# Spockuto/drand

Hardware: AMD Instinct MI355X
Metric: beacons verified/s (batch chain verify) (higher is better)
Workload: dtype u32 (381-bit Montgomery, 12x32-bit limbs); 1 GPU; configs[1]: 1000000-round chained beacon history per GPU, chain.VerifyBeacon per round; beacons_per_gpu=1000000, segment_len=64, parallelism=range-shard x1

## Files before the change

drand_amd/csrc/bls_constants.h:

```cpp
#pragma once
#include <stdint.h>
namespace bls {
static constexpr uint32_t P_RAW[12] = {0xffffaaabu, 0xb9feffffu, 0xb153ffffu, 0x1eabfffeu, 0xf6b0f624u, 0x6730d2a0u, 0xf38512bfu, 0x64774b84u, 0x434bacd7u, 0x4b1ba7b6u, 0x397fe69au, 0x1a0111eau};
static constexpr uint32_t P2_RAW[12] = {0xffff5556u, 0x73fdffffu, 0x62a7ffffu, 0x3d57fffdu, 0xed61ec48u, 0xce61a541u, 0xe70a257eu, 0xc8ee9709u, 0x869759aeu, 0x96374f6cu, 0x72ffcd34u, 0x340223d4u};
static constexpr uint32_t P4_RAW[12] = {0xfffeaaacu, 0xe7fbffffu, 0xc54ffffeu, 0x7aaffffau, 0xdac3d890u, 0x9cc34a83u, 0xce144afdu, 0x91dd2e13u, 0xd2eb35du, 0x2c6e9ed9u, 0xe5ff9a69u, 0x680447a8u};
static constexpr uint32_t P_INV32 = 0xfffcfffdu;
static constexpr uint32_t P_INV28 = 0xffcfffdu;
static constexpr uint32_t NEG28_16P[14] = {0x1ffaaab0u, 0x1efffffeu, 0x1ffffb9eu, 0x1ffeb152u, 0x1241eabeu, 0x10f6b0f5u, 0x16730d29u, 0x138512beu, 0x1774b84eu, 0x1bacd763u, 0x1a7b6433u, 0x169a4b1au, 0x1ea397fdu, 0x1a0110u};
static constexpr uint32_t NEG28_32P[14] = {0x2ff55560u, 0x2dfffffdu, 0x2ffff73du, 0x2ffd62a5u, 0x2483d57du, 0x21ed61eau, 0x2ce61a52u, 0x270a257cu, 0x2ee9709cu, 0x2759aec6u, 0x24f6c867u, 0x2d349635u, 0x2d472ffau, 0x340221u};
static constexpr uint32_t NEG28_4P[14] = {0x1ffeaaacu, 0x1fbffffeu, 0x1ffffee6u, 0x1fffac53u, 0x18907aaeu, 0x183dac3cu, 0x1d9cc349u, 0x1ce144aeu, 0x11dd2e12u, 0x12eb35d8u, 0x1e9ed90cu, 0x19a692c5u, 0x17a8e5feu, 0x68043u};
static constexpr uint32_t P28[14] = {0xfffaaabu, 0xfefffffu, 0x3ffffb9u, 0xfffeb15u, 0x6241eabu, 0xa0f6b0fu, 0xf6730d2u, 0xf38512bu, 0x4774b84u, 0x4bacd76u, 0xba7b643u, 0xe69a4b1u, 0x1ea397fu, 0x1a011u};
static constexpr uint32_t FP_INV_FIX[12] = {0x46546125u, 0x2a3b8f55u, 0x6d2fabd9u, 0xdf7c01c3u, 0xfd5fa0c1u, 0xad2b495du, 0xdb357496u, 0x9be1fa38u, 0x9cf0a900u, 0xd59c4badu, 0xdf0786dcu, 0x59a7509u};
static constexpr uint32_t FP_ONE[12] = {0x347fcb8u, 0x19d80000u, 0x6d2002b1u, 0x12e00cdeu, 0xa2090c72u, 0x37669f83u, 0xda0f73e0u, 0x9b09b42u, 0x8f1297bbu, 0xa7c515d9u, 0xfcfa012cu, 0x577a659u};
static constexpr uint32_t FP_R2[12] = {0x510370edu, 0x626d1c34u, 0xc53e243du, 0xd65aec45u, 0x3317d3b1u, 0x4f36a009u, 0x5d74088bu, 0x8c10ea72u, 0x75865d11u, 0xd507320au, 0xa759fd5cu, 0xc8d4cc8u};
static constexpr uint32_t FP_2POW256_R2[12] = {0xbe8eaa74u, 0xc38ed26eu, 0x981fba0u, 0x7d393ebdu, 0xbbe5d6f8u, 0xa0f90a33u, 0x57cc7447u, 0xc62094au, 0x5091120cu, 0x3c87c481u, 0x306035d0u, 0x122a8du};
static constexpr uint32_t FP_INV2[12] = {0x1a3fe5cu, 0x8cec0000u, 0x36900158u, 0x970066fu, 0xd1048639u, 0x1bb34fc1u, 0x6d07b9f0u, 0x84d84da1u, 0xc7894bddu, 0x53e28aecu, 0xfe7d0096u, 0x2bbd32cu};
static constexpr uint32_t FP_TWO[12] = {0x68ff970u, 0x33b00000u, 0xda400562u, 0x25c019bcu, 0x441218e4u, 0x6ecd3f07u, 0xb41ee7c0u, 0x13613685u, 0x1e252f76u, 0x4f8a2bb3u, 0xf9f40259u, 0xaef4cb3u};
static constexpr uint32_t EXP_P_MINUS_2[12] = {0xffffaaa9u, 0xb9feffffu, 0xb153ffffu, 0x1eabfffeu, 0xf6b0f624u, 0x6730d2a0u, 0xf38512bfu, 0x64774b84u, 0x434bacd7u, 0x4b1ba7b6u, 0x397fe69au, 0x1a0111eau};
static constexpr uint32_t EXP_P_PLUS_1_DIV_4[12] = {0xffffeaabu, 0xee7fbfffu, 0xac54ffffu, 0x7aaffffu, 0x3dac3d89u, 0xd9cc34a8u, 0x3ce144afu, 0xd91dd2e1u, 0x90d2eb35u, 0x92c6e9edu, 0x8e5ff9a6u, 0x680447au};
static constexpr uint32_t EXP_P_MINUS_1_DIV_2[12] = {0xffffd555u, 0xdcff7fffu, 0x58a9ffffu, 0xf55ffffu, 0x7b587b12u, 0xb3986950u, 0x79c2895fu, 0xb23ba5c2u, 0x21a5d66bu, 0x258dd3dbu, 0x1cbff34du, 0xd0088f5u};
static constexpr uint32_t EXP_P_MINUS_3_DIV_4[12] = {0xffffeaaau, 0xee7fbfffu, 0xac54ffffu, 0x7aaffffu, 0x3dac3d89u, 0xd9cc34a8u, 0x3ce144afu, 0xd91dd2e1u, 0x90d2eb35u, 0x92c6e9edu, 0x8e5ff9a6u, 0x680447au};
static constexpr int EXP_SQRT_W4_N = 79, EXP_SQRT_W4_TAIL = 1;
static constexpr uint16_t EXP_SQRT_W4[79] = {13, 2305, 1025, 1807, 1029, 1543, 1547, 1039, 1039, 1549, 1549, 1545, 771, 1805, 1037, 1551, 1293, 1033, 2061, 1547, 773, 771, 1549, 1031, 771, 769, 1543, 1031, 1289, 1031, 2057, 775, 1287, 1797, 1801, 1291, 1039, 771, 1287, 1027, 2061, 1285, 513, 2319, 1293, 771, 2063, 771, 1801, 2319, 1029, 1291, 1039, 1039, 1039, 775, 1291, 1541, 1289, 1039, 1039, 1039, 1039, 1037, 515, 1551, 1039, 1295, 1039, 1039, 1039, 1039, 1039, 1039, 1039, 773, 1029, 1029, 513};
static constexpr uint32_t FP_P_MINUS_1_DIV_2_RAW[12] = {0xffffd555u, 0xdcff7fffu, 0x58a9ffffu, 0xf55ffffu, 0x7b587b12u, 0xb3986950u, 0x79c2895fu, 0xb23ba5c2u, 0x21a5d66bu, 0x258dd3dbu, 0x1cbff34du, 0xd0088f5u};
static constexpr uint32_t B2_TWIST[2][12] = {{0xd1ff2e0u, 0x67600000u, 0xb4800ac4u, 0x4b803379u, 0x882431c8u, 0xdd9a7e0eu, 0x683dcf80u, 0x26c26d0bu, 0x3c4a5eecu, 0x9f145766u, 0xf3e804b2u, 0x15de9967u},
    {0xd1ff2e0u, 0x67600000u, 0xb4800ac4u, 0x4b803379u, 0x882431c8u, 0xdd9a7e0eu, 0x683dcf80u, 0x26c26d0bu, 0x3c4a5eecu, 0x9f145766u, 0xf3e804b2u, 0x15de9967u}};
static constexpr uint32_t B2_TWIST_X3[2][12] = {{0x2760834au, 0xc2220000u, 0xbad8204du, 0xa5289a6fu, 0xab0aa910u, 0xca6dd4e9u, 0x51af4903u, 0xab58b018u, 0x2e47c315u, 0x4705b6c6u, 0x68b840e3u, 0xd99a863u},
    {0x2760834au, 0xc2220000u, 0xbad8204du, 0xa5289a6fu, 0xab0aa910u, 0xca6dd4e9u, 0x51af4903u, 0xab58b018u, 0x2e47c315u, 0x4705b6c6u, 0x68b840e3u, 0xd99a863u}};
static constexpr uint32_t G1_GEN_X[12] = {0x534715c5u, 0x1a3890fdu, 0xdbebf58du, 0xe3106880u, 0xab47927eu, 0xf6d425c9u, 0x71e550beu, 0x37ef9707u, 0x54a1c004u, 0xe04fd71du, 0x4a8d053fu, 0x6b9deacu};
static constexpr uint32_t G1_GEN_Y[12] = {0xe748c62fu, 0x1f06d50cu, 0x70418edau, 0x5b1f1b0fu, 0x35a73c52u, 0xfe707508u, 0xdb8a28e1u, 0x8ac13c96u, 0xc55b1b8fu, 0x5f1fe8ccu, 0x342dd2beu, 0xdc3f018u};
static constexpr uint32_t G1_GEN_NEG_Y[12] = {0x18b6e47cu, 0x9af82af3u, 0x41127125u, 0xc38ce4efu, 0xc109b9d1u, 0x68c05d98u, 0x17fae9ddu, 0xd9b60eeeu, 0x7df09147u, 0xebfbbee9u, 0x55213dbu, 0xc3d21d2u};
static constexpr int G1_B = 4;
static constexpr uint32_t SSWU_A[2][12] = {{0x0u, 0x0u, 0x0u, 0x0u, 0x0u, 0x0u, 0x0u, 0x0u, 0x0u, 0x0u, 0x0u, 0x0u},
    {0x138d971au, 0xe6b20003u, 0xab9a8615u, 0xb47410c7u, 0xb9eb97e3u, 0xc8ac67f7u, 0xde7ef8d1u, 0x7644ceb4u, 0xfca67d47u, 0x9d5dba5cu, 0xef660fbau, 0xbf6749du}};
static constexpr uint32_t SSWU_B[2][12] = {{0xf8d9b1c4u, 0x22b4000cu, 0x88faa454u, 0x3742e05cu, 0x41395d09u, 0x8d402710u, 0x5ae28bd9u, 0x1b5b3a2cu, 0xdad4ad03u, 0x4337d19u, 0x6e61acc1u, 0x141ac5c4u},
    {0xf8d9b1c4u, 0x22b4000cu, 0x88faa454u, 0x3742e05cu, 0x41395d09u, 0x8d402710u, 0x5ae28bd9u, 0x1b5b3a2cu, 0xdad4ad03u, 0x4337d19u, 0x6e61acc1u, 0x141ac5c4u}};
static constexpr uint32_t SSWU_Z[2][12] = {{0xf96fb13bu, 0x864effffu, 0xd713fa9du, 0xf8ebe641u, 0xb29edd3fu, 0xf8639399u, 0x3f662afeu, 0x511614ffu, 0x25267d61u, 0xfb917c03u, 0x3f8be440u, 0xf11c536u},
    {0xfcb7adf3u, 0xa026ffffu, 0x4433fd4eu, 0xbcbf320u, 0x54a7e9b2u, 0x2fca331du, 0x19759edfu, 0x5ac6b042u, 0xb439151cu, 0xa35691dcu, 0x3c85e56du, 0x14896b90u}};
static constexpr uint32_t SSWU_MINUS_B_OVER_A[2][12] = {{0x477f0826u, 0x10e35555u, 0xe87905b7u, 0x95649687u, 0xad25656u, 0x514359a7u, 0xa7fffc74u, 0xcf1ad2efu, 0x92e4744cu, 0xd0f3c9f5u, 0xfd481bb0u, 0x4af0497u},
    {0xb880a285u, 0xa91baaaau, 0xc8dafa48u, 0x89476976u, 0xebde9fcdu, 0x15ed78f9u, 0x4b85164bu, 0x955c7895u, 0xb067388au, 0x7a27ddc0u, 0x3c37cae9u, 0x15520d52u}};
static constexpr uint32_t SSWU_B_OVER_ZA[2][12] = {{0x417fce6eu, 0x9cfa4444u, 0x94e50124u, 0xb77a8481u, 0x355d4477u, 0x76a711eeu, 0x87ffff4au, 0x296bc3c9u, 0xea2db0dcu, 0x9030c1fdu, 0xff74d256u, 0xefcdb7u},
    {0x3b803f61u, 0xe3103333u, 0xf2a4fc91u, 0xf83c7279u, 0x569928bcu, 0x33b9cd6u, 0x5b8514e0u, 0xe8340028u, 0x84c29a42u, 0x9a8961bcu, 0x3b216f96u, 0x1731a8c2u}};
static constexpr uint32_t SSWU_SQRT_MINUS_NZ3[12] = {0x8d0eb493u, 0x7d72bd83u, 0x48e019f7u, 0x55b5ace0u, 0x571a00fdu, 0x9f4c7ed0u, 0x26a5cc92u, 0xb1adf598u, 0x2560b3ffu, 0x611680a2u, 0x15d7caf5u, 0x2ddf189u};
static constexpr uint32_t ISO_XNUM[4][2][12] = {
    {{0xe09e0c6bu, 0x3130c71cu, 0xb88d3e7cu, 0xfb03080bu, 0xef69fd13u, 0x836004dbu, 0xbc8765aeu, 0x8c02926cu, 0x9ac20150u, 0x3b748bccu, 0x3a7d34a7u, 0x19c2f748u},
     {0xe09e0c6bu, 0x3130c71cu, 0xb88d3e7cu, 0xfb03080bu, 0xef69fd13u, 0x836004dbu, 0xbc8765aeu, 0x8c02926cu, 0x9ac20150u, 0x3b748bccu, 0x3a7d34a7u, 0x19c2f748u}},
    {{0x0u, 0x0u, 0x0u, 0x0u, 0x0u, 0x0u, 0x0u, 0x0u, 0x0u, 0x0u, 0x0u, 0x0u},
     {0x4c952532u, 0xe1bf5555u, 0xfde2a37cu, 0x8cc7ddadu, 0x49b32d92u, 0xb10ee30cu, 0xb22f8229u, 0x29233efbu, 0xaf5633f2u, 0x1d5a358au, 0x2e654145u, 0x2c1a5acu}},
    {{0x59b51812u, 0x491f5555u, 0xb262ae41u, 0xd8481127u, 0xd1d75f5au, 0x8ea9611au, 0x1a6d51aau, 0x4fe5ac07u, 0xeba092deu, 0xbc6e8cf0u, 0x224d45f7u, 0x18a03f14u},
     {0xa64a9299u, 0x70dfaaaau, 0xfef151beu, 0x4663eed6u, 0x24d996c9u, 0xd8877186u, 0xd917c114u, 0x14919f7du, 0x57ab19f9u, 0x8ead1ac5u, 0x1732a0a2u, 0x160d2d6u}},
    {{0xc7799757u, 0x4dc21c71u, 0xa7878e85u, 0xf6b156c2u, 0x622a6daeu, 0xea2686bdu, 0xbbf6502du, 0xe38ec96du, 0x8a9de2a8u, 0xca970a44u, 0x1f9bb921u, 0xf0de38cu},
     {0x0u, 0x0u, 0x0u, 0x0u, 0x0u, 0x0u, 0x0u, 0x0u, 0x0u, 0x0u, 0x0u, 0x0u}}};
static constexpr uint32_t ISO_XDEN[3][2][12] = {
    {{0x0u, 0x0u, 0x0u, 0x0u, 0x0u, 0x0u, 0x0u, 0x0u, 0x0u, 0x0u, 0x0u, 0x0u},
     {0x13bb96f0u, 0x5b2fffffu, 0x643f3e2cu, 0x9bbc615cu, 0xd883e22cu, 0xde304d09u, 0xe3f894e6u, 0x8dc90d81u, 0xf78020dbu, 0x824c5633u, 0x71ae1515u, 0x166a5554u}},
    {{0x2760834au, 0xc2220000u, 0xbad8204du, 0xa5289a6fu, 0xab0aa910u, 0xca6dd4e9u, 0x51af4903u, 0xab58b018u, 0x2e47c315u, 0x4705b6c6u, 0x68b840e3u, 0xd99a863u},
     {0xd89f2761u, 0xf7dcffffu, 0xf67bdfb1u, 0x7983658eu, 0x4ba64d13u, 0x9cc2fdb7u, 0xa1d5c9bbu, 0xb91e9b6cu, 0x1503e9c1u, 0x415f0f0u, 0xd0c7a5b7u, 0xc676986u}},
    {{0x347fcb8u, 0x19d80000u, 0x6d2002b1u, 0x12e00cdeu, 0xa2090c72u, 0x37669f83u, 0xda0f73e0u, 0x9b09b42u, 0x8f1297bbu, 0xa7c515d9u, 0xfcfa012cu, 0x577a659u},
     {0x0u, 0x0u, 0x0u, 0x0u, 0x0u, 0x0u, 0x0u, 0x0u, 0x0u, 0x0u, 0x0u, 0x0u}}};
static constexpr uint32_t ISO_YNUM[4][2][12] = {
    {{0xfc94688eu, 0x5d4c84bdu, 0xd498e2aeu, 0xe31cf4abu, 0xb6e04d92u, 0xa0223d24u, 0x195094cbu, 0xb108e51u, 0x87f98fcu, 0x97994773u, 0x74de4b3au, 0xba95982u},
     {0xfc94688eu, 0x5d4c84bdu, 0xd498e2aeu, 0xe31cf4abu, 0xb6e04d92u, 0xa0223d24u, 0x195094cbu, 0xb108e51u, 0x87f98fcu, 0x97994773u, 0x74de4b3au, 0xba95982u}},
    {{0x0u, 0x0u, 0x0u, 0x0u, 0x0u, 0x0u, 0x0u, 0x0u, 0x0u, 0x0u, 0x0u, 0x0u},
     {0x91dcb082u, 0x66ebc71cu, 0xf430fde0u, 0xcf5dd32au, 0x9005a116u, 0x55b52da9u, 0xcade666u, 0x99c87dc1u, 0x817e27fcu, 0xf884c5f6u, 0xa28c997au, 0x1890b86bu}},
    {{0x53251ea2u, 0x156f5555u, 0xd822a8dfu, 0xb287f76au, 0x8dc54676u, 0x1fdc2213u, 0x664e69eau, 0x3c847581u, 0xcd7b6368u, 0x6ce4613du, 0x2859439eu, 0xdb0f260u},
     {0xacda8c09u, 0xa48faaaau, 0xd9315720u, 0x6c240893u, 0x68ebafadu, 0x4754b08du, 0x8d36a8d5u, 0x27f2d603u, 0x75d0496fu, 0xde374678u, 0x1126a2fbu, 0xc501f8au}},
    {{0x682cb11cu, 0x7969a12fu, 0x34425d3u, 0x62a8e314u, 0x31822d7cu, 0x7f036ea1u, 0xbd2f9630u, 0xd5a2d607u, 0x3d8f4364u, 0x802c347bu, 0x8a1647du, 0x3a664cau},
     {0x0u, 0x0u, 0x0u, 0x0u, 0x0u, 0x0u, 0x0u, 0x0u, 0x0u, 0x0u, 0x0u, 0x0u}}};
static constexpr uint32_t ISO_YDEN[4][2][12] = {
    {{0x76673449u, 0x8124fffau, 0xe2d7750bu, 0xd0e4830u, 0x41a27e57u, 0x312db116u, 0x963a1facu, 0x5c61d772u, 0x7c8664f0u, 0x963fbea8u, 0x8a94fd7du, 0x478a667u},
     {0x76673449u, 0x8124fffau, 0xe2d7750bu, 0xd0e4830u, 0x41a27e57u, 0x312db116u, 0x963a1facu, 0x5c61d772u, 0x7c8664f0u, 0x963fbea8u, 0x8a94fd7du, 0x478a667u}},
    {{0x0u, 0x0u, 0x0u, 0x0u, 0x0u, 0x0u, 0x0u, 0x0u, 0x0u, 0x0u, 0x0u, 0x0u},
     {0x3b336f7au, 0x9d91fffdu, 0xca15ba85u, 0x95dd2417u, 0x9c29ba3du, 0xcc2f41dbu, 0xc4df9935u, 0xe06c917bu, 0x5fe908e3u, 0xf0adb32fu, 0xe20a720bu, 0xf3cdc28u}},
    {{0x3b10c4efu, 0xa3330000u, 0x98443074u, 0xf7bce7a7u, 0x808ffd98u, 0xafa4bf5eu, 0x7a86ed85u, 0x81050824u, 0x456ba4a0u, 0xea889229u, 0x1d146154u, 0x14667c95u},
     {0xc4eee5bcu, 0x16cbffffu, 0x190fcf8bu, 0x26ef1857u, 0x7620f88bu, 0xb78c1342u, 0x78fe2539u, 0xe3724360u, 0xfde00836u, 0x6093158cu, 0x1c6b8545u, 0x59a9555u}},
    {{0x347fcb8u, 0x19d80000u, 0x6d2002b1u, 0x12e00cdeu, 0xa2090c72u, 0x37669f83u, 0xda0f73e0u, 0x9b09b42u, 0x8f1297bbu, 0xa7c515d9u, 0xfcfa012cu, 0x577a659u},
     {0x0u, 0x0u, 0x0u, 0x0u, 0x0u, 0x0u, 0x0u, 0x0u, 0x0u, 0x0u, 0x0u, 0x0u}}};
static constexpr uint32_t PSI_KX[2][12] = {{0x0u, 0x0u, 0x0u, 0x0u, 0x0u, 0x0u, 0x0u, 0x0u, 0x0u, 0x0u, 0x0u, 0x0u},
    {0x758a1811u, 0x1c96e486u, 0x8561d5c1u, 0x6366543eu, 0xfc9113eu, 0xe5efbb4bu, 0x8680210au, 0x99941307u, 0xf7f70026u, 0xbfcb02eeu, 0x59199086u, 0x1291e685u}};
static constexpr uint32_t PSI_KY[2][12] = {{0x5cc17b84u, 0xe7cc5da5u, 0x6771835du, 0xae313e1eu, 0x9a07a9e4u, 0x6625579bu, 0xb7f1997du, 0x271cc4dau, 0xfea667f9u, 0x70c65115u, 0x746a4a33u, 0xd16de5bu},
    {0xa33e2f27u, 0xd232a25au, 0x49e27ca1u, 0x707ac1e0u, 0x5ca94c3fu, 0x10b7b05u, 0x3b937942u, 0x3d5a86aau, 0x44a544deu, 0xda5556a0u, 0xc5159c66u, 0xcea338eu}};
static constexpr uint32_t PSI2_KX[2][12] = {{0x72421b59u, 0x2bee486u, 0x1841d310u, 0x50864760u, 0x6dc004ccu, 0xae891bc7u, 0xac70ad2au, 0x8fe377c4u, 0x68e4686bu, 0x1805ed15u, 0x5c1f8f5au, 0xd1a402bu},
    {0x0u, 0x0u, 0x0u, 0x0u, 0x0u, 0x0u, 0x0u, 0x0u, 0x0u, 0x0u, 0x0u, 0x0u}};
static constexpr uint32_t PSI2_KY[2][12] = {{0xfcb7adf3u, 0xa026ffffu, 0x4433fd4eu, 0xbcbf320u, 0x54a7e9b2u, 0x2fca331du, 0x19759edfu, 0x5ac6b042u, 0xb439151cu, 0xa35691dcu, 0x3c85e56du, 0x14896b90u},
    {0x0u, 0x0u, 0x0u, 0x0u, 0x0u, 0x0u, 0x0u, 0x0u, 0x0u, 0x0u, 0x0u, 0x0u}};
static constexpr uint32_t FROB1_GAMMA[6][2][12] = {
    {{0x347fcb8u, 0x19d80000u, 0x6d2002b1u, 0x12e00cdeu, 0xa2090c72u, 0x37669f83u, 0xda0f73e0u, 0x9b09b42u, 0x8f1297bbu, 0xa7c515d9u, 0xfcfa012cu, 0x577a659u},
     {0x0u, 0x0u, 0x0u, 0x0u, 0x0u, 0x0u, 0x0u, 0x0u, 0x0u, 0x0u, 0x0u, 0x0u}},
    {{0x19f1ba38u, 0x18ed52b3u, 0x15a3131fu, 0xde3f9328u, 0x4a4df35bu, 0x6f74657cu, 0x266b7cccu, 0xd2acd4ffu, 0x88cae398u, 0x121243b6u, 0x376fa613u, 0x1c3e72du},
     {0xe60df073u, 0xa111ad4cu, 0x9bb0ece0u, 0x406c6cd6u, 0xac6302c8u, 0xf7bc6d24u, 0xcd1995f2u, 0x91ca7685u, 0xba80c93eu, 0x390963ffu, 0x2104087u, 0x183d2abdu}},
    {{0x0u, 0x0u, 0x0u, 0x0u, 0x0u, 0x0u, 0x0u, 0x0u, 0x0u, 0x0u, 0x0u, 0x0u},
     {0x72421b59u, 0x2bee486u, 0x1841d310u, 0x50864760u, 0x6dc004ccu, 0xae891bc7u, 0xac70ad2au, 0x8fe377c4u, 0x68e4686bu, 0x1805ed15u, 0x5c1f8f5au, 0xd1a402bu}},
    {{0xa33e2f27u, 0xd232a25au, 0x49e27ca1u, 0x707ac1e0u, 0x5ca94c3fu, 0x10b7b05u, 0x3b937942u, 0x3d5a86aau, 0x44a544deu, 0xda5556a0u, 0xc5159c66u, 0xcea338eu},
     {0xa33e2f27u, 0xd232a25au, 0x49e27ca1u, 0x707ac1e0u, 0x5ca94c3fu, 0x10b7b05u, 0x3b937942u, 0x3d5a86aau, 0x44a544deu, 0xda5556a0u, 0xc5159c66u, 0xcea338eu}},
    {{0x758a1811u, 0x1c96e486u, 0x8561d5c1u, 0x6366543eu, 0xfc9113eu, 0xe5efbb4bu, 0x8680210au, 0x99941307u, 0xf7f70026u, 0xbfcb02eeu, 0x59199086u, 0x1291e685u},
     {0x0u, 0x0u, 0x0u, 0x0u, 0x0u, 0x0u, 0x0u, 0x0u, 0x0u, 0x0u, 0x0u, 0x0u}},
    {{0xbd2fe95fu, 0xeb1ff50du, 0x5f858fc0u, 0x4eba5508u, 0xa6f73f9bu, 0x707fe081u, 0x61fef60eu, 0x10075ba9u, 0xcd702877u, 0xec679a56u, 0xfc854279u, 0xeae1abbu},
     {0x42cfc14cu, 0xcedf0af2u, 0x51ce703eu, 0xcff1aaf6u, 0x4fb9b688u, 0xf6b0f21fu, 0x91861cb0u, 0x546fefdbu, 0x75db8460u, 0x5eb40d5fu, 0x3cfaa420u, 0xb52f72eu}}};
static constexpr uint32_t FROB2_GAMMA[6][2][12] = {
    {{0x347fcb8u, 0x19d80000u, 0x6d2002b1u, 0x12e00cdeu, 0xa2090c72u, 0x37669f83u, 0xda0f73e0u, 0x9b09b42u, 0x8f1297bbu, 0xa7c515d9u, 0xfcfa012cu, 0x577a659u},
     {0x0u, 0x0u, 0x0u, 0x0u, 0x0u, 0x0u, 0x0u, 0x0u, 0x0u, 0x0u, 0x0u, 0x0u}},
    {{0x8dbd8f52u, 0xb7401b79u, 0x99122cefu, 0xce25b89eu, 0x88f0f157u, 0xb8a7b6d9u, 0x47146594u, 0xd493d3c0u, 0xda67446bu, 0x3315baa0u, 0xdd605740u, 0xce6d1beu},
     {0x0u, 0x0u, 0x0u, 0x0u, 0x0u, 0x0u, 0x0u, 0x0u, 0x0u, 0x0u, 0x0u, 0x0u}},
    {{0x8a75929au, 0x9d681b79u, 0x2bf22a3eu, 0xbb45abc0u, 0xe6e7e4e5u, 0x81411755u, 0x6d04f1b4u, 0xcae3387du, 0x4b54acb0u, 0x8b50a4c7u, 0xe0665613u, 0x76f2b64u},
     {0x0u, 0x0u, 0x0u, 0x0u, 0x0u, 0x0u, 0x0u, 0x0u, 0x0u, 0x0u, 0x0u, 0x0u}},
    {{0xfcb7adf3u, 0xa026ffffu, 0x4433fd4eu, 0xbcbf320u, 0x54a7e9b2u, 0x2fca331du, 0x19759edfu, 0x5ac6b042u, 0xb439151cu, 0xa35691dcu, 0x3c85e56du, 0x14896b90u},
     {0x0u, 0x0u, 0x0u, 0x0u, 0x0u, 0x0u, 0x0u, 0x0u, 0x0u, 0x0u, 0x0u, 0x0u}},
    {{0x72421b59u, 0x2bee486u, 0x1841d310u, 0x50864760u, 0x6dc004ccu, 0xae891bc7u, 0xac70ad2au, 0x8fe377c4u, 0x68e4686bu, 0x1805ed15u, 0x5c1f8f5au, 0xd1a402bu},
     {0x0u, 0x0u, 0x0u, 0x0u, 0x0u, 0x0u, 0x0u, 0x0u, 0x0u, 0x0u, 0x0u, 0x0u}},
    {{0x758a1811u, 0x1c96e486u, 0x8561d5c1u, 0x6366543eu, 0xfc9113eu, 0xe5efbb4bu, 0x8680210au, 0x99941307u, 0xf7f70026u, 0xbfcb02eeu, 0x59199086u, 0x1291e685u},
     {0x0u, 0x0u, 0x0u, 0x0u, 0x0u, 0x0u, 0x0u, 0x0u, 0x0u, 0x0u, 0x0u, 0x0u}}};
static constexpr uint64_t BLS_X_ABS = 0xd201000000010000ull;
static constexpr uint32_t R_ORDER[8] = {0x1u, 0xffffffffu, 0xfffe5bfeu, 0x53bda402u, 0x9a1d805u, 0x3339d808u, 0x299d7d48u, 0x73eda753u};
static constexpr uint32_t FR_RAW[8] = {0x1u, 0xffffffffu, 0xfffe5bfeu, 0x53bda402u, 0x9a1d805u, 0x3339d808u, 0x299d7d48u, 0x73eda753u};
static constexpr uint32_t FR_INV32 = 0xffffffffu;
static constexpr uint32_t FR_R2[8] = {0xf3f29c6du, 0xc999e990u, 0x87925c23u, 0x2b6cedcbu, 0x7254398fu, 0x5d31496u, 0x9f59ff11u, 0x748d9d9u};
static constexpr uint32_t FR_ONE[8] = {0xfffffffeu, 0x1u, 0x34802u, 0x5884b7fau, 0xecbc4ff5u, 0x998c4fefu, 0xacc5056fu, 0x1824b159u};
static constexpr uint32_t EXP_R_MINUS_2[8] = {0xffffffffu, 0xfffffffeu, 0xfffe5bfeu, 0x53bda402u, 0x9a1d805u, 0x3339d808u, 0x299d7d48u, 0x73eda753u};
static constexpr uint32_t SHA256_K[64] = {0x428a2f98u, 0x71374491u, 0xb5c0fbcfu, 0xe9b5dba5u, 0x3956c25bu, 0x59f111f1u, 0x923f82a4u, 0xab1c5ed5u, 0xd807aa98u, 0x12835b01u, 0x243185beu, 0x550c7dc3u, 0x72be5d74u, 0x80deb1feu, 0x9bdc06a7u, 0xc19bf174u, 0xe49b69c1u, 0xefbe4786u, 0xfc19dc6u, 0x240ca1ccu, 0x2de92c6fu, 0x4a7484aau, 0x5cb0a9dcu, 0x76f988dau, 0x983e5152u, 0xa831c66du, 0xb00327c8u, 0xbf597fc7u, 0xc6e00bf3u, 0xd5a79147u, 0x6ca6351u, 0x14292967u, 0x27b70a85u, 0x2e1b2138u, 0x4d2c6dfcu, 0x53380d13u, 0x650a7354u, 0x766a0abbu, 0x81c2c92eu, 0x92722c85u, 0xa2bfe8a1u, 0xa81a664bu, 0xc24b8b70u, 0xc76c51a3u, 0xd192e819u, 0xd6990624u, 0xf40e3585u, 0x106aa070u, 0x19a4c116u, 0x1e376c08u, 0x2748774cu, 0x34b0bcb5u, 0x391c0cb3u, 0x4ed8aa4au, 0x5b9cca4fu, 0x682e6ff3u, 0x748f82eeu, 0x78a5636fu, 0x84c87814u, 0x8cc70208u, 0x90befffau, 0xa4506cebu, 0xbef9a3f7u, 0xc67178f2u};
static constexpr uint32_t SHA256_IV[8] = {0x6a09e667u, 0xbb67ae85u, 0x3c6ef372u, 0xa54ff53au, 0x510e527fu, 0x9b05688cu, 0x1f83d9abu, 0x5be0cd19u};
static constexpr uint32_t SHA256_ZPAD_MIDSTATE[8] = {0xda5698beu, 0x17b9b469u, 0x62335799u, 0x779fbecau, 0x8ce5d491u, 0xc0d26243u, 0xbafef9eau, 0x1837a9d8u};
static constexpr int DST_LEN = 43;
static constexpr uint8_t DST[43] = {66, 76, 83, 95, 83, 73, 71, 95, 66, 76, 83, 49, 50, 51, 56, 49, 71, 50, 95, 88, 77, 68, 58, 83, 72, 65, 45, 50, 53, 54, 95, 83, 83, 87, 85, 95, 82, 79, 95, 78, 85, 76, 95};
static constexpr uint32_t XMD_B0_A_TAIL[8] = {0x1000042u, 0x4c535f53u, 0x49475f42u, 0x4c533132u, 0x33383147u, 0x325f584du, 0x443a5348u, 0x412d3235u};
static constexpr uint32_t XMD_B0_B[16] = {0x365f5353u, 0x57555f52u, 0x4f5f4e55u, 0x4c5f2b80u, 0x0u, 0x0u, 0x0u, 0x0u, 0x0u, 0x0u, 0x0u, 0x0u, 0x0u, 0x0u, 0x0u, 0x478u};
static constexpr uint32_t XMD_BI_A_TAIL[8] = {0x424c53u, 0x5f534947u, 0x5f424c53u, 0x31323338u, 0x3147325fu, 0x584d443au, 0x5348412du, 0x3235365fu};
static constexpr uint32_t XMD_BI_B[16] = {0x53535755u, 0x5f524f5fu, 0x4e554c5fu, 0x2b800000u, 0x0u, 0x0u, 0x0u, 0x0u, 0x0u, 0x0u, 0x0u, 0x0u, 0x0u, 0x0u, 0x0u, 0x268u};
}
```

drand_amd/csrc/engine_ctx.h:

```cpp
#pragma once
#include <hip/hip_runtime.h>

#include <algorithm>
#include <cerrno>
#include <cstdarg>
#include <cstdio>
#include <cstdlib>
#include <cstring>
#include <string>
#include <vector>

#include "../../include/blsverify.h"
#include "hostlogic.h"
#include "kernels.h"

namespace blsv_detail {

constexpr size_t kMaxChunk = size_t(1) << 20;
constexpr size_t kMinChunk = size_t(1) << 14;
constexpr size_t kLineSub = kMaxChunk;
constexpr size_t kPkTable = 4096;
constexpr size_t kFexpParkWords(size_t items) { return blsk::FEXP_PARK_WORDS(items) + 48 * 64; }
constexpr size_t kHqWords(size_t items) { return std::max(items * blsk::HQ_WORDS, kFexpParkWords(items)); }
constexpr size_t kStagingBytesPerItem =
    4 * (blsk::H_WORDS + blsk::HQ_WORDS + 3 + blsk::S_WORDS + 4 * blsk::F_WORDS + blsk::MILLER_LINE_WORDS) + 3;
static_assert(kHqWords(kMaxChunk) <= (blsk::HQ_WORDS + 3) * kMaxChunk, "kStagingBytesPerItem: HQ with the park");
static_assert(576ull * kMaxChunk < 0x7fffffffull, "SoA object resource exceeds its 31-bit num_records");
static_assert((133ull * kMaxChunk) * 4 < 0xffffffffull, "SoA VGPR byte offset exceeds 32 bits");
static_assert(48ull * 4 * kMaxChunk < 0x7fffffffull, "3-lane park slot resource exceeds 31 bits");
static_assert(blsk::G1_WORDS <= blsk::H_WORDS, "timelock: the U table does not fit the H staging");
static_assert(blsk::F_WORDS <= blsk::HQ_WORDS, "timelock: the captured Fp12 does not fit the HQ staging");
static_assert(BLSV_GT_LEN == 4 * blsk::F_WORDS, "timelock: the Gt encoding is one F staging row per item");
static_assert(BLSV_U_LEN <= 4 * blsk::S_WORDS, "timelock: a host call's compressed U bytes do not fit the S staging");
static_assert(BLSV_SCALAR_LEN <= 4 * blsk::S_WORDS, "sealing: a host call's scalars do not fit the S staging");
static_assert(BLSV_U_LEN <= 4 * blsk::H_WORDS, "sealing: the compressed U bytes do not fit the H staging");
static_assert(blsk::G1_WORDS <= blsk::S_WORDS, "sealing: the decoded key does not fit the S staging");
static_assert(blsk::FEXP_PARK_WORDS(1) + blsk::kTlockTabWords <= 64 * blsk::MILLER_LINE_WORDS,
              "sealing: the base's line table does not fit LN behind the park (the smallest workspace is 64 items)");

static_assert(96 + BLSV_SCALAR_LEN + 8 + BLSV_U_LEN + 1 <= 4 * blsk::S_WORDS,
              "sealing to many rounds: the P table, scalars, rounds, U and ok bytes do not fit the S staging");
static_assert(96 == 4 * blsk::G1_WORDS && (96 + BLSV_SCALAR_LEN) % 8 == 0,
              "sealing to many rounds: seal_rounds_layout's P entry, and the alignment of the rounds behind the scalars");
static_assert(blsk::kMillerLine1Words <= blsk::MILLER_LINE_WORDS &&
                  blsk::FEXP_PARK_WORDS(kMaxChunk) <= blsk::MILLER_LINE_WORDS * kMaxChunk,
              "sealing to many rounds: the single-pair lines, then the park, do not fit LN");

static_assert(2 * blsk::kTlockTabWords <= blsk::MILLER_LINE_WORDS,
              "opening across rounds: the tables of a pass's signatures (at most one per item) exceed half of LN");
static_assert(blsk::FEXP_PARK_WORDS(kMaxChunk) <= blsk::MILLER_LINE_WORDS * kMaxChunk,
              "opening across rounds: the park does not fit LN behind the f pass");
static_assert(2 + 4 + 4 + 4 * blsk::kTlockTileWords <= 4 * 3 * blsk::F_WORDS,
              "opening across rounds: the signatures' flags and the plan of a pass do not fit the FW staging");

static_assert(2 * BLSV_TLOCK_MSG_MAX <= 4 * blsk::F_WORDS,
              "timelock in one call: a pass's input and output bytes do not fit the F staging");

static_assert(BLSV_SEED_LEN == 32 && BLSV_V_LEN == 32 && BLSV_SCALAR_LEN == 32,
              "authenticated timelock: tauth_layout's rows of seeds, V bytes and scalars");
static_assert(blsk::kTauthSeedLen == BLSV_SEED_LEN && blsk::kTauthVLen == BLSV_V_LEN,
              "authenticated timelock: the header's sizes are the kernels'");
static_assert(32 + 32 + 8 + BLSV_U_LEN + 32 + 2 * BLSV_TLOCK_MSG_MAX + 1 + 16 <= 1024,
              "authenticated timelock: tauth_fits bounds a pass's staging by 1 KiB per item");
static_assert(blsk::G1_WORDS <= blsk::H_WORDS, "authenticated timelock: the U table the opening tail reads is the pass's own in H");

struct DBuf {
  void* p = nullptr;
  size_t sz = 0;
  ~DBuf() {
    if (p) (void)hipFree(p);
  }
  void release() {
    if (p) (void)hipFree(p);
    p = nullptr;
    sz = 0;
  }
  hipError_t ensure(size_t need) {
    if (need <= sz) return hipSuccess;
    if (p) {
      (void)hipFree(p);
      p = nullptr;
      sz = 0;
    }
    size_t want = std::max(need, size_t(256));
    hipError_t e = hipMalloc(&p, want);
    if (e == hipSuccess) sz = want;
    return e;
  }
  template <typename T>
  T* as() const {
    return static_cast<T*>(p);
  }
};

struct PinBuf {
  void* p = nullptr;
  size_t sz = 0;
  ~PinBuf() {
    if (p) (void)hipHostFree(p);
  }
  hipError_t ensure(size_t need) {
    if (need <= sz) return hipSuccess;
    if (p) (void)hipHostFree(p);
    p = nullptr;
    sz = 0;
    const size_t want = std::max(need + need / 2, size_t(4096));
    hipError_t e = hipHostMalloc(&p, want, hipHostMallocDefault);
    if (e == hipSuccess) sz = want;
    return e;
  }
  template <typename T>
  T* as() const {
    return static_cast<T*>(p);
  }
};

}
using namespace blsv_detail;

enum Stage {
  ST_HASH = 0,
  ST_DECOMP = 1,
  ST_MILLER = 2,
  ST_FEXP = 3,
  ST_FINISH = 4,
  ST_LAT = 5,
  ST_RLC = 6,
  ST_TLOCK = 7,
  ST_N = 8
};
struct ProfRec {
  int stage;
  size_t items;
  hipEvent_t a, b;
  hipEvent_t a2 = nullptr, b2 = nullptr;
};

constexpr size_t kRlcGroupDefault = 64;
constexpr size_t kRlcGroupMin = 8, kRlcGroupMax = 4096;
constexpr size_t kLatMaxDefault = 1536;
inline size_t chunk_env() {
  static const size_t v = [] {
    const char* e = getenv("BLSV_CHUNK");
    if (!e) return kMaxChunk;
    char* end = nullptr;
    errno = 0;
    const unsigned long long x = strtoull(e, &end, 10);
    if (end == e || *end != '\0' || errno == ERANGE || e[0] == '-' || x == 0) {
      fprintf(stderr, "blsverify: ignoring BLSV_CHUNK=\"%s\" (not a positive integer); chunk stays %zu\n", e, kMaxChunk);
      return kMaxChunk;
    }
    const size_t c = (size_t)std::min<unsigned long long>(std::max<unsigned long long>(x, kMinChunk), kMaxChunk);
    return (c + 63) & ~size_t(63);
  }();
  return v;
}

inline size_t lat_max_env() {
  static const size_t v = [] {
    const char* e = getenv("BLSV_LAT_MAX");
    if (!e) return kLatMaxDefault;
    char* end = nullptr;
    errno = 0;
    const unsigned long long x = strtoull(e, &end, 10);
    if (end == e || *end != '\0' || errno == ERANGE || e[0] == '-') {
      fprintf(stderr, "blsverify: ignoring BLSV_LAT_MAX=\"%s\" (not a non-negative integer); cutover stays %zu\n", e,
              kLatMaxDefault);
      return kLatMaxDefault;
    }
    return (size_t)std::min<unsigned long long>(x, kMaxChunk);
  }();
  return v;
}

inline size_t tlock_lat_max_env() {
  static const size_t v = [] {
    const char* e = getenv("BLSV_TLOCK_LAT_MAX");
    if (!e) return size_t(0);
    char* end = nullptr;
    errno = 0;
    const unsigned long long x = strtoull(e, &end, 10);
    if (end == e || *end != '\0' || errno == ERANGE || e[0] == '-') {
      fprintf(stderr, "blsverify: ignoring BLSV_TLOCK_LAT_MAX=\"%s\" (not a non-negative integer); it stays 0\n", e);
      return size_t(0);
    }
    return (size_t)std::min<unsigned long long>(x, kMaxChunk);
  }();
  return v;
}

inline size_t tseal_lat_max_env() {
  static const size_t v = [] {
    const char* e = getenv("BLSV_TSEAL_LAT_MAX");
    if (!e) return size_t(0);
    char* end = nullptr;
    errno = 0;
    const unsigned long long x = strtoull(e, &end, 10);
    if (end == e || *end != '\0' || errno == ERANGE || e[0] == '-') {
      fprintf(stderr, "blsverify: ignoring BLSV_TSEAL_LAT_MAX=\"%s\" (not a non-negative integer); it stays 0\n", e);
      return size_t(0);
    }
    return (size_t)std::min<unsigned long long>(x, kMaxChunk);
  }();
  return v;
}

inline size_t tauth_lat_max_env(const char* name) {
  const char* e = getenv(name);
  if (!e) return 0;
  char* end = nullptr;
  errno = 0;
  const unsigned long long x = strtoull(e, &end, 10);
  if (end == e || *end != '\0' || errno == ERANGE || e[0] == '-') {
    fprintf(stderr, "blsverify: ignoring %s=\"%s\" (not a non-negative integer); it stays 0\n", name, e);
    return 0;
  }
  return (size_t)std::min<unsigned long long>(x, kMaxChunk);
}

struct rlc_state {
  size_t group = kRlcGroupDefault;
  bool seed_pinned = false;
  uint8_t seed[32] = {0};
  uint64_t groups = 0, groups_failed = 0, items_exact = 0;
  DBuf part, gH, gS, g_hinf, g_sinf, gcls, cH, cS, c_hinf, c_sinf, ccls, fail, out96;
  PinBuf host;
};

struct tlock_state {
  bool valid = false;
  uint8_t sig[96] = {0};
  uint8_t cls = 0;
  uint64_t prepared = 0, items = 0;
  DBuf d_sig, S, s_inf, s_cls, tab;
};

struct tseal_state {
  bool valid = false, t1_built = false;
  uint8_t pk[48] = {0};
  uint64_t round = 0;
  uint64_t bases = 0, items = 0;
  DBuf t1, t2;
};

struct tsealr_state {
  bool valid = false;
  uint8_t pk[48] = {0};
  uint64_t keys = 0, items = 0;
  DBuf tk;
};

struct tlockr_state {
  size_t dense_min = kTlockDenseMinDefault;
  uint64_t items = 0;
  DBuf prepared;
};

struct tlock_lat_state {
  size_t lat_max = 0;
  uint64_t launches = 0, items = 0;
  DBuf buf;
  std::vector<uint8_t> up, down;
  TlockLatPlan plan;
};

struct tseal_lat_state {
  size_t lat_max = 0;
  uint64_t launches = 0, items = 0;
  DBuf buf;
  std::vector<uint8_t> up, down;
};

struct tauth_state {
  DBuf buf;
};

struct tauth_lat_state {
  size_t open_max = 0, seal_max = 0;
  uint64_t open_launches = 0, open_items = 0, seal_launches = 0, seal_items = 0;
  int walk_waves = 8;
  DBuf buf;
  std::vector<uint8_t> up, down;
  TlockLatPlan plan;
};

struct blsv_ctx {
  int device = 0;
  bool prof = false;
  size_t chunk = chunk_env();
  size_t lat_max = std::min(lat_max_env(), chunk);
  uint64_t oom_halvings = 0;
  size_t tail_q_dev = 0, tail_q = 0;
  std::vector<ProfRec> recs;
  std::vector<hipEvent_t> event_pool;
  hipStream_t stream = nullptr;
  hipStream_t side = nullptr;
  hipEvent_t fork_ev = nullptr, join_ev = nullptr;
  hipStream_t side2 = nullptr;
  hipEvent_t hash_ev[2] = {nullptr, nullptr};
  std::string err;
  bool has_group = false;
  size_t t = 0, n = 0;
  DBuf commits, commit_inf;
  std::vector<uint8_t> group_bytes;
  DBuf pk_all, pk_all_inf;
  size_t pk_all_n = 0;
  bool pk_all_built = false;
  DBuf pk_tab, pk_inf;
  uint8_t pk_cache[48];
  bool pk_cache_valid = false;
  size_t cap = 0;
  DBuf H, S, F, FW, LN, h_inf, s_inf, cls;
  DBuf HQ;
  DBuf in_sigs, in_msgs, in_off, in_len, in_rounds, seeds, bitmap, first_bad, sk, idx, lambdas, scratch, out,
      pp_tab, pp_inf, sel, g1_cls, misc;
  PinBuf pin;
  PinBuf io_up, io_down;
  size_t io_up_off = 0;
  struct SpecSlot {
    DBuf sig, S, s_inf, cls, sel, lam, scratch, out, vmsg, voff, vlen, vcls;
    DBuf hout, saff;
    PinBuf host;
  } spec[2];
  uint64_t spec_hits = 0, spec_misses = 0;
  DBuf arena;
  rlc_state rlc;
  tlock_state tlock;
  tseal_state tseal;
  tsealr_state tsealr;
  tlockr_state tlockr;
  tlock_lat_state tlock_lat;
  tseal_lat_state tseal_lat;
  tauth_lat_state tauth_lat;
  tauth_state tauth;
};

#define HIPCHK(ctx, expr)                                                             \
  do {                                                                                \
    hipError_t e_ = (expr);                                                           \
    if (e_ != hipSuccess) return fail((ctx), BLSV_EHIP, "%s: %s", #expr, hipGetErrorString(e_)); \
  } while (0)

inline int fail(blsv_ctx* ctx, int code, const char* fmt, ...) {
  char buf[512];
  va_list ap;
  va_start(ap, fmt);
  vsnprintf(buf, sizeof buf, fmt, ap);
  va_end(ap);
  if (ctx) ctx->err = buf;
  return code;
}


int ensure_workspace(blsv_ctx* c, size_t cnt);
void release_workspace(blsv_ctx* c);

int svc_verify_mixed(blsv_ctx* c, size_t n, const uint8_t* msgs, const uint64_t* off, const uint32_t* lens,
                     const uint8_t* sigs96, const uint32_t* idx, const uint32_t* d_tab, const uint8_t* d_tab_inf,
                     uint8_t* cls_out);
```

drand_amd/csrc/gen_constants.py:

```python
import hashlib
import os

P = 0x1A0111EA397FE69A4B1BA7B6434BACD764774B84F38512BF6730D2A0F6B0F6241EABFFFEB153FFFFB9FEFFFFFFFFAAAB
R_ORDER = 0x73EDA753299D7D483339D80809A1D80553BDA402FFFE5BFEFFFFFFFF00000001
X_ABS = 0xD201000000010000
RM = 1 << 392
NL = 12
G1_X = 0x17F1D3A73197D7942695638C4FA9AC0FC3688C4F9774B905A14E3A3F171BAC586C55E83FF97A1AEFFB3AF00ADB22C6BB
G1_Y = 0x08B3F481E3AAA0F1A09E30ED741D8AE4FCF5E095D5D00AF600DB18CB2C04B3EDD03CC744A2888AE40CAA232946C5E7E1
DST = b"BLS_SIG_BLS12381G2_XMD:SHA-256_SSWU_RO_NUL_"


def limbs(v, n=NL):
    return [(v >> (32 * i)) & 0xFFFFFFFF for i in range(n)]


def mont(v):
    return (v % P) * RM % P


def m2(a, b):
    return ((a[0] * b[0] - a[1] * b[1]) % P, (a[0] * b[1] + a[1] * b[0]) % P)


def pow2(a, e):
    r = (1, 0)
    while e:
        if e & 1:
            r = m2(r, a)
        a = m2(a, a)
        e >>= 1
    return r


def inv2(a):
    n = pow((a[0] ** 2 + a[1] ** 2) % P, P - 2, P)
    return (a[0] * n % P, -a[1] * n % P)


XI = (1, 1)


def c_fp(name, v, montgomery=True):
    vv = mont(v) if montgomery else v
    return f"static constexpr uint32_t {name}[12] = {{{', '.join(hex(x) + 'u' for x in limbs(vv))}}};"


def c_fp2(name, a):
    return (f"static constexpr uint32_t {name}[2][12] = {{{{{', '.join(hex(x) + 'u' for x in limbs(mont(a[0])))}}},\n"
            f"    {{{', '.join(hex(x) + 'u' for x in limbs(mont(a[1])))}}}}};")


def c_words(name, e, n):
    w = [(e >> (32 * i)) & 0xFFFFFFFF for i in range(n)]
    return f"static constexpr uint32_t {name}[{n}] = {{{', '.join(hex(x) + 'u' for x in w)}}};  // little-endian words"


def sha256_midstate_zero_block():
    K = [0x428a2f98, 0x71374491, 0xb5c0fbcf, 0xe9b5dba5, 0x3956c25b, 0x59f111f1, 0x923f82a4, 0xab1c5ed5,
         0xd807aa98, 0x12835b01, 0x243185be, 0x550c7dc3, 0x72be5d74, 0x80deb1fe, 0x9bdc06a7, 0xc19bf174,
         0xe49b69c1, 0xefbe4786, 0x0fc19dc6, 0x240ca1cc, 0x2de92c6f, 0x4a7484aa, 0x5cb0a9dc, 0x76f988da,
         0x983e5152, 0xa831c66d, 0xb00327c8, 0xbf597fc7, 0xc6e00bf3, 0xd5a79147, 0x06ca6351, 0x14292967,
         0x27b70a85, 0x2e1b2138, 0x4d2c6dfc, 0x53380d13, 0x650a7354, 0x766a0abb, 0x81c2c92e, 0x92722c85,
         0xa2bfe8a1, 0xa81a664b, 0xc24b8b70, 0xc76c51a3, 0xd192e819, 0xd6990624, 0xf40e3585, 0x106aa070,
         0x19a4c116, 0x1e376c08, 0x2748774c, 0x34b0bcb5, 0x391c0cb3, 0x4ed8aa4a, 0x5b9cca4f, 0x682e6ff3,
         0x748f82ee, 0x78a5636f, 0x84c87814, 0x8cc70208, 0x90befffa, 0xa4506ceb, 0xbef9a3f7, 0xc67178f2]
    H = [0x6a09e667, 0xbb67ae85, 0x3c6ef372, 0xa54ff53a, 0x510e527f, 0x9b05688c, 0x1f83d9ab, 0x5be0cd19]
    M = 0xFFFFFFFF

    def rotr(x, n):
        return ((x >> n) | (x << (32 - n))) & M
    w = [0] * 64
    for t in range(16, 64):
        s0 = rotr(w[t - 15], 7) ^ rotr(w[t - 15], 18) ^ (w[t - 15] >> 3)
        s1 = rotr(w[t - 2], 17) ^ rotr(w[t - 2], 19) ^ (w[t - 2] >> 10)
        w[t] = (w[t - 16] + s0 + w[t - 7] + s1) & M
    a, b, c, d, e, f, g, h = H
    for t in range(64):
        S1 = rotr(e, 6) ^ rotr(e, 11) ^ rotr(e, 25)
        ch = (e & f) ^ (~e & g)
        t1 = (h + S1 + ch + K[t] + w[t]) & M
        S0 = rotr(a, 2) ^ rotr(a, 13) ^ rotr(a, 22)
        mj = (a & b) ^ (a & c) ^ (b & c)
        t2 = (S0 + mj) & M
        h, g, f, e, d, c, b, a = g, f, e, (d + t1) & M, c, b, a, (t1 + t2) & M
    return [(x + y) & M for x, y in zip(H, [a, b, c, d, e, f, g, h])], K


def main():
    out = []
    w = out.append
    w("// GENERATED by drand_amd/csrc/gen_constants.py -- do not edit.")
    w("// BLS12-381 constants; Fp values are 12 x u32 little-endian limbs in Montgomery form (R = 2^392)")
    w("// unless marked RAW.")
    w("#pragma once")
    w("#include <stdint.h>")
    w("namespace bls {")
    w(c_fp("P_RAW", P, montgomery=False))
    w(c_fp("P2_RAW", 2 * P, montgomery=False) + "  // 2p: the range bound of every stored Fp value (fp.h)")
    w(c_fp("P4_RAW", 4 * P, montgomery=False) + "  // 4p < 2^383: negation offset for a lazily-added squaring operand")
    pinv = (-pow(P, -1, 1 << 32)) % (1 << 32)
    w(f"static constexpr uint32_t P_INV32 = {hex(pinv)}u;  // -p^-1 mod 2^32")
    w(f"static constexpr uint32_t P_INV28 = {hex(pinv & ((1 << 28) - 1))}u;  // -p^-1 mod 2^28")
    c16 = [((16 * P) >> (28 * k)) & ((1 << 28) - 1) for k in range(14)]
    d16 = [c16[0] + (1 << 28)] + [c16[k] + (1 << 28) - 1 for k in range(1, 13)] + [c16[13] - 1]
    assert sum(d << (28 * k) for k, d in enumerate(d16)) == 16 * P and all(d < (1 << 29) for d in d16)
    assert d16[13] > (8 * P) >> 364 and all(d >= (1 << 28) - 1 for d in d16[:13])
    w("static constexpr uint32_t NEG28_16P[14] = {" + ", ".join(hex(d) + "u" for d in d16)
      + "};  // 16p in radix 2^28 with every limb >= any operand limb: -y = NEG28_16P - y limb-wise, no borrows")
    c32 = [((32 * P) >> (28 * k)) & ((1 << 28) - 1) for k in range(14)]
    d32 = [c32[0] + (1 << 29)] + [c32[k] + (1 << 29) - 2 for k in range(1, 13)] + [c32[13] - 2]
    assert sum(d << (28 * k) for k, d in enumerate(d32)) == 32 * P and all(d < (1 << 30) for d in d32)
    assert d32[13] >= 2 * ((8 * P) >> 364) and all(d >= (1 << 29) - 2 for d in d32[:13])
    w("static constexpr uint32_t NEG28_32P[14] = {" + ", ".join(hex(d) + "u" for d in d32)
      + "};  // 32p in radix 2^28, every limb >= any limb of a sum of two split operands: -(x + y) limb-wise")
    c4 = [((4 * P) >> (28 * k)) & ((1 << 28) - 1) for k in range(14)]
    d4 = [c4[0] + (1 << 28)] + [c4[k] + (1 << 28) - 1 for k in range(1, 13)] + [c4[13] - 1]
    assert sum(d << (28 * k) for k, d in enumerate(d4)) == 4 * P and all(d < (1 << 29) for d in d4)
    assert d4[13] >= (2 * P) >> 364 and all(d >= (1 << 28) - 1 for d in d4[:13])
    w("static constexpr uint32_t NEG28_4P[14] = {" + ", ".join(hex(d) + "u" for d in d4)
      + "};  // 4p in radix 2^28, every limb >= any limb of a value < 2p: -y = NEG28_4P - y limb-wise (limbs < 2^29)")
    w("static constexpr uint32_t P28[14] = {" + ", ".join(hex((P >> (28 * k)) & ((1 << 28) - 1)) + "u" for k in range(14)) + "};  // p in radix 2^28")
    w(c_fp("FP_INV_FIX", pow(2, 625, P) * pow(RM, 3, P) % P, montgomery=False)
      + "  // RAW 2^625 R^3 mod p: fp_inv's binary GCD leaves y^-1 = v 2^625; fp_mul(v, this) = y^-1 R^2")
    w(c_fp("FP_ONE", 1))
    w(c_fp("FP_R2", RM * RM % P, montgomery=False) + "  // RAW R^2 mod p: to_mont(x) = mont_mul(x, R2)")
    w(c_fp("FP_2POW256_R2", (1 << 256) * RM * RM % P, montgomery=False)
      + "  // RAW 2^256 R^2 mod p (hash_to_field hi half)")
    w(c_fp("FP_INV2", pow(2, P - 2, P)))
    w(c_fp("FP_TWO", 2))
    w(c_words("EXP_P_MINUS_2", P - 2, 12))
    w(c_words("EXP_P_PLUS_1_DIV_4", (P + 1) // 4, 12))
    w(c_words("EXP_P_MINUS_1_DIV_2", (P - 1) // 2, 12))
    w(c_words("EXP_P_MINUS_3_DIV_4", (P - 3) // 4, 12) + "  // a^((p-3)/4): sqrt and its inverse in one exp")
    bits = bin((P - 3) // 4)[2:]
    win, i, pend, sched = 4, 0, 0, []
    while i < len(bits):
        if bits[i] == "0":
            pend += 1
            i += 1
            continue
        j = min(i + win, len(bits))
        while bits[j - 1] == "0":
            j -= 1
        sched.append(((pend + j - i) if sched else 0) << 8 | int(bits[i:j], 2))
        pend, i = 0, j
    val = 0
    for ent in sched:
        val = (val << (ent >> 8)) + (ent & 255)
    assert (val << pend) == (P - 3) // 4 and all((e & 255) % 2 == 1 for e in sched)
    w("static constexpr int EXP_SQRT_W4_N = %d, EXP_SQRT_W4_TAIL = %d;" % (len(sched), pend))
    w("static constexpr uint16_t EXP_SQRT_W4[%d] = {" % len(sched) + ", ".join(str(x) for x in sched)
      + "};  // (p-3)/4, 4-bit sliding window: squarings << 8 | odd digit (first entry: the start digit)")
    w(c_fp("FP_P_MINUS_1_DIV_2_RAW", (P - 1) // 2, montgomery=False) + "  // RAW, for the sign rule")
    w(c_fp2("B2_TWIST", (4, 4)) + "  // b' = 4(1+i)")
    w(c_fp2("B2_TWIST_X3", (12, 12)) + "  // 3b'")
    w(c_fp("G1_GEN_X", G1_X))
    w(c_fp("G1_GEN_Y", G1_Y))
    w(c_fp("G1_GEN_NEG_Y", (-G1_Y) % P))
    w("static constexpr int G1_B = 4;")
    A = (0, 240)
    B = (1012, 1012)
    Z = ((-2) % P, (-1) % P)
    w(c_fp2("SSWU_A", A))
    w(c_fp2("SSWU_B", B))
    w(c_fp2("SSWU_Z", Z))
    negB_over_A = m2(((-B[0]) % P, (-B[1]) % P), inv2(A))
    w(c_fp2("SSWU_MINUS_B_OVER_A", negB_over_A))
    w(c_fp2("SSWU_B_OVER_ZA", m2(B, inv2(m2(Z, A)))))
    nz = (Z[0] * Z[0] + Z[1] * Z[1]) % P
    c = (-nz * nz * nz) % P
    cr = pow(c, (P + 1) // 4, P)
    assert cr * cr % P == c, "-N(Z)^3 must be a square"
    w(c_fp("SSWU_SQRT_MINUS_NZ3", cr) + "  // sqrt(-N(Z)^3) in Fp")

    def h(v):
        return v % P
    iso = {
        "ISO_XNUM": [(h(0x5C759507E8E333EBB5B7A9A47D7ED8532C52D39FD3A042A88B58423C50AE15D5C2638E343D9C71C6238AAAAAAAA97D6),
                      h(0x5C759507E8E333EBB5B7A9A47D7ED8532C52D39FD3A042A88B58423C50AE15D5C2638E343D9C71C6238AAAAAAAA97D6)),
                     (0, h(0x11560BF17BAA99BC32126FCED787C88F984F87ADF7AE0C7F9A208C6B4F20A4181472AAA9CB8D555526A9FFFFFFFFC71A)),
                     (h(0x11560BF17BAA99BC32126FCED787C88F984F87ADF7AE0C7F9A208C6B4F20A4181472AAA9CB8D555526A9FFFFFFFFC71E),
                      h(0x8AB05F8BDD54CDE190937E76BC3E447CC27C3D6FBD7063FCD104635A790520C0A395554E5C6AAAA9354FFFFFFFFE38D)),
                     (h(0x171D6541FA38CCFAED6DEA691F5FB614CB14B4E7F4E810AA22D6108F142B85757098E38D0F671C7188E2AAAAAAAA5ED1), 0)],
        "ISO_XDEN": [(0, (-72) % P), (12, (-12) % P), (1, 0)],
        "ISO_YNUM": [(h(0x1530477C7AB4113B59A4C18B076D11930F7DA5D4A07F649BF54439D87D27E500FC8C25EBF8C92F6812CFC71C71C6D706),
                      h(0x1530477C7AB4113B59A4C18B076D11930F7DA5D4A07F649BF54439D87D27E500FC8C25EBF8C92F6812CFC71C71C6D706)),
                     (0, h(0x5C759507E8E333EBB5B7A9A47D7ED8532C52D39FD3A042A88B58423C50AE15D5C2638E343D9C71C6238AAAAAAAA97BE)),
                     (h(0x11560BF17BAA99BC32126FCED787C88F984F87ADF7AE0C7F9A208C6B4F20A4181472AAA9CB8D555526A9FFFFFFFFC71C),
                      h(0x8AB05F8BDD54CDE190937E76BC3E447CC27C3D6FBD7063FCD104635A790520C0A395554E5C6AAAA9354FFFFFFFFE38F)),
                     (h(0x124C9AD43B6CF79BFBF7043DE3811AD0761B0F37A1E26286B0E977C69AA274524E79097A56DC4BD9E1B371C71C718B10), 0)],
        "ISO_YDEN": [((-432) % P, (-432) % P), (0, (-216) % P), (18, (-18) % P), (1, 0)],
    }
    for name, coeffs in iso.items():
        rows = []
        for c in coeffs:
            rows.append("{{" + ", ".join(hex(x) + "u" for x in limbs(mont(c[0]))) + "},\n     {"
                        + ", ".join(hex(x) + "u" for x in limbs(mont(c[1]))) + "}}")
        w(f"static constexpr uint32_t {name}[{len(coeffs)}][2][12] = {{\n    " + ",\n    ".join(rows) + "};")
    kx = inv2(pow2(XI, (P - 1) // 3))
    ky = inv2(pow2(XI, (P - 1) // 2))
    w(c_fp2("PSI_KX", kx))
    w(c_fp2("PSI_KY", ky))
    kx2 = m2((kx[0], (-kx[1]) % P), kx)
    ky2 = m2((ky[0], (-ky[1]) % P), ky)
    w(c_fp2("PSI2_KX", kx2))
    w(c_fp2("PSI2_KY", ky2))
    g1 = pow2(XI, (P - 1) // 6)
    g2 = pow2(XI, (P * P - 1) // 6)
    g1p = [(1, 0)]
    g2p = [(1, 0)]
    for _ in range(5):
        g1p.append(m2(g1p[-1], g1))
        g2p.append(m2(g2p[-1], g2))
    w("// FROB1_GAMMA[k] = xi^(k(p-1)/6), FROB2_GAMMA[k] = xi^(k(p^2-1)/6), k = 0..5 (w-power index)")
    for name, arr in (("FROB1_GAMMA", g1p), ("FROB2_GAMMA", g2p)):
        rows = []
        for c in arr:
            rows.append("{{" + ", ".join(hex(x) + "u" for x in limbs(mont(c[0]))) + "},\n     {"
                        + ", ".join(hex(x) + "u" for x in limbs(mont(c[1]))) + "}}")
        w(f"static constexpr uint32_t {name}[6][2][12] = {{\n    " + ",\n    ".join(rows) + "};")
    w(f"static constexpr uint64_t BLS_X_ABS = {hex(X_ABS)}ull;  // x = -BLS_X_ABS")
    w(c_words("R_ORDER", R_ORDER, 8))
    RR = 1 << 256
    w(c_words("FR_RAW", R_ORDER, 8))
    w(f"static constexpr uint32_t FR_INV32 = {hex((-pow(R_ORDER, -1, 1 << 32)) % (1 << 32))}u;")
    w(c_words("FR_R2", RR * RR % R_ORDER, 8) + "  // RAW R^2 mod r")
    w(c_words("FR_ONE", RR % R_ORDER, 8) + "  // Montgomery 1")
    w(c_words("EXP_R_MINUS_2", R_ORDER - 2, 8))
    mid, K = sha256_midstate_zero_block()
    w("static constexpr uint32_t SHA256_K[64] = {" + ", ".join(hex(x) + "u" for x in K) + "};")
    w("static constexpr uint32_t SHA256_IV[8] = {0x6a09e667u, 0xbb67ae85u, 0x3c6ef372u, 0xa54ff53au, "
      "0x510e527fu, 0x9b05688cu, 0x1f83d9abu, 0x5be0cd19u};")
    w("static constexpr uint32_t SHA256_ZPAD_MIDSTATE[8] = {" + ", ".join(hex(x) + "u" for x in mid) + "};")
    w(f"static constexpr int DST_LEN = {len(DST)};")
    w("static constexpr uint8_t DST[" + str(len(DST)) + "] = {" + ", ".join(str(x) for x in DST) + "};")
    dst_prime = DST + bytes([len(DST)])

    def be_words(bs):
        assert len(bs) % 4 == 0
        return [int.from_bytes(bs[i:i + 4], "big") for i in range(0, len(bs), 4)]

    def pad_tail(tail, total_len):
        bs = tail + b"\x80"
        while (len(bs) % 64) != 56:
            bs += b"\x00"
        return bs + (total_len * 8).to_bytes(8, "big")
    b0_a_tail = b"\x01\x00\x00" + dst_prime[:29]
    assert len(b0_a_tail) == 32
    b0_b = pad_tail(dst_prime[29:], 64 + 32 + 2 + 1 + len(dst_prime))
    assert len(b0_b) == 64
    bi_a_tail = b"\x00" + dst_prime[:31]
    bi_b = pad_tail(dst_prime[31:], 32 + 1 + len(dst_prime))
    assert len(bi_b) == 64
    w("// expand_message_xmd block words (big-endian): words 8..15 of the first block, whole 2nd block")
    w("static constexpr uint32_t XMD_B0_A_TAIL[8] = {" + ", ".join(hex(x) + "u" for x in be_words(b0_a_tail)) + "};")
    w("static constexpr uint32_t XMD_B0_B[16] = {" + ", ".join(hex(x) + "u" for x in be_words(b0_b)) + "};")
    w("static constexpr uint32_t XMD_BI_A_TAIL[8] = {" + ", ".join(hex(x) + "u" for x in be_words(bi_a_tail))
      + "};  // byte 0 of word 0 = i (OR in i << 24)")
    w("static constexpr uint32_t XMD_BI_B[16] = {" + ", ".join(hex(x) + "u" for x in be_words(bi_b)) + "};")
    w("}  // namespace bls")
    assert hashlib.sha256(bytes(64)).digest()
    path = os.path.join(os.path.dirname(os.path.abspath(__file__)), "bls_constants.h")
    with open(path, "w") as f:
        f.write("\n".join(out) + "\n")
    print("wrote", path)


if __name__ == "__main__":
    main()
```

drand_amd/csrc/host_internal.h:

```cpp
#pragma once
#include <functional>
#include <initializer_list>

#include "engine_ctx.h"
#include "hostlogic.h"

#pragma GCC visibility push(hidden)

constexpr size_t kIoCap = size_t(1) << 20;
hipError_t h2d(blsv_ctx* c, void* dst, const void* src, size_t len);
struct Down {
  void* user;
  const void* dev;
  size_t len;
};
hipError_t download_sync(blsv_ctx* c, std::initializer_list<Down> ds);

hipEvent_t take_event(blsv_ctx* c);
struct StageTimer {
  blsv_ctx* c;
  int stage;
  size_t items;
  hipStream_t st;
  hipEvent_t a = nullptr;
  StageTimer(blsv_ctx* c_, int stage_, size_t items_, hipStream_t st_) : c(c_), stage(stage_), items(items_), st(st_) {
    if (c->prof && (a = take_event(c))) (void)hipEventRecord(a, st);
  }
  ~StageTimer() {
    if (!a) return;
    hipEvent_t b = take_event(c);
    if (!b) return;
    (void)hipEventRecord(b, st);
    c->recs.push_back({stage, items, a, b});
  }
};

struct Staging {
  uint32_t *H, *HQ, *S, *F, *FW, *LN;
  uint8_t *h_inf, *s_inf, *cls;
};
inline Staging staging(const blsv_ctx* c) {
  return {c->H.as<uint32_t>(),    c->HQ.as<uint32_t>(),   c->S.as<uint32_t>(),
          c->F.as<uint32_t>(),    c->FW.as<uint32_t>(),   c->LN.as<uint32_t>(),
          c->h_inf.as<uint8_t>(), c->s_inf.as<uint8_t>(), c->cls.as<uint8_t>()};
}

struct SigSrc {
  const uint8_t* d;
  size_t stride, offset;
};
struct PkSel {
  const uint32_t* tab;
  const uint8_t* inf;
  const uint32_t* idx;
};
inline PkSel group_pk(const blsv_ctx* c) { return {c->commits.as<uint32_t>(), c->commit_inf.as<uint8_t>(), nullptr}; }

inline void hash_chained(blsv_ctx* c, const blsk::ChainedSrc& src, size_t base, size_t cnt, hipStream_t st) {
  const Staging w = staging(c);
  blsk::launch_hash_chained(src, base, cnt, w.H, w.h_inf, w.HQ, st);
}
inline void hash_messages(blsv_ctx* c, const uint8_t* d_msgs, const uint64_t* d_off, const uint32_t* d_len, size_t base,
                          size_t cnt, hipStream_t st) {
  const Staging w = staging(c);
  blsk::launch_hash_messages(d_msgs, d_off + base, d_len + base, cnt, w.H, w.h_inf, w.HQ, st);
}
inline void hash_uploaded(blsv_ctx* c, size_t base, size_t cnt, hipStream_t st) {
  hash_messages(c, c->in_msgs.as<uint8_t>(), c->in_off.as<uint64_t>(), c->in_len.as<uint32_t>(), base, cnt, st);
}
inline void lat_uploaded(blsv_ctx* c, const SigSrc& sig, size_t cnt, const PkSel& pk, uint8_t* cls, uint32_t* S,
                         uint8_t* s_inf, hipStream_t st) {
  blsk::launch_lat_messages(c->in_msgs.as<uint8_t>(), c->in_off.as<uint64_t>(), c->in_len.as<uint32_t>(), sig.d,
                            sig.stride, sig.offset, cnt, pk.tab, pk.inf, pk.idx, cls, S, s_inf, st);
}
inline void final_exp(blsv_ctx* c, size_t cnt, size_t base, size_t m, uint8_t* cls, hipStream_t st,
                      uint32_t* out = nullptr) {
  const Staging w = staging(c);
  blsk::launch_final_exp(w.F, w.FW, cnt, base, m, cls, st, w.HQ + (base ? blsk::FEXP_PARK_WORDS(base) : 0), out);
}
inline void final_exp(blsv_ctx* c, size_t cnt, uint8_t* cls, hipStream_t st, uint32_t* out = nullptr) {
  final_exp(c, cnt, 0, cnt, cls, st, out);
}

inline bool use_lat(const blsv_ctx* c, size_t n) { return n > 0 && n <= std::min(c->lat_max, c->cap); }
inline bool use_rlc(const blsv_ctx* c, size_t n) { return n > c->lat_max && n >= 2 * c->rlc.group; }

template <typename F>
inline int for_each_pass(const blsv_ctx* c, size_t n, F f) {
  for (size_t base = 0; base < n; base += c->cap) {
    const int rc = f(base, std::min(c->cap, n - base));
    if (rc) return rc;
  }
  return BLSV_OK;
}

using HashFn = std::function<void(size_t base, size_t cnt, hipStream_t st)>;
struct Tail {
  bool randomized = false;
  uint32_t seed[8] = {0};
  bool fused_subgroup() const { return !randomized; }
};
struct PassOut {
  uint64_t* bitmap;
  unsigned long long* first_bad;
  uint8_t* cls;
  uint64_t label0;
};
int run_head(blsv_ctx* c, const SigSrc& sig, size_t base, size_t cnt, const Tail& tail, hipStream_t st,
             const HashFn& hash);
int run_passes(blsv_ctx* c, size_t n, const SigSrc& sig, const PkSel& pk, const HashFn& hash, const Tail& tail,
               const PassOut& out, hipStream_t st);
int ctx_outputs(blsv_ctx* c, size_t n, bool with_cls, PassOut& out);

int rlc_draw_seed(blsv_ctx* c, uint32_t (&w)[8]);
int rlc_sums(blsv_ctx* c, size_t base, size_t cnt, const uint32_t (&seed)[8], hipStream_t st);

int stage_chain(blsv_ctx* c, uint64_t first_round, const uint8_t* prevs, size_t prev0_len, bool prev_rows,
                const uint8_t* sigs96, size_t n, blsk::ChainedSrc& src);
int decode_g1(blsv_ctx* c, const uint8_t* pk48, size_t cnt, DBuf& tab, DBuf& inf, std::vector<uint8_t>& cls);
int upload_messages(blsv_ctx* c, const uint8_t* msgs, const uint32_t* msg_lens, size_t n);

struct MaskTail {
  size_t mlen = 0;
  bool host = false;
  bool secret = false;
};
uint8_t* mask_host_out(const blsv_ctx* c, const MaskTail& mk, size_t cnt);
int mask_tail(blsv_ctx* c, const MaskTail& mk, const uint8_t* flag, uint8_t good, size_t cnt, const uint8_t* in,
              uint8_t* d_out, hipStream_t st);
hipError_t mask_wipe(blsv_ctx* c, const MaskTail& mk, size_t cnt, hipStream_t st);

struct AuthTail {
  bool on = false;
  const uint8_t* vs = nullptr;
  const uint8_t* seeds = nullptr;
  uint8_t* out_vs = nullptr;
  AuthTail at(size_t base) const {
    AuthTail a = *this;
    if (vs) a.vs += base * 32;
    if (seeds) a.seeds += base * 32;
    if (out_vs) a.out_vs += base * 32;
    return a;
  }
};
int auth_open_tail(blsv_ctx* c, const AuthTail& au, const MaskTail& mk, size_t cnt, const uint8_t* ws, uint8_t* d_out,
                   hipStream_t st);
int auth_seal_tail(blsv_ctx* c, const AuthTail& au, const MaskTail& mk, const uint8_t* cls, size_t cnt,
                   const uint8_t* msgs, uint8_t* d_out_ws, hipStream_t st);

int tlock_prepare_sig(blsv_ctx* c, const uint8_t* sig96, hipStream_t st, uint8_t* sig_class);
int tlock_passes(blsv_ctx* c, bool host, const uint8_t* us, size_t n, uint8_t* out, uint8_t* cls, hipStream_t st,
                 const MaskTail& mk = MaskTail(), const uint8_t* mk_in = nullptr, const AuthTail& au = AuthTail());
int rounds_passes(blsv_ctx* c, bool host, const uint8_t* sigs96, const uint64_t* counts, size_t m, const uint8_t* us,
                  size_t n, uint8_t* out, uint8_t* cls, uint8_t* d_sig_class, hipStream_t st,
                  const MaskTail& mk = MaskTail(), const uint8_t* mk_in = nullptr, const AuthTail& au = AuthTail());
int seal_prepare(blsv_ctx* c, const uint8_t* pk48, uint64_t round, size_t n, hipStream_t st);
int seal_passes(blsv_ctx* c, bool host, const uint8_t* scalars, size_t n, uint8_t* us, uint8_t* gt, uint8_t* ok,
                hipStream_t st, const MaskTail& mk = MaskTail(), const uint8_t* mk_in = nullptr,
                const AuthTail& au = AuthTail());
int sealr_passes(blsv_ctx* c, bool host, const uint64_t* rounds, const uint8_t* scalars, size_t n, uint8_t* us,
                 uint8_t* gt, uint8_t* ok, hipStream_t st, const MaskTail& mk = MaskTail(),
                 const uint8_t* mk_in = nullptr, const AuthTail& au = AuthTail());

struct TlockLatOut {
  const uint8_t *gt, *cls, *sig_cls;
};
int tlock_lat_run(blsv_ctx* c, const uint8_t* sigs96, size_t m, const uint32_t* sig_of, const uint32_t* idle,
                  size_t n_idle, const uint8_t* us48, size_t n, TlockLatOut& o, const uint8_t* cs = nullptr,
                  size_t mlen = 0);
void tlock_lat_copy_out(const TlockLatOut& o, size_t n, uint8_t* out, uint8_t* ok, uint8_t* reject_class,
                        size_t out_len = BLSV_GT_LEN);

int sealr_prepare(blsv_ctx* c, const uint8_t* pk48, size_t n, hipStream_t st);

int tseal_lat_run(blsv_ctx* c, const uint8_t* pk48, const uint64_t* rounds, uint64_t round, const uint8_t* scalars32,
                  size_t n, uint8_t* out_us48, uint8_t* out, uint8_t* ok, const uint8_t* msgs = nullptr, size_t mlen = 0);

int auth_t1(blsv_ctx* c, hipStream_t st);

int tauth_lat_open_run(blsv_ctx* c, const uint8_t* sigs96, size_t m, const uint32_t* sig_of, const uint32_t* idle,
                       size_t n_idle, const uint8_t* us48, const uint8_t* vs32, const uint8_t* ws, size_t mlen, size_t n,
                       TlockLatOut& o);
int tauth_lat_seal_run(blsv_ctx* c, const uint8_t* pk48, const uint64_t* rounds, uint64_t round, const uint8_t* seeds32,
                       const uint8_t* msgs, size_t mlen, size_t n, uint8_t* out_us48, uint8_t* out_vs32, uint8_t* out_ws,
                       uint8_t* ok);

int seal_key(blsv_ctx* c, const uint8_t* pk48, const uint8_t** key);

#pragma GCC visibility pop
```

drand_amd/csrc/k_group.hip:

```cpp
#include "kcommon.h"

namespace blsk {


struct fr {
  uint32_t l[8];
};

DI fr fr_mul(const fr& a, const fr& b) {
  uint32_t t[8];
#pragma unroll
  for (int j = 0; j < 8; j++) t[j] = 0;
#pragma unroll
  for (int i = 0; i < 8; i++) {
    const uint32_t bi = b.l[i];
    uint64_t A = (uint64_t)a.l[0] * bi + t[0];
    const uint32_t m = (uint32_t)A * FR_INV32;
    uint64_t C = (uint64_t)m * FR_RAW[0] + (uint32_t)A;
#pragma unroll
    for (int j = 1; j < 8; j++) {
      A = (uint64_t)a.l[j] * bi + t[j] + (A >> 32);
      C = (uint64_t)m * FR_RAW[j] + (uint32_t)A + (C >> 32);
      t[j - 1] = (uint32_t)C;
    }
    t[7] = (uint32_t)(C >> 32) + (uint32_t)(A >> 32);
  }
  uint32_t d[8];
  unsigned br = 0;
#pragma unroll
  for (int i = 0; i < 8; i++) d[i] = __builtin_subc(t[i], FR_RAW[i], br, &br);
  fr r;
#pragma unroll
  for (int i = 0; i < 8; i++) r.l[i] = br ? t[i] : d[i];
  return r;
}

DI fr fr_small(uint32_t v) {
  fr raw = {{v, 0, 0, 0, 0, 0, 0, 0}};
  fr r2;
#pragma unroll
  for (int i = 0; i < 8; i++) r2.l[i] = FR_R2[i];
  return fr_mul(raw, r2);
}

DI fr fr_sub(const fr& a, const fr& b) {
  uint32_t d[8];
  unsigned br = 0;
#pragma unroll
  for (int i = 0; i < 8; i++) d[i] = __builtin_subc(a.l[i], b.l[i], br, &br);
  uint32_t m = br ? 0xffffffffu : 0u;
  unsigned c = 0;
  fr r;
#pragma unroll
  for (int i = 0; i < 8; i++) r.l[i] = __builtin_addc(d[i], FR_RAW[i] & m, c, &c);
  return r;
}

DI fr fr_inv(const fr& a) {
  fr r;
#pragma unroll
  for (int i = 0; i < 8; i++) r.l[i] = FR_ONE[i];
  for (int w = 7; w >= 0; w--) {
    for (int b = 31; b >= 0; b--) {
      r = fr_mul(r, r);
      if ((EXP_R_MINUS_2[w] >> b) & 1u) r = fr_mul(r, a);
    }
  }
  return r;
}

DI void st_g1(uint32_t* tab, size_t k, const g1a& a) {
#pragma unroll
  for (int w = 0; w < 12; w++) {
    tab[k * G1_WORDS + w] = a.x.l[w];
    tab[k * G1_WORDS + 12 + w] = a.y.l[w];
  }
}

DI g1a ld_g1(const uint32_t* tab, size_t k) {
  g1a a;
#pragma unroll
  for (int w = 0; w < 12; w++) {
    a.x.l[w] = tab[k * G1_WORDS + w];
    a.y.l[w] = tab[k * G1_WORDS + 12 + w];
  }
  return a;
}

__global__ void __launch_bounds__(TPB) k_decompress_g1(const uint8_t* in, size_t cnt, uint32_t* tab, uint8_t* inf,
                                                       uint8_t* cls) {
  size_t i = (size_t)blockIdx.x * TPB + threadIdx.x;
  if (i >= cnt) return;
  uint8_t buf[48];
  for (int k = 0; k < 48; k++) buf[k] = in[i * 48 + k];
  g1a a;
  bool is_inf;
  uint8_t c = g1_decompress(buf, a, is_inf);
  if (c != REJ_OK) {
    a.x = fp_zero();
    a.y = fp_zero();
    is_inf = true;
  }
  st_g1(tab, i, a);
  inf[i] = is_inf;
  cls[i] = c;
}

__global__ void __launch_bounds__(TPB) k_pubpoly_eval(const uint32_t* commits, const uint8_t* commit_inf, uint32_t t,
                                                      const uint32_t* idx, size_t cnt, uint32_t* out_tab,
                                                      uint8_t* out_inf) {
  size_t i = (size_t)blockIdx.x * TPB + threadIdx.x;
  if (i >= cnt) return;
  const uint32_t x = idx[i] + 1u;
  g1j v = jac_infinity<fp>();
  for (int j = (int)t - 1; j >= 0; j--) {
    g1j acc = jac_infinity<fp>();
    for (int b = 31 - __builtin_clz(x); b >= 0; b--) {
      acc = jac_dbl(acc);
      if ((x >> b) & 1u) acc = jac_add(acc, v);
    }
    v = acc;
    if (!commit_inf[j]) v = jac_add_aff(v, ld_g1(commits, j));
  }
  const bool is_inf = jac_is_inf(v);
  g1a a = g1_to_aff(v);
  if (is_inf) {
    a.x = fp_zero();
    a.y = fp_zero();
  }
  st_g1(out_tab, i, a);
  out_inf[i] = is_inf;
}

void launch_decompress_g1(const uint8_t* in, size_t cnt, uint32_t* tab, uint8_t* inf, uint8_t* cls, hipStream_t st) {
  if (!cnt) return;
  hipLaunchKernelGGL(k_decompress_g1, dim3(grid_for(cnt)), dim3(TPB), 0, st, in, cnt, tab, inf, cls);
}

void launch_pubpoly_eval(const uint32_t* commits, const uint8_t* commit_inf, uint32_t t, const uint32_t* idx,
                         size_t cnt, uint32_t* out_tab, uint8_t* out_inf, hipStream_t st) {
  if (!cnt) return;
  hipLaunchKernelGGL(k_pubpoly_eval, dim3(grid_for(cnt)), dim3(TPB), 0, st, commits, commit_inf, t, idx, cnt,
                     out_tab, out_inf);
}



}
```

drand_amd/csrc/k_miller.hip:

```cpp
#include <type_traits>

#include "kcommon.h"
#include "kmiller.h"
#include "testops.h"

namespace blsk {

DI int line_slot(int step, int k) { return (step * 2 + k) * 6; }
template <bool CHECK>
BLS_KERNEL(BLS_WPE_LINES)
k_miller_lines(const uint32_t* pk_tab, const uint8_t* pk_inf, const uint32_t* pk_idx, const uint32_t* H,
               const uint8_t* h_inf, const uint32_t* S, const uint8_t* s_inf,
               std::conditional_t<CHECK, uint8_t*, const uint8_t*> cls, size_t cnt, size_t base, size_t m, size_t sub,
               uint32_t* LN) {
  const int k = (int)(blockIdx.x & 1u);
  const size_t i = (size_t)(blockIdx.x >> 1) * TPB + threadIdx.x;
  if (i >= m) return;
  const size_t g = base + i;
  if (cls[g] != REJ_OK) return;
  const uint32_t kk = pk_idx ? pk_idx[g] : 0u;
  const bool act[2] = {!(pk_inf[kk] | h_inf[g]), !s_inf[g]};
  {
    const uint32_t* Qb = k == 0 ? H : S;
    auto load_q = [&]() {
      size_t j = g;
      asm volatile("" : "+v"(j));
      return g2a{ld_fp2(Qb, cnt, j, 0), ld_fp2(Qb, cnt, j, 2)};
    };
    auto emit = [&](int step, const line& l) {
      const int s = line_slot(step, k);
      const line o = act[k] ? l : line_one();
      st_fp2<BLS_LN_AUX_ST>(LN, sub, i, s + 0, o.a0);
      st_fp2<BLS_LN_AUX_ST>(LN, sub, i, s + 2, o.a1);
      st_fp2<BLS_LN_AUX_ST>(LN, sub, i, s + 4, o.a4);
    };
    auto pcoord = [&](int c) {
      size_t o = (size_t)kk * G1_WORDS + 12 * c;
      asm volatile("" : "+v"(o));
      fp v;
#pragma unroll
      for (int w = 0; w < 12; w++) v.l[w] = pk_tab[o + w];
      return k == 0 ? v : fp_load_const(c == 0 ? G1_GEN_X : G1_GEN_NEG_Y);
    };
    if (!act[k]) {
#pragma unroll 1
      for (int s = 0; s < MILLER_STEPS; s++) emit(s, line_one());
      return;
    }
    int step = 0;
    auto put = [&](int c, const fp2& v) { st_fp2<BLS_LN_AUX_ST>(LN, sub, i, line_slot(step, k) + 2 * c, v); };
    auto xp = [&]() { return pcoord(0); };
    auto yp = [&]() { return pcoord(1); };
    const g2proj_lds T{g_ml_T + threadIdx.x};
    {
      const g2a Q0 = load_q();
      T.set(0, Q0.x);
      T.set(1, Q0.y);
      T.set(2, fp2_one());
    }
#pragma unroll 1
    for (int b = 62; b >= 0; b--) {
      miller_dbl_step_ts(T, put, xp, yp);
      step++;
      if ((BLS_X_ABS >> b) & 1ull) {
        miller_add_step_ts(T, load_q, put, xp, yp);
        step++;
      }
    }
    if constexpr (CHECK) {
      if (k == 1 && !miller_t_in_subgroup(T, load_q)) {
        size_t j = g;
        asm volatile("" : "+v"(j));
        cls[j] = REJ_NOT_IN_SUBGROUP;
      }
    }
  }
}

static __shared__ uint32_t g_mf_L[120 * BLS_LANES];
DI void mf_put(int c, const fp2& v) {
  const unsigned l = threadIdx.x;
#pragma unroll
  for (int k = 0; k < 12; k++) {
    g_mf_L[(c * 24 + k) * BLS_LANES + l] = v.c0.l[k];
    g_mf_L[(c * 24 + 12 + k) * BLS_LANES + l] = v.c1.l[k];
  }
}
DI fp2 mf_get(int c) {
  unsigned l = threadIdx.x;
  asm volatile("" : "+v"(l));
  fp2 v;
#pragma unroll
  for (int k = 0; k < 12; k++) {
    v.c0.l[k] = g_mf_L[(c * 24 + k) * BLS_LANES + l];
    v.c1.l[k] = g_mf_L[(c * 24 + 12 + k) * BLS_LANES + l];
  }
  return v;
}
template <typename LB>
DI fp6 fp6_mul_lb(const fp6& a, LB lb) {
#if BLS_F6_LIN
  return fp6_mul_lin_lb(a, lb, KpLds16());
#else
  fp2 t0 = fp2_mul(a.c0, lb(0));
  fp2 t1 = fp2_mul(a.c1, lb(1));
  fp2 t2 = fp2_mul(a.c2, lb(2));
  fp2 c0 = fp2_add(fp2_mul_xi(fp2_sub(fp2_sub(fp2_mul(fp2_add_lazy(a.c1, a.c2), fp2_add_lazy(lb(1), lb(2))), t1), t2)), t0);
  fp2 c1 = fp2_add(fp2_sub(fp2_sub(fp2_mul(fp2_add_lazy(a.c0, a.c1), fp2_add_lazy(lb(0), lb(1))), t0), t1), fp2_mul_xi(t2));
  fp2 c2 = fp2_add(fp2_sub(fp2_sub(fp2_mul(fp2_add_lazy(a.c0, a.c2), fp2_add_lazy(lb(0), lb(2))), t0), t2), t1);
  return {c0, c1, c2};
#endif
}
DI fp12 fp12_mul_by_line_pair_lds(const fp12& f) {
  const fp6 t0 = fp6_mul_lb(f.c0, [](int c) { return mf_get(c); });
  fp6 t1;
  {
    const fp2 b1 = mf_get(3), b2 = mf_get(4);
    t1 = fp6_mul_by_12(f.c1, b1, b2);
  }
  const fp6 c1 = fp6_sub(fp6_sub(fp6_mul_lb(fp6_add_lazy(f.c0, f.c1), [](int c) {
                                   return c == 0 ? mf_get(0) : fp2_add_lazy(mf_get(c), mf_get(c + 2));
                                 }),
                                 t0),
                         t1);
  return {fp6_add(t0, fp6_mul_v(t1)), c1};
}

BLS_KERNEL(BLS_WPE_MILLER_F) k_miller_f(const uint32_t* LN, const uint8_t* cls, size_t cnt, size_t base,
                                                  size_t m, size_t sub, uint32_t* F) {
#if BLS_F6_LIN
  kp_lds_init<16>();
#endif
  const size_t i = (size_t)blockIdx.x * TPB + threadIdx.x;
  if (i >= m) return;
  const size_t g = base + i;
  if (cls[g] != REJ_OK) return;
  auto load = [&](int step, int k) {
    const int s = line_slot(step, k);
    return line{ld_fp2<BLS_LN_AUX_LD>(LN, sub, i, s + 0), ld_fp2<BLS_LN_AUX_LD>(LN, sub, i, s + 2),
                ld_fp2<BLS_LN_AUX_LD>(LN, sub, i, s + 4)};
  };
  fp12 f = fp12_one();
  int step = 0;
#pragma unroll 1
  for (int b = 62; b >= 0; b--) {
#pragma unroll 1
    for (int rep = 0; rep < 2; rep++) {
      if (rep == 1 && !((BLS_X_ABS >> b) & 1ull)) break;
#if BLS_F6_LIN
      if (rep == 0 && b != 62) f = fp12_sqr_lin(f, KpLds16());
#else
      if (rep == 0 && b != 62) f = fp12_sqr(f);
#endif
      {
        const fp12 L = line_mul_line(load(step, 0), load(step, 1));
        if (step == 0) {
          f = L;
          step++;
          continue;
        }
        mf_put(0, L.c0.c0);
        mf_put(1, L.c0.c1);
        mf_put(2, L.c0.c2);
        mf_put(3, L.c1.c1);
        mf_put(4, L.c1.c2);
      }
      f = fp12_mul_by_line_pair_lds(f);
      step++;
    }
  }
  st_fp12(F, cnt, g, fp12_conj(f));
}

constexpr uint64_t miller_sq_bits(int half) {
  uint64_t m = 0;
  int s = 0;
  for (int i = 62; i >= 0; i--) {
    if (i != 62 && s / 64 == half) m |= 1ull << (s % 64);
    s++;
    if ((BLS_X_ABS >> i) & 1ull) s++;
  }
  return m;
}
constexpr uint64_t MILLER_SQ_LO = miller_sq_bits(0), MILLER_SQ_HI = miller_sq_bits(1);

#ifndef BLS_MILLER_TRI_MAX
#define BLS_MILLER_TRI_MAX 65536
#endif
constexpr size_t kMillerTriMax = BLS_MILLER_TRI_MAX;

#ifndef BLS_WPE_MILLER_TRI
#define BLS_WPE_MILLER_TRI 2
#endif

BLS_KERNEL(BLS_WPE_MILLER_TRI) k_miller_f_tri(const uint32_t* LN, const uint8_t* cls, size_t cnt, size_t base,
                                              size_t m, size_t sub, uint32_t* F, uint32_t* park) {
  const tri_lane t = tri_lane_id();
  const size_t ir = (size_t)blockIdx.x * TRI_GROUPS + t.group;
  const bool in_range = t.group < TRI_GROUPS && ir < m;
  const size_t i = in_range ? ir : m - 1;
  const bool live = in_range && cls[base + i] == REJ_OK;
  const size_t park_n = (size_t)gridDim.x * TPB, park_i = (size_t)blockIdx.x * TPB + t.lane;
  fp4 A;
#pragma unroll 1
  for (int s = 0; s < MILLER_STEPS; s++) {
    const bool sq = ((s < 64 ? MILLER_SQ_LO >> s : MILLER_SQ_HI >> (s - 64)) & 1ull) != 0;
    if (sq) A = tri_sqr_lp(t, A);
    const int s0 = line_slot(s, 0), s1 = line_slot(s, 1);
    auto la = [&](int c) {
      size_t j = i;
      asm volatile("" : "+v"(j));
      return ld_fp2_v<BLS_LN_AUX_LD>(LN + (size_t)s0 * 12 * sub, sub, j, 2 * c);
    };
    auto lb = [&](int c) {
      size_t j = i;
      asm volatile("" : "+v"(j));
      return ld_fp2_v<BLS_LN_AUX_LD>(LN + (size_t)s1 * 12 * sub, sub, j, 2 * c);
    };
    const fp4 L = tri_line_pair(t, la, lb);
    if (s == 0) {
      A = L;
    } else {
      A = tri_mul_lp(t, A, L, park, park_n, park_i);
    }
  }
  A = tri_conj(t, A);
  if (live) tri_store(F, cnt, base + i, t.role, A);
}

template <int OP, int NIN, int NOUT>
__global__ void __launch_bounds__(TPB) k_test_op_mf(const uint32_t* in, size_t cnt, uint32_t* out) {
#if BLS_F6_LIN
  kp_lds_init<16>();
#endif
  const size_t i = (size_t)blockIdx.x * TPB + threadIdx.x;
  if (i >= cnt) return;
  fp x[NIN], r[NOUT];
#pragma unroll
  for (int k = 0; k < NIN; k++)
#pragma unroll
    for (int w = 0; w < 12; w++) x[k].l[w] = in[(i * NIN + k) * 12 + w];
  if constexpr (OP == TOP_fp6_mul_lb) {
#pragma unroll
    for (int c = 0; c < 3; c++) mf_put(c, t_f2(x, 6 + 2 * c));
    t_put6(r, 0, fp6_mul_lb(t_f6(x, 0), [](int c) { return mf_get(c); }));
  } else {
#pragma unroll
    for (int c = 0; c < 5; c++) mf_put(c, t_f2(x, 12 + 2 * c));
    t_put12(r, 0, fp12_mul_by_line_pair_lds(t_f12(x, 0)));
  }
#pragma unroll
  for (int k = 0; k < NOUT; k++)
#pragma unroll
    for (int w = 0; w < 12; w++) out[(i * NOUT + k) * 12 + w] = r[k].l[w];
}

bool launch_test_op_mf(int op, const uint32_t* in, size_t cnt, uint32_t* out, hipStream_t st) {
  if (op != TOP_fp6_mul_lb && op != TOP_fp12_mul_by_line_pair_lds) return false;
  if (!cnt) return true;
  if (op == TOP_fp6_mul_lb)
    hipLaunchKernelGGL((k_test_op_mf<TOP_fp6_mul_lb, 12, 6>), dim3(grid_for(cnt)), dim3(TPB), 0, st, in, cnt, out);
  else
    hipLaunchKernelGGL((k_test_op_mf<TOP_fp12_mul_by_line_pair_lds, 22, 12>), dim3(grid_for(cnt)), dim3(TPB), 0, st, in,
                       cnt, out);
  return true;
}

void launch_miller_lines(const uint32_t* pk_tab, const uint8_t* pk_inf, const uint32_t* pk_idx, const uint32_t* H,
                         const uint8_t* h_inf, const uint32_t* S, const uint8_t* s_inf, uint8_t* cls, size_t cnt,
                         size_t base, size_t m, uint32_t* LN, size_t sub, bool check_subgroup, hipStream_t st) {
  if (!m) return;
  if (check_subgroup)
    hipLaunchKernelGGL(k_miller_lines<true>, dim3(2 * grid_for(m)), dim3(TPB), 0, st, pk_tab, pk_inf, pk_idx, H, h_inf,
                       S, s_inf, cls, cnt, base, m, sub, LN);
  else
    hipLaunchKernelGGL(k_miller_lines<false>, dim3(2 * grid_for(m)), dim3(TPB), 0, st, pk_tab, pk_inf, pk_idx, H,
                       h_inf, S, s_inf, (const uint8_t*)cls, cnt, base, m, sub, LN);
}

void launch_miller_f(const uint32_t* LN, size_t sub, const uint8_t* cls, size_t cnt, size_t base, size_t m,
                     uint32_t* F, uint32_t* park, bool single_lane, hipStream_t st) {
  if (!m) return;
  LN += base % sub;
  if (m <= kMillerTriMax && !single_lane) {
    hipLaunchKernelGGL(k_miller_f_tri, dim3((unsigned)((m + TRI_GROUPS - 1) / TRI_GROUPS)), dim3(TPB), 0, st, LN, cls,
                       cnt, base, m, sub, F, park);
  } else {
    hipLaunchKernelGGL(k_miller_f, dim3(grid_for(m)), dim3(TPB), 0, st, LN, cls, cnt, base, m, sub, F);
  }
}

void launch_miller(const uint32_t* pk_tab, const uint8_t* pk_inf, const uint32_t* pk_idx, const uint32_t* H,
                   const uint8_t* h_inf, const uint32_t* S, const uint8_t* s_inf, uint8_t* cls, size_t cnt,
                   uint32_t* F, uint32_t* LN, size_t sub, uint32_t* park, bool check_subgroup, hipStream_t st) {
  if (!cnt) return;
  for (size_t b = 0; b < cnt; b += sub) {
    const size_t m = cnt - b < sub ? cnt - b : sub;
    launch_miller_lines(pk_tab, pk_inf, pk_idx, H, h_inf, S, s_inf, cls, cnt, b, m, LN, sub, check_subgroup, st);
    launch_miller_f(LN, sub, cls, cnt, b, m, F, park, false, st);
  }
}

}
```

drand_amd/csrc/kernels.h:

```cpp
#pragma once
#include <hip/hip_runtime.h>
#include <stddef.h>
#include <stdint.h>

namespace blsk {

constexpr int H_WORDS = 48;
constexpr int S_WORDS = 48;
constexpr int F_WORDS = 144;
constexpr int G1_WORDS = 24;

struct ChainedSrc {
  const uint8_t* sigs;
  const uint8_t* seeds;
  uint64_t first_round;
  uint64_t seg_len;
  uint32_t seed0_len;
  uint64_t seg_phase;
};

constexpr int HQ_WORDS = 144;
void launch_hash_chained(const ChainedSrc& src, size_t base, size_t cnt, uint32_t* H, uint8_t* h_inf,
                         uint32_t* Q, hipStream_t st);
void launch_hash_unchained(const uint64_t* rounds, uint64_t first_round, size_t base, size_t cnt, uint32_t* H,
                           uint8_t* h_inf, uint32_t* Q, hipStream_t st);
void launch_hash_messages(const uint8_t* msgs, const uint64_t* off, const uint32_t* len, size_t cnt,
                          uint32_t* H, uint8_t* h_inf, uint32_t* Q, hipStream_t st);
void launch_decompress_g2(const uint8_t* sigs, size_t stride, size_t offset, size_t base, size_t cnt, uint32_t* S,
                          uint8_t* s_inf, uint8_t* cls, hipStream_t st);
constexpr int MILLER_LINE_WORDS = 68 * 2 * 6 * 12;
void launch_miller(const uint32_t* pk_tab, const uint8_t* pk_inf, const uint32_t* pk_idx, const uint32_t* H,
                   const uint8_t* h_inf, const uint32_t* S, const uint8_t* s_inf, uint8_t* cls, size_t cnt,
                   uint32_t* F, uint32_t* LN, size_t sub, uint32_t* park, bool check_subgroup, hipStream_t st);
void launch_miller_lines(const uint32_t* pk_tab, const uint8_t* pk_inf, const uint32_t* pk_idx, const uint32_t* H,
                         const uint8_t* h_inf, const uint32_t* S, const uint8_t* s_inf, uint8_t* cls, size_t cnt,
                         size_t base, size_t m, uint32_t* LN, size_t sub, bool check_subgroup, hipStream_t st);
void launch_miller_f(const uint32_t* LN, size_t sub, const uint8_t* cls, size_t cnt, size_t base, size_t m,
                     uint32_t* F, uint32_t* park, bool single_lane, hipStream_t st);
constexpr size_t TRI_PARK_WORDS(size_t items) { return 48 * 64 * ((items + 20) / 21); }
constexpr size_t FEXP_PARK_WORDS(size_t items) { return TRI_PARK_WORDS(items); }
void launch_final_exp(uint32_t* F, uint32_t* W, size_t n, size_t base, size_t m, uint8_t* cls, hipStream_t st,
                      uint32_t* park, uint32_t* out = nullptr);
void launch_finish(const uint8_t* cls, size_t base, size_t cnt, uint64_t* bitmap, unsigned long long* first_bad,
                   uint64_t label0, hipStream_t st);

constexpr size_t kRlcLaneItems = 8;
constexpr size_t kRlcPartWords = 72;
constexpr size_t rlc_lanes(size_t cnt) { return (cnt + kRlcLaneItems - 1) / kRlcLaneItems; }
constexpr size_t rlc_groups(size_t cnt, size_t group) { return (cnt + group - 1) / group; }
void launch_rlc_sums(const uint32_t* H, const uint8_t* h_inf, const uint32_t* S, const uint8_t* s_inf,
                     const uint8_t* cls, size_t cnt, uint64_t index0, const uint32_t* seed_words, size_t group,
                     uint32_t* part, uint32_t* GH, uint8_t* g_hinf, uint32_t* GS, uint8_t* g_sinf, hipStream_t st);
void launch_rlc_gather(const uint32_t* fail, size_t group, size_t m, const uint32_t* H, const uint8_t* h_inf,
                       const uint32_t* S, const uint8_t* s_inf, const uint8_t* cls, size_t cnt, uint32_t* CH,
                       uint8_t* c_hinf, uint32_t* CS, uint8_t* c_sinf, uint8_t* ccls, hipStream_t st);
void launch_rlc_scatter(const uint32_t* fail, size_t group, size_t m, const uint8_t* ccls, uint8_t* cls, size_t cnt,
                        hipStream_t st);
void launch_rlc_compress(const uint32_t* GP, const uint8_t* g_inf, size_t ng, uint8_t* out96, hipStream_t st);

constexpr size_t kTlockTabWords = 68 * 3 * 24;
void launch_tlock_prepare(const uint32_t* S, const uint8_t* s_inf, const uint8_t* s_cls, uint32_t* tab, hipStream_t st);
void launch_tlock_f(const uint32_t* tab, const uint32_t* U, const uint8_t* u_inf, const uint8_t* cls,
                    const uint8_t* sig_inf, size_t cnt, uint32_t* F, hipStream_t st);
void launch_tlock_encode(const uint32_t* E, const uint8_t* cls, size_t cnt, uint8_t* out, hipStream_t st);

constexpr uint32_t kTlockTileMixed = 0xffffffffu;
constexpr size_t kTlockTileWords = 3;
void launch_tlock_prepare_many(const uint32_t* S, const uint8_t* s_inf, const uint8_t* s_cls, size_t M, uint32_t* tab,
                               unsigned long long* prepared, hipStream_t st);
void launch_tlock_f_tiles(const uint32_t* tiles, size_t n_uniform, size_t n_mixed, const uint32_t* sig_of,
                          const uint32_t* tab, size_t M, const uint8_t* sig_inf, const uint8_t* sig_cls,
                          const uint32_t* U, const uint8_t* u_inf, uint8_t* cls, size_t cnt, uint32_t* F,
                          hipStream_t st);
void launch_tlock_scatter_classes(const uint8_t* src, const uint32_t* sig_j, size_t M, uint8_t* dst, hipStream_t st);

constexpr size_t kTsealT1Words = 64 * 15 * 24;
constexpr size_t kTsealT2Words = 64 * 15 * 144;
void launch_tseal_g1_table(uint32_t* T1, hipStream_t st);
void launch_tseal_gt_table(const uint32_t* B, uint32_t* T2, hipStream_t st);
void launch_tseal_u(const uint32_t* T1, const uint8_t* scalars, size_t cnt, uint8_t* us, uint8_t* ok, uint8_t* cls,
                    hipStream_t st);
void launch_tseal_gt(const uint32_t* T2, const uint8_t* scalars, const uint8_t* cls, size_t cnt, uint32_t* E,
                     hipStream_t st);

constexpr size_t kMillerLine1Words = 68 * 6 * 12;
void launch_tseal_key_table(const uint32_t* key, uint32_t* TK, hipStream_t st);
void launch_tsealr_point(const uint32_t* TK, const uint8_t* scalars, const uint8_t* cls, size_t cnt, uint32_t* P,
                         hipStream_t st);
void launch_miller_lines1(const uint32_t* P, const uint32_t* H, const uint8_t* h_inf, const uint8_t* cls, size_t cnt,
                          uint32_t* LN, hipStream_t st);
void launch_miller_f1(const uint32_t* LN, const uint8_t* h_inf, const uint8_t* cls, size_t cnt, uint32_t* F,
                      hipStream_t st);

constexpr size_t kTmaskMsgMax = 256;
void launch_tmask(const uint32_t* E, const uint8_t* flag, uint8_t good, size_t cnt, const uint8_t* in, uint8_t* out,
                  size_t mlen, hipStream_t st);
void launch_tmask_encoded(const uint8_t* gt576, const uint8_t* flag, uint8_t good, size_t cnt, const uint8_t* in,
                          uint8_t* out, size_t mlen, hipStream_t st);

constexpr size_t kTauthSeedLen = 32, kTauthVLen = 32;
void launch_tauth_derive(const uint8_t* seeds, const uint8_t* msgs, size_t cnt, size_t mlen, uint8_t* scalars,
                         hipStream_t st);
void launch_tauth_seal_tail(const uint32_t* E, const uint8_t* cls, size_t cnt, const uint8_t* seeds, const uint8_t* msgs,
                            size_t mlen, uint8_t* out_vs, uint8_t* out_ws, hipStream_t st);
void launch_tauth_open_tail(const uint32_t* E, const uint32_t* U, const uint8_t* u_inf, uint8_t* cls, size_t cnt,
                            const uint32_t* T1, const uint8_t* vs, const uint8_t* ws, size_t mlen, uint8_t* out,
                            hipStream_t st);

int lat_trace_read(uint64_t* out, int n, hipStream_t st);
int lat_trace_clear(hipStream_t st);
int lat_trace_enable(int on, hipStream_t st);
extern int g_generic_chains_all;
void launch_lat_chained(const ChainedSrc& src, size_t base, size_t cnt, const uint32_t* pk_tab, const uint8_t* pk_inf,
                        uint8_t* cls, hipStream_t st);
void launch_lat_unchained(const uint64_t* rounds, uint64_t first_round, const uint8_t* sigs, size_t base, size_t cnt,
                          const uint32_t* pk_tab, const uint8_t* pk_inf, uint8_t* cls, hipStream_t st);
void launch_lat_messages(const uint8_t* msgs, const uint64_t* off, const uint32_t* len, const uint8_t* sigs,
                         size_t stride, size_t offset, size_t cnt, const uint32_t* pk_tab, const uint8_t* pk_inf,
                         const uint32_t* pk_idx, uint8_t* cls, uint32_t* S, uint8_t* s_inf, hipStream_t st);
void launch_lat_tlock(const uint8_t* sigs, const uint32_t* sig_of, const uint8_t* us, size_t n_items,
                      const uint32_t* idle, size_t n_idle, uint8_t* out, uint8_t* cls, uint8_t* sig_cls,
                      hipStream_t st);
void launch_lat_tseal(const uint32_t* T1, const uint32_t* TK, const uint64_t* rounds, uint64_t round,
                      const uint8_t* scalars, size_t n, uint8_t* us, uint8_t* gts, uint8_t* ok, hipStream_t st);

void launch_decompress_g1(const uint8_t* in, size_t cnt, uint32_t* tab, uint8_t* inf, uint8_t* cls, hipStream_t st);
void launch_pubpoly_eval(const uint32_t* commits, const uint8_t* commit_inf, uint32_t t, const uint32_t* idx,
                         size_t cnt, uint32_t* out_tab, uint8_t* out_inf, hipStream_t st);
void launch_lat_tauth_open(const uint8_t* sigs, const uint32_t* sig_of, const uint8_t* us, const uint8_t* vs,
                           const uint8_t* ws, size_t mlen, size_t n_items, const uint32_t* idle, size_t n_idle,
                           const uint32_t* T1, uint8_t* out, uint8_t* cls, uint8_t* sig_cls, int walk_waves,
                           hipStream_t st);
void launch_lat_tauth_seal(const uint32_t* T1, const uint32_t* TK, const uint64_t* rounds, uint64_t round,
                           const uint8_t* seeds, const uint8_t* msgs, size_t mlen, size_t n, uint8_t* us, uint8_t* vs,
                           uint8_t* ws, uint8_t* ok, hipStream_t st);

void launch_lat_decode(const uint8_t* sigs, size_t stride, size_t offset, size_t cnt, uint32_t* S, uint8_t* s_inf,
                       uint8_t* cls, hipStream_t st);
void launch_decompress_g2_only(const uint8_t* sigs, size_t stride, size_t offset, size_t base, size_t cnt,
                               uint32_t* S, uint8_t* s_inf, uint8_t* cls, hipStream_t st);
void launch_lat_recover(const uint32_t* S, size_t n_s, const uint8_t* s_inf, const uint32_t* sel,
                        const uint32_t* lambdas, uint32_t t, uint32_t* scratch, uint8_t* out96, hipStream_t st,
                        uint32_t* saff = nullptr);
constexpr size_t kLatHoutWords = 448, kLatSaffWords = 192;
void launch_lat_hash_key(const uint8_t* msgs, const uint64_t* off, const uint32_t* len, const uint32_t* pk_tab,
                         const uint8_t* pk_inf, uint32_t* hout, hipStream_t st);
void launch_lat_verify_pre(const uint32_t* hout, const uint32_t* saff, uint8_t* cls, hipStream_t st);
void launch_sign(const uint32_t* sk_words, int32_t index, const uint32_t* H, const uint8_t* h_inf, size_t cnt,
                 uint8_t* out, size_t out_stride, hipStream_t st);
void launch_gen_chained(const uint32_t* sk_words, const ChainedSrc& src, size_t n, uint8_t* sigs_out, hipStream_t st);

bool launch_test_op(int op, const uint32_t* in, size_t cnt, uint32_t* out, uint32_t* park, hipStream_t st);
bool launch_test_op_mf(int op, const uint32_t* in, size_t cnt, uint32_t* out, hipStream_t st);
void launch_test_fp_mul(const uint32_t* a, const uint32_t* b, size_t cnt, uint32_t* out, hipStream_t st);
void launch_test_pairing(const uint32_t* p_tab, const uint32_t* q_aff, size_t cnt, uint32_t* out_f, hipStream_t st);
void launch_test_unpack_g2(const uint32_t* H, size_t cnt, uint32_t* out, hipStream_t st);
void launch_test_pack_fp12(const uint32_t* f, size_t cnt, uint32_t* F, hipStream_t st);
void launch_test_unpack_fp12(const uint32_t* F, size_t cnt, uint32_t* out, hipStream_t st);
void launch_test_final_exp_ref(const uint32_t* F, size_t cnt, uint32_t* out, hipStream_t st);

}
```

drand_amd/csrc/pairing.h:

```cpp
#pragma once
#include "curve.h"

namespace bls {

struct g2proj {
  fp2 x, y, z;
};

DI fp2 fp2_mul_3b(const fp2& c) {
  fp2 x4 = fp2_dbl(fp2_dbl(fp2_mul_xi(c)));
  return fp2_add(fp2_dbl(x4), x4);
}

template <bool INL = false>
DI void miller_dbl_step(g2proj& t, fp2& l00, fp2& l01, fp2& l11, const fp& xp, const fp& yp) {
  auto mul = [](const fp2& a, const fp2& b) { return INL ? fp2_mul_inl(a, b) : fp2_mul(a, b); };
  auto sqr = [](const fp2& a) { return INL ? fp2_sqr_inl(a) : fp2_sqr(a); };
  fp2 A = fp2_half(mul(t.x, t.y));
  fp2 B = sqr(t.y);
  fp2 C = sqr(t.z);
  fp2 E = fp2_mul_3b(C);
  fp2 F = fp2_mul3(E);
  fp2 G = fp2_half(fp2_add(B, F));
  fp2 H = fp2_sub(sqr(fp2_add_lazy(t.y, t.z)), fp2_add(B, C));
  fp2 X2 = sqr(t.x);
  l00 = fp2_sub(E, B);
  l01 = fp2_mul_fp(fp2_mul3(X2), xp);
  l11 = fp2_neg(fp2_mul_fp(H, yp));
  t.x = mul(A, fp2_sub(B, F));
  t.y = fp2_sub(sqr(G), fp2_mul3(sqr(E)));
  t.z = mul(B, H);
}



struct g2proj_reg {
  g2proj& t;
  DI fp2 get(int c) const { return c == 0 ? t.x : c == 1 ? t.y : t.z; }
  DI void set(int c, const fp2& v) const {
    if (c == 0) t.x = v;
    else if (c == 1) t.y = v;
    else t.z = v;
  }
};

template <typename TS, typename Put, typename XP, typename YP>
DI void miller_dbl_step_ts(const TS& t, Put put, XP xp, YP yp) {
  const fp2 B = fp2_sqr_inl(t.get(1));
  BLS_SCHED_FENCE();
  const fp2 C = fp2_sqr_inl(t.get(2));
  BLS_SCHED_FENCE();
  const fp2 H = fp2_sub(fp2_sqr_inl(fp2_add_lazy(t.get(1), t.get(2))), fp2_add(B, C));
  BLS_SCHED_FENCE();
  put(2, fp2_neg(fp2_mul_fp_inl(H, yp())));
  BLS_SCHED_FENCE();
  t.set(2, fp2_mul_inl_k<0>(B, H));
  BLS_SCHED_FENCE();
  const fp2 E = fp2_mul_3b(C);
  const fp2 F = fp2_mul3(E);
  const fp2 G = fp2_half(fp2_add(B, F));
  put(0, fp2_sub(E, B));
  const fp2 BF = fp2_sub(B, F);
  const fp2 A = fp2_half(fp2_mul_inl_k<1>(t.get(0), t.get(1)));
  BLS_SCHED_FENCE();
  put(1, fp2_mul_fp_inl(fp2_mul3(fp2_sqr_inl(t.get(0))), xp()));
  BLS_SCHED_FENCE();
  t.set(0, fp2_mul_inl(A, BF));
  BLS_SCHED_FENCE();
  const fp2 G2 = fp2_sqr_inl(G);
  BLS_SCHED_FENCE();
  t.set(1, fp2_sub(G2, fp2_mul3(fp2_sqr_inl(E))));
}

template <typename TS, typename Put, typename Q, typename XP, typename YP>
DI void miller_add_step_ts(const TS& t, Q qload, Put put, XP xp, YP yp) {
  fp2 theta, delta;
  {
    const g2a q = qload();
    theta = fp2_sub(t.get(1), fp2_mul_inl(q.y, t.get(2)));
    BLS_SCHED_FENCE();
    delta = fp2_sub(t.get(0), fp2_mul_inl(q.x, t.get(2)));
    BLS_SCHED_FENCE();
    const fp2 u = fp2_mul_inl(theta, q.x);
    BLS_SCHED_FENCE();
    put(0, fp2_sub(u, fp2_mul_inl(delta, q.y)));
    BLS_SCHED_FENCE();
  }
  put(1, fp2_neg(fp2_mul_fp_inl(theta, xp())));
  BLS_SCHED_FENCE();
  put(2, fp2_mul_fp_inl(delta, yp()));
  BLS_SCHED_FENCE();
  const fp2 C = fp2_sqr_inl(theta);
  BLS_SCHED_FENCE();
  const fp2 D = fp2_sqr_inl(delta);
  BLS_SCHED_FENCE();
  const fp2 E = fp2_mul_inl(D, delta);
  BLS_SCHED_FENCE();
  const fp2 F = fp2_mul_inl(t.get(2), C);
  BLS_SCHED_FENCE();
  const fp2 G = fp2_mul_inl(t.get(0), D);
  BLS_SCHED_FENCE();
  const fp2 H = fp2_sub(fp2_add(E, F), fp2_dbl(G));
  t.set(0, fp2_mul_inl(delta, H));
  BLS_SCHED_FENCE();
  t.set(1, fp2_sub(fp2_mul_inl(theta, fp2_sub(G, H)), fp2_mul_inl(t.get(1), E)));
  BLS_SCHED_FENCE();
  t.set(2, fp2_mul_inl(t.get(2), E));
}

template <typename TS, typename Q>
DI bool miller_t_in_subgroup(const TS& t, Q qload) {
  bool ok = !fp2_is_zero(t.get(2));
  {
    const fp2 px = fp2_mul_inl(fp2_conj(qload().x), fp2_load_const(PSI_KX));
    BLS_SCHED_FENCE();
    ok &= fp2_eq(t.get(0), fp2_mul_inl(px, t.get(2)));
  }
  BLS_SCHED_FENCE();
  {
    const fp2 py = fp2_mul_inl(fp2_conj(qload().y), fp2_load_const(PSI_KY));
    BLS_SCHED_FENCE();
    ok &= fp2_eq(fp2_neg(t.get(1)), fp2_mul_inl(py, t.get(2)));
  }
  return ok;
}

template <typename Put, typename XP, typename YP>
DI void miller_dbl_step_inl(g2proj& t, Put put, XP xp, YP yp) {
  miller_dbl_step_ts(g2proj_reg{t}, put, xp, yp);
}
template <typename Put, typename Q, typename XP, typename YP>
DI void miller_add_step_inl(g2proj& t, Q qload, Put put, XP xp, YP yp) {
  miller_add_step_ts(g2proj_reg{t}, qload, put, xp, yp);
}

DI void miller_add_step(g2proj& t, const g2a& q, fp2& l00, fp2& l01, fp2& l11, const fp& xp, const fp& yp) {
  fp2 theta = fp2_sub(t.y, fp2_mul(q.y, t.z));
  fp2 delta = fp2_sub(t.x, fp2_mul(q.x, t.z));
  l00 = fp2_sub(fp2_mul(theta, q.x), fp2_mul(delta, q.y));
  l01 = fp2_neg(fp2_mul_fp(theta, xp));
  l11 = fp2_mul_fp(delta, yp);
  fp2 C = fp2_sqr(theta);
  fp2 D = fp2_sqr(delta);
  fp2 E = fp2_mul(D, delta);
  fp2 F = fp2_mul(t.z, C);
  fp2 G = fp2_mul(t.x, D);
  fp2 H = fp2_sub(fp2_add(E, F), fp2_dbl(G));
  t.x = fp2_mul(delta, H);
  t.y = fp2_sub(fp2_mul(theta, fp2_sub(G, H)), fp2_mul(t.y, E));
  t.z = fp2_mul(t.z, E);
}

struct line {
  fp2 a0, a1, a4;
};

DI fp12 line_mul_line(const line& a, const line& b) {
  fp2 t00 = fp2_mul(a.a0, b.a0), t11 = fp2_mul(a.a1, b.a1), t44 = fp2_mul(a.a4, b.a4);
  fp2 c01 = fp2_sub(fp2_sub(fp2_mul(fp2_add_lazy(a.a0, a.a1), fp2_add_lazy(b.a0, b.a1)), t00), t11);
  fp2 c11 = fp2_sub(fp2_sub(fp2_mul(fp2_add_lazy(a.a0, a.a4), fp2_add_lazy(b.a0, b.a4)), t00), t44);
  fp2 c12 = fp2_sub(fp2_sub(fp2_mul(fp2_add_lazy(a.a1, a.a4), fp2_add_lazy(b.a1, b.a4)), t11), t44);
  return {{fp2_add(t00, fp2_mul_xi(t44)), c01, t11}, {fp2_zero(), c11, c12}};
}

DI fp6 fp6_mul_by_12(const fp6& a, const fp2& b1, const fp2& b2) {
  fp2 t1 = fp2_mul(a.c1, b1), t2 = fp2_mul(a.c2, b2);
  fp2 m = fp2_sub(fp2_sub(fp2_mul(fp2_add_lazy(a.c1, a.c2), fp2_add_lazy(b1, b2)), t1), t2);
  return {fp2_mul_xi(m), fp2_add(fp2_mul(a.c0, b1), fp2_mul_xi(t2)), fp2_add(fp2_mul(a.c0, b2), t1)};
}

DI fp12 fp12_mul_by_line_pair(const fp12& f, const fp12& L) {
  fp6 t0 = fp6_mul(f.c0, L.c0);
  fp6 t1 = fp6_mul_by_12(f.c1, L.c1.c1, L.c1.c2);
  fp6 Ls = {L.c0.c0, fp2_add_lazy(L.c0.c1, L.c1.c1), fp2_add_lazy(L.c0.c2, L.c1.c2)};
  fp6 c1 = fp6_sub(fp6_sub(fp6_mul(fp6_add_lazy(f.c0, f.c1), Ls), t0), t1);
  return {fp6_add(t0, fp6_mul_v(t1)), c1};
}

DI line line_one() { return {fp2_one(), fp2_zero(), fp2_zero()}; }

DI fp12 miller_loop_2(const g1a (&P)[2], const g2a (&Q)[2], const bool (&active)[2]) {
  g2proj T[2];
#pragma unroll
  for (int k = 0; k < 2; k++) T[k] = {Q[k].x, Q[k].y, fp2_one()};
  fp12 f = fp12_one();
  bool first = true;
#pragma unroll 1
  for (int i = 62; i >= 0; i--) {
    if (!first) f = fp12_sqr(f);
    line l[2];
#pragma unroll
    for (int k = 0; k < 2; k++) {
      miller_dbl_step(T[k], l[k].a0, l[k].a1, l[k].a4, P[k].x, P[k].y);
      if (!active[k]) l[k] = line_one();
    }
    f = first ? line_mul_line(l[0], l[1]) : fp12_mul_by_line_pair(f, line_mul_line(l[0], l[1]));
    first = false;
    if ((BLS_X_ABS >> i) & 1ull) {
#pragma unroll
      for (int k = 0; k < 2; k++) {
        miller_add_step(T[k], Q[k], l[k].a0, l[k].a1, l[k].a4, P[k].x, P[k].y);
        if (!active[k]) l[k] = line_one();
      }
      f = fp12_mul_by_line_pair(f, line_mul_line(l[0], l[1]));
    }
  }
  return fp12_conj(f);
}

constexpr int MILLER_STEPS = 68;

template <typename LoadQ, typename Emit>
DI void miller_lines(const g1a& P, LoadQ load_q, Emit emit) {
  const g2a Q0 = load_q();
  g2proj T = {Q0.x, Q0.y, fp2_one()};
  int step = 0;
#pragma unroll 1
  for (int i = 62; i >= 0; i--) {
    line l;
    miller_dbl_step<false>(T, l.a0, l.a1, l.a4, P.x, P.y);
    emit(step++, l);
    if ((BLS_X_ABS >> i) & 1ull) {
      miller_add_step(T, load_q(), l.a0, l.a1, l.a4, P.x, P.y);
      emit(step++, l);
    }
  }
}

template <typename LoadLine>
DI fp12 miller_f_from_lines(LoadLine load) {
  fp12 f = fp12_one();
  int step = 0;
#pragma unroll 1
  for (int i = 62; i >= 0; i--) {
    if (i != 62) f = fp12_sqr(f);
    const fp12 L = line_mul_line(load(step, 0), load(step, 1));
    f = step == 0 ? L : fp12_mul_by_line_pair(f, L);
    step++;
    if ((BLS_X_ABS >> i) & 1ull) {
      f = fp12_mul_by_line_pair(f, line_mul_line(load(step, 0), load(step, 1)));
      step++;
    }
  }
  return fp12_conj(f);
}

template <int NP>
DI fp12 miller_loop_multi(const g1a (&P)[NP], const g2a (&Q)[NP], const bool (&active)[NP]) {
  g2proj T[NP];
#pragma unroll
  for (int k = 0; k < NP; k++) T[k] = {Q[k].x, Q[k].y, fp2_one()};
  fp12 f = fp12_one();
  bool first = true;
#pragma unroll 1
  for (int i = 62; i >= 0; i--) {
    if (!first) f = fp12_sqr(f);
#pragma unroll
    for (int k = 0; k < NP; k++) {
      fp2 l00, l01, l11;
      miller_dbl_step(T[k], l00, l01, l11, P[k].x, P[k].y);
      if (active[k]) f = fp12_mul_by_014(f, l00, l01, l11);
    }
    first = false;
    if ((BLS_X_ABS >> i) & 1ull) {
#pragma unroll
      for (int k = 0; k < NP; k++) {
        fp2 l00, l01, l11;
        miller_add_step(T[k], Q[k], l00, l01, l11, P[k].x, P[k].y);
        if (active[k]) f = fp12_mul_by_014(f, l00, l01, l11);
      }
    }
  }
  return fp12_conj(f);
}

DI fp12 fexp_easy(const fp12& f) {
  fp12 t = fp12_mul(fp12_conj(f), fp12_inv(f));
  return fp12_mul(fp12_frob2(t), t);
}

struct fexp_no_cube {
  DI void operator()(const fp12&) const {}
};

template <typename Load, typename Cube>
DI fp12 fp12_pow_x_abs_reload(Load load, Cube cube) {
  constexpr uint64_t NSQ = 1ull | (2ull << 6) | (3ull << 12) | (9ull << 18) | (32ull << 24) | (16ull << 30);
  fp12 r = load();
#pragma unroll 1
  for (int s = 0; s < 6; s++) {
    const int n = (int)((NSQ >> (6 * s)) & 63u);
#pragma unroll 1
    for (int k = 0; k < n; k++) r = fp12_cyclotomic_sqr(r);
    if (s < 5) r = fp12_mul(r, load());
    if (s == 0) cube(r);
  }
  return r;
}

template <int MODE, typename LX, typename LC, typename LG3, typename Cube>
DI fp12 fexp_step(LX lx, LC lc, LG3 lg3, Cube cube) {
  fp12 r = fp12_conj(fp12_pow_x_abs_reload(lx, cube));
  if (MODE == 0 || MODE == 1) return fp12_mul(r, fp12_conj(lx()));
  if (MODE == 2) return fp12_mul(r, fp12_frob(lx()));
  if (MODE == 3) return r;
  r = fp12_mul(r, lg3());
  return fp12_mul(r, fp12_frob4(lc()));
}

template <typename LX, typename LC, typename LG3>
DI bool fexp_step4_is_one(LX lx, LC lc, LG3 lg3) {
  const fp12 r = fp12_mul(fp12_conj(fp12_pow_x_abs_reload(lx, fexp_no_cube())), lg3());
  return fp12_eq(r, fp12_conj(fp12_frob4(lc()))) & !fp12_is_zero(r);
}

struct fexp_staged {
  fp12 g, g3, c, t;
};
DI fexp_staged fexp_stage_to_t(const fp12& f) {
  fexp_staged s;
  s.g = fexp_easy(f);
  auto none = [&]() { return s.g; };
  const fexp_no_cube nc;
  const fp12 a = fexp_step<0>([&]() { return s.g; }, none, none, [&](const fp12& v) { s.g3 = v; });
  const fp12 b = fexp_step<1>([&]() { return a; }, none, none, nc);
  s.c = fexp_step<2>([&]() { return b; }, none, none, nc);
  s.t = fexp_step<3>([&]() { return s.c; }, none, none, nc);
  return s;
}

DI fp12 final_exponentiation(const fp12& f) {
  const fexp_staged s = fexp_stage_to_t(f);
  return fexp_step<4>([&]() { return s.t; }, [&]() { return s.c; }, [&]() { return s.g3; }, fexp_no_cube());
}
DI bool final_exponentiation_is_one(const fp12& f) {
  const fexp_staged s = fexp_stage_to_t(f);
  return fexp_step4_is_one([&]() { return s.t; }, [&]() { return s.c; }, [&]() { return s.g3; });
}

}
```

drand_amd/csrc/threshold.cpp:

```cpp
#include <numeric>

#include "host_internal.h"

extern "C" int blsv_set_group(blsv_ctx* c, const uint8_t* commits48, size_t t, size_t n) {
  if (!c || !commits48 || t == 0 || t > 65536) return fail(c, BLSV_EINVAL, "set_group: bad arguments");
  (void)hipSetDevice(c->device);
  if (c->has_group && c->t == t && c->n == n && c->group_bytes.size() == t * 48 &&
      memcmp(c->group_bytes.data(), commits48, t * 48) == 0)
    return BLSV_OK;
  c->has_group = false;
  c->group_bytes.clear();
  std::vector<uint8_t> cls;
  int rc = decode_g1(c, commits48, t, c->commits, c->commit_inf, cls);
  if (rc) return rc;
  for (size_t i = 0; i < t; i++)
    if (cls[i]) return fail(c, BLSV_EINVAL, "set_group: commitment %zu rejected (class %d)", i, (int)cls[i]);
  c->pk_all_n = 0;
  c->pk_all_built = false;
  c->t = t;
  c->n = n;
  c->group_bytes.assign(commits48, commits48 + t * 48);
  c->has_group = true;
  return BLSV_OK;
}

static std::vector<uint32_t> identity(size_t m) {
  std::vector<uint32_t> v(m);
  std::iota(v.begin(), v.end(), 0u);
  return v;
}

static void pubpoly_eval(blsv_ctx* c, const uint32_t* d_idx, size_t cnt, DBuf& tab, DBuf& inf) {
  blsk::launch_pubpoly_eval(c->commits.as<uint32_t>(), c->commit_inf.as<uint8_t>(), (uint32_t)c->t, d_idx, cnt,
                            tab.as<uint32_t>(), inf.as<uint8_t>(), c->stream);
}

static int ensure_pk_table(blsv_ctx* c) {
  if (c->pk_all_built) return BLSV_OK;
  const size_t m = std::min(c->n, kPkTable);
  if (m) {
    const std::vector<uint32_t> ident = identity(m);
    HIPCHK(c, c->idx.ensure(m * 4));
    HIPCHK(c, c->pk_all.ensure(m * blsk::G1_WORDS * 4));
    HIPCHK(c, c->pk_all_inf.ensure(m));
    HIPCHK(c, hipMemcpyAsync(c->idx.p, ident.data(), m * 4, hipMemcpyHostToDevice, c->stream));
    pubpoly_eval(c, c->idx.as<uint32_t>(), m, c->pk_all, c->pk_all_inf);
    HIPCHK(c, hipGetLastError());
    HIPCHK(c, hipStreamSynchronize(c->stream));
  }
  c->pk_all_n = m;
  c->pk_all_built = true;
  return BLSV_OK;
}

static int partials_stage(blsv_ctx* c, const uint8_t* msg, size_t msg_len, const uint8_t* partials,
                          size_t partial_len, size_t k, std::vector<uint8_t>& cls, std::vector<uint32_t>& index,
                          const uint32_t* msg_lens = nullptr) {
  cls.assign(k, BLSV_REJ_OK);
  index.assign(k, 0);
  if (!c->has_group) return fail(c, BLSV_ENOGROUP, "partials: no group set");
  if (k > c->chunk) return fail(c, BLSV_EINVAL, "partials: more than the context chunk (%zu) in one call", c->chunk);
  share_indices(partials, partial_len, k, index);
  if (partial_len != 98) {
    cls.assign(k, partial_len < 2 ? BLSV_REJ_SHARE_INDEX : BLSV_REJ_LENGTH);
    return BLSV_OK;
  }
  int rc = ensure_pk_table(c);
  if (rc) return rc;
  rc = ensure_workspace(c, k);
  if (rc) return rc;
  if (k > c->cap) return fail(c, BLSV_EINVAL, "partials: more than the context chunk (%zu) in one call", c->cap);
  std::vector<uint32_t> lens(k, (uint32_t)msg_len);
  std::vector<uint8_t> packed;
  if (msg_lens) {
    rc = upload_messages(c, msg, msg_lens, k);
  } else {
    packed.reserve(k * msg_len);
    for (size_t i = 0; i < k; i++) packed.insert(packed.end(), msg, msg + msg_len);
    rc = upload_messages(c, packed.data(), lens.data(), k);
  }
  if (rc) return rc;
  HIPCHK(c, c->idx.ensure(k * 4));
  HIPCHK(c, h2d(c, c->idx.p, index.data(), k * 4));
  bool in_table = true;
  for (size_t i = 0; i < k; i++) in_table = in_table && index[i] < c->pk_all_n;
  std::vector<uint32_t> ident;
  PkSel pk{c->pk_all.as<uint32_t>(), c->pk_all_inf.as<uint8_t>(), c->idx.as<uint32_t>()};
  if (!in_table) {
    HIPCHK(c, c->pp_tab.ensure(k * blsk::G1_WORDS * 4));
    HIPCHK(c, c->pp_inf.ensure(k));
    HIPCHK(c, c->sel.ensure(k * 4));
    ident = identity(k);
    HIPCHK(c, h2d(c, c->sel.p, ident.data(), k * 4));
    pubpoly_eval(c, c->idx.as<uint32_t>(), k, c->pp_tab, c->pp_inf);
    pk = {c->pp_tab.as<uint32_t>(), c->pp_inf.as<uint8_t>(), c->sel.as<uint32_t>()};
  }
  HIPCHK(c, c->in_sigs.ensure(k * partial_len + 96));
  HIPCHK(c, h2d(c, c->in_sigs.p, partials, k * partial_len));
  const SigSrc sig{c->in_sigs.as<uint8_t>(), partial_len, 2};
  if (use_lat(c, k)) {
    StageTimer tm(c, ST_LAT, k, c->stream);
    lat_uploaded(c, sig, k, pk, c->cls.as<uint8_t>(), c->S.as<uint32_t>(), c->s_inf.as<uint8_t>(), c->stream);
    HIPCHK(c, hipGetLastError());
  } else {
    PassOut out;
    rc = ctx_outputs(c, k, false, out);
    if (rc) return rc;
    rc = run_passes(
        c, k, sig, pk, [&](size_t base, size_t cnt, hipStream_t st) { hash_uploaded(c, base, cnt, st); }, Tail(), out,
        c->stream);
    if (rc) return rc;
  }
  HIPCHK(c, download_sync(c, {{cls.data(), c->cls.p, k}}));
  return BLSV_OK;
}

static void put_verdicts(const std::vector<uint8_t>& cls, size_t lo, size_t k, uint8_t* ok, uint8_t* reject_class) {
  for (size_t i = 0; i < k; i++) {
    ok[i] = cls[lo + i] == BLSV_REJ_OK;
    if (reject_class) reject_class[i] = cls[lo + i];
  }
}

static int verify_partials(blsv_ctx* c, const uint8_t* msg, size_t msg_len, const uint32_t* msg_lens,
                           const uint8_t* partials, size_t partial_len, size_t k, uint8_t* ok, uint8_t* reject_class) {
  (void)hipSetDevice(c->device);
  std::vector<uint8_t> cls;
  std::vector<uint32_t> index;
  const int rc = partials_stage(c, msg, msg_len, partials, partial_len, k, cls, index, msg_lens);
  if (rc) return rc;
  put_verdicts(cls, 0, k, ok, reject_class);
  return BLSV_OK;
}

static int recover_from(blsv_ctx* c, const std::vector<uint8_t>& cls, const std::vector<uint32_t>& index, size_t lo,
                        size_t hi, size_t t, size_t n, uint8_t* out_sig96) {
  std::vector<uint32_t> sel, idx;
  if (!select_shares(cls, index, lo, hi, t, n, sel, idx))
    return fail(c, BLSV_ENOTENOUGH, "share: not enough good public shares to reconstruct secret commitment");
  HIPCHK(c, c->sel.ensure(t * 4));
  HIPCHK(c, c->idx.ensure(t * 4));
  HIPCHK(c, c->lambdas.ensure(t * 32));
  HIPCHK(c, c->scratch.ensure(t * 192 * 4));
  HIPCHK(c, c->out.ensure(96));
  HIPCHK(c, h2d(c, c->sel.p, sel.data(), t * 4));
  std::vector<uint32_t> lam(t * 8);
  host_lagrange(idx.data(), t, lam.data());
  HIPCHK(c, h2d(c, c->lambdas.p, lam.data(), t * 32));
  blsk::launch_lat_recover(c->S.as<uint32_t>(), cls.size(), c->s_inf.as<uint8_t>(), c->sel.as<uint32_t>(),
                           c->lambdas.as<uint32_t>(), (uint32_t)t, c->scratch.as<uint32_t>(), c->out.as<uint8_t>(),
                           c->stream);
  HIPCHK(c, hipGetLastError());
  HIPCHK(c, download_sync(c, {{out_sig96, c->out.p, 96}}));
  return BLSV_OK;
}

struct SpecRecover {
  bool launched = false;
  bool verified = false;
  std::vector<uint32_t> sel;
};

static int spec_recover_launch(blsv_ctx* c, int slot, const uint8_t* partials, size_t partial_len,
                               const std::vector<uint32_t>& index, size_t lo, size_t hi, size_t t, size_t n,
                               SpecRecover& sr, const uint8_t* vmsg = nullptr, size_t vmsg_len = 0) {
  sr.launched = false;
  sr.verified = false;
  std::vector<uint8_t> all_ok(index.size(), BLSV_REJ_OK);
  std::vector<uint32_t> idx;
  if (!select_shares(all_ok, index, lo, hi, t, n, sr.sel, idx)) return BLSV_OK;
  auto& sp = c->spec[slot];
  const size_t tt = sr.sel.size();
  const size_t v_off = tt * 96 + tt * 8 + 96, m_off = v_off + 64;
  const bool verify = vmsg != nullptr && vmsg_len <= kIoCap / 4;
  const size_t lam_off = (m_off + (verify ? vmsg_len + 64 : 0) + 7) & ~size_t(7);
  const size_t host_need = lam_off + tt * 32 + 64;
  if (sp.host.sz < host_need) {
    HIPCHK(c, hipStreamSynchronize(c->side));
    HIPCHK(c, hipStreamSynchronize(c->side2));
  }
  HIPCHK(c, sp.host.ensure(host_need));
  uint8_t* h_sig = sp.host.as<uint8_t>();
  uint32_t* h_idx = reinterpret_cast<uint32_t*>(h_sig + tt * 96);
  uint32_t* h_sel = h_idx + tt;
  uint32_t* h_lam = reinterpret_cast<uint32_t*>(h_sig + lam_off);
  for (size_t j = 0; j < tt; j++) {
    std::memcpy(h_sig + j * 96, partials + (size_t)sr.sel[j] * partial_len + 2, 96);
    h_idx[j] = idx[j];
    h_sel[j] = (uint32_t)j;
  }
  HIPCHK(c, sp.sig.ensure(tt * 96));
  HIPCHK(c, sp.S.ensure(tt * blsk::S_WORDS * 4));
  HIPCHK(c, sp.s_inf.ensure(tt));
  HIPCHK(c, sp.cls.ensure(tt));
  HIPCHK(c, sp.sel.ensure(tt * 4));
  HIPCHK(c, sp.lam.ensure(tt * 32));
  HIPCHK(c, sp.scratch.ensure(tt * 192 * 4));
  HIPCHK(c, sp.out.ensure(96));
  if (verify) {
    uint8_t* h_msg = h_sig + m_off;
    std::memcpy(h_msg, vmsg, vmsg_len);
    uint64_t* h_off = reinterpret_cast<uint64_t*>(h_msg + ((vmsg_len + 7) & ~size_t(7)));
    h_off[0] = 0;
    h_off[1] = vmsg_len;
    uint32_t* h_len = reinterpret_cast<uint32_t*>(h_off + 2);
    h_len[0] = (uint32_t)vmsg_len;
    HIPCHK(c, sp.vmsg.ensure(vmsg_len + 1));
    HIPCHK(c, sp.voff.ensure(16));
    HIPCHK(c, sp.vlen.ensure(4));
    HIPCHK(c, sp.vcls.ensure(64));
    HIPCHK(c, sp.hout.ensure(blsk::kLatHoutWords * 4));
    HIPCHK(c, sp.saff.ensure(blsk::kLatSaffWords * 4));
    if (vmsg_len) HIPCHK(c, hipMemcpyAsync(sp.vmsg.p, h_msg, vmsg_len, hipMemcpyHostToDevice, c->side2));
    HIPCHK(c, hipMemcpyAsync(sp.voff.p, h_off, 16, hipMemcpyHostToDevice, c->side2));
    HIPCHK(c, hipMemcpyAsync(sp.vlen.p, h_len, 4, hipMemcpyHostToDevice, c->side2));
    const PkSel pk = group_pk(c);
    blsk::launch_lat_hash_key(sp.vmsg.as<uint8_t>(), sp.voff.as<uint64_t>(), sp.vlen.as<uint32_t>(), pk.tab, pk.inf,
                              sp.hout.as<uint32_t>(), c->side2);
    HIPCHK(c, hipGetLastError());
    HIPCHK(c, hipEventRecord(c->hash_ev[slot], c->side2));
  }
  hipStream_t st = c->side;
  HIPCHK(c, hipMemcpyAsync(sp.sig.p, h_sig, tt * 96, hipMemcpyHostToDevice, st));
  HIPCHK(c, hipMemcpyAsync(sp.sel.p, h_sel, tt * 4, hipMemcpyHostToDevice, st));
  blsk::launch_lat_decode(sp.sig.as<uint8_t>(), 96, 0, tt, sp.S.as<uint32_t>(), sp.s_inf.as<uint8_t>(),
                          sp.cls.as<uint8_t>(), st);
  host_lagrange(h_idx, tt, h_lam);
  HIPCHK(c, hipMemcpyAsync(sp.lam.p, h_lam, tt * 32, hipMemcpyHostToDevice, st));
  blsk::launch_lat_recover(sp.S.as<uint32_t>(), tt, sp.s_inf.as<uint8_t>(), sp.sel.as<uint32_t>(),
                           sp.lam.as<uint32_t>(), (uint32_t)tt, sp.scratch.as<uint32_t>(), sp.out.as<uint8_t>(), st,
                           verify ? sp.saff.as<uint32_t>() : nullptr);
  HIPCHK(c, hipGetLastError());
  HIPCHK(c, hipMemcpyAsync(h_sig + tt * 96 + tt * 8, sp.out.p, 96, hipMemcpyDeviceToHost, st));
  if (verify) {
    HIPCHK(c, hipStreamWaitEvent(st, c->hash_ev[slot], 0));
    blsk::launch_lat_verify_pre(sp.hout.as<uint32_t>(), sp.saff.as<uint32_t>(), sp.vcls.as<uint8_t>(), st);
    HIPCHK(c, hipGetLastError());
    HIPCHK(c, hipMemcpyAsync(h_sig + v_off, sp.vcls.p, 1, hipMemcpyDeviceToHost, st));
    sr.verified = true;
  }
  sr.launched = true;
  return BLSV_OK;
}

static int spec_recover_finish(blsv_ctx* c, int slot, const SpecRecover& sr, const std::vector<uint8_t>& cls,
                               const std::vector<uint32_t>& index, size_t lo, size_t hi, size_t t, size_t n,
                               uint8_t* out_sig96, int* vcls = nullptr) {
  if (vcls) *vcls = -1;
  if (sr.launched) {
    HIPCHK(c, hipStreamSynchronize(c->side));
    std::vector<uint32_t> sel, idx;
    if (select_shares(cls, index, lo, hi, t, n, sel, idx) && sel == sr.sel) {
      const size_t tt = sr.sel.size();
      const uint8_t* h = c->spec[slot].host.as<uint8_t>();
      std::memcpy(out_sig96, h + tt * 96 + tt * 8, 96);
      if (vcls && sr.verified) *vcls = h[tt * 96 + tt * 8 + 96];
      c->spec_hits++;
      return BLSV_OK;
    }
    c->spec_misses++;
  }
  return recover_from(c, cls, index, lo, hi, t, n, out_sig96);
}

struct SideDrain {
  blsv_ctx* c;
  bool armed = false;
  ~SideDrain() {
    if (!armed) return;
    (void)hipStreamSynchronize(c->side);
    (void)hipStreamSynchronize(c->side2);
  }
};

static bool spec_applies(const blsv_ctx* c, size_t k, size_t partial_len) {
  return partial_len == 98 && c->has_group && k > 0 && k <= std::min(c->lat_max, c->chunk);
}

extern "C" {

int blsv_verify_partials(blsv_ctx* c, const uint8_t* msg, size_t msg_len, const uint8_t* partials, size_t partial_len,
                         size_t k, uint8_t* ok, uint8_t* reject_class) {
  if (!c) return BLSV_EINVAL;
  if ((k && (!partials || !ok)) || (msg_len && !msg)) return fail(c, BLSV_EINVAL, "verify_partials: null arguments");
  return verify_partials(c, msg, msg_len, nullptr, partials, partial_len, k, ok, reject_class);
}

int blsv_verify_partials_multi(blsv_ctx* c, const uint8_t* msgs, const uint32_t* msg_lens, const uint8_t* partials,
                               size_t partial_len, size_t k, uint8_t* ok, uint8_t* reject_class) {
  if (!c) return BLSV_EINVAL;
  if (k && (!partials || !ok || !msgs || !msg_lens)) return fail(c, BLSV_EINVAL, "verify_partials_multi: null arguments");
  return verify_partials(c, msgs, 0, msg_lens, partials, partial_len, k, ok, reject_class);
}

int blsv_recover(blsv_ctx* c, const uint8_t* msg, size_t msg_len, const uint8_t* partials, size_t partial_len,
                 size_t k, size_t t, size_t n, uint8_t* out_sig96) {
  if (!c) return BLSV_EINVAL;
  if (!out_sig96 || t == 0 || (k && !partials) || (msg_len && !msg)) return fail(c, BLSV_EINVAL, "recover: bad arguments");
  (void)hipSetDevice(c->device);
  std::vector<uint8_t> cls;
  std::vector<uint32_t> index;
  int rc = partials_stage(c, msg, msg_len, partials, partial_len, k, cls, index);
  if (rc) return rc;
  return recover_from(c, cls, index, 0, k, t, n, out_sig96);
}

int blsv_aggregate(blsv_ctx* c, const uint8_t* msg, size_t msg_len, const uint8_t* partials, size_t partial_len,
                   size_t k, size_t t, size_t n, uint8_t* ok, uint8_t* reject_class, uint8_t* out_sig96,
                   uint8_t* group_ok) {
  if (!c) return BLSV_EINVAL;
  if (!out_sig96 || !ok || !group_ok || t == 0 || (k && !partials) || (msg_len && !msg))
    return fail(c, BLSV_EINVAL, "aggregate: bad arguments");
  (void)hipSetDevice(c->device);
  std::vector<uint8_t> cls;
  std::vector<uint32_t> index;
  SpecRecover sr;
  SideDrain drain{c};
  if (spec_applies(c, k, partial_len)) {
    share_indices(partials, partial_len, k, index);
    drain.armed = true;
    int rc0 = spec_recover_launch(c, 0, partials, partial_len, index, 0, k, t, n, sr, msg, msg_len);
    if (rc0) return rc0;
  }
  int rc = partials_stage(c, msg, msg_len, partials, partial_len, k, cls, index);
  if (rc) return rc;
  put_verdicts(cls, 0, k, ok, reject_class);
  *group_ok = 0;
  int vcls = -1;
  rc = spec_recover_finish(c, 0, sr, cls, index, 0, k, t, n, out_sig96, &vcls);
  if (rc) return rc;
  if (vcls >= 0) {
    *group_ok = vcls == BLSV_REJ_OK;
    return BLSV_OK;
  }
  const uint32_t len = (uint32_t)msg_len;
  uint8_t bm = 0, cls1 = 0;
  uint64_t fb = 0;
  rc = blsv_verify_messages(c, nullptr, msg, &len, 1, out_sig96, &bm, &fb, &cls1);
  if (rc) return rc;
  *group_ok = bm & 1;
  return BLSV_OK;
}

int blsv_aggregate_round(blsv_ctx* c, const uint8_t* msg1, size_t msg1_len, const uint8_t* partials1, size_t k1,
                         const uint8_t* msg2, size_t msg2_len, const uint8_t* partials2, size_t k2,
                         size_t partial_len, size_t t, size_t n, uint8_t* ok1, uint8_t* ok2, uint8_t* sig1_96,
                         uint8_t* sig2_96, int32_t* status, uint8_t* v2_valid) {
  if (!c) return BLSV_EINVAL;
  if (!sig1_96 || !sig2_96 || !status || !v2_valid || t == 0 || (k1 && (!partials1 || !ok1)) ||
      (k2 && (!partials2 || !ok2 || !msg2)) || (msg1_len && !msg1))
    return fail(c, BLSV_EINVAL, "aggregate_round: bad arguments");
  (void)hipSetDevice(c->device);
  *status = BLSV_AGG_V1_RECOVER_FAIL;
  *v2_valid = 0;
  const size_t k = k1 + k2;
  std::vector<uint8_t> msgs, parts;
  std::vector<uint32_t> lens(k);
  msgs.reserve(k1 * msg1_len + k2 * msg2_len);
  parts.reserve(k * partial_len);
  for (size_t i = 0; i < k1; i++) {
    msgs.insert(msgs.end(), msg1, msg1 + msg1_len);
    lens[i] = (uint32_t)msg1_len;
  }
  for (size_t i = 0; i < k2; i++) {
    msgs.insert(msgs.end(), msg2, msg2 + msg2_len);
    lens[k1 + i] = (uint32_t)msg2_len;
  }
  if (k1) parts.insert(parts.end(), partials1, partials1 + k1 * partial_len);
  if (k2) parts.insert(parts.end(), partials2, partials2 + k2 * partial_len);
  std::vector<uint8_t> cls;
  std::vector<uint32_t> index;
  const bool try_v2 = k2 >= t;
  SpecRecover sr1, sr2;
  SideDrain drain{c};
  if (spec_applies(c, k, partial_len)) {
    share_indices(parts.data(), partial_len, k, index);
    drain.armed = true;
    int rc0 = spec_recover_launch(c, 0, parts.data(), partial_len, index, 0, k1, t, n, sr1, msg1 ? msg1 : parts.data(),
                                  msg1_len);
    if (!rc0 && try_v2)
      rc0 = spec_recover_launch(c, 1, parts.data(), partial_len, index, k1, k, t, n, sr2, msg2, msg2_len);
    if (rc0) return rc0;
  }
  int rc = partials_stage(c, msgs.data(), 0, parts.data(), partial_len, k, cls, index, lens.data());
  if (rc) return rc;
  put_verdicts(cls, 0, k1, ok1, nullptr);
  put_verdicts(cls, k1, k2, ok2, nullptr);
  int vc1 = -1, vc2 = -1;
  rc = spec_recover_finish(c, 0, sr1, cls, index, 0, k1, t, n, sig1_96, &vc1);
  if (rc == BLSV_ENOTENOUGH) return BLSV_OK;
  if (rc) return rc;
  bool v2_recovered = false;
  if (try_v2) {
    rc = spec_recover_finish(c, 1, sr2, cls, index, k1, k, t, n, sig2_96, &vc2);
    if (rc && rc != BLSV_ENOTENOUGH) return rc;
    v2_recovered = rc == BLSV_OK;
  }
  const uint32_t vlens[2] = {(uint32_t)msg1_len, (uint32_t)msg2_len};
  std::vector<uint8_t> vmsg(msg1, msg1 + msg1_len), vsig(sig1_96, sig1_96 + 96);
  if (v2_recovered) {
    vmsg.insert(vmsg.end(), msg2, msg2 + msg2_len);
    vsig.insert(vsig.end(), sig2_96, sig2_96 + 96);
  }
  uint8_t bm = 0, vcls[2] = {0, 0};
  uint64_t fb = 0;
  if (vc1 >= 0 && (!v2_recovered || vc2 >= 0)) {
    bm = (uint8_t)((vc1 == BLSV_REJ_OK) | ((v2_recovered && vc2 == BLSV_REJ_OK) << 1));
  } else {
    rc = blsv_verify_messages(c, nullptr, vmsg.data(), vlens, v2_recovered ? 2 : 1, vsig.data(), &bm, &fb, vcls);
    if (rc) return rc;
  }
  if (!(bm & 1)) {
    *status = BLSV_AGG_V1_INVALID;
    return BLSV_OK;
  }
  if (try_v2 && !v2_recovered) {
    *status = BLSV_AGG_V2_RECOVER_FAIL;
    return BLSV_OK;
  }
  *v2_valid = v2_recovered ? (uint8_t)((bm >> 1) & 1) : 0;
  *status = v2_recovered ? BLSV_AGG_OK_V2 : BLSV_AGG_OK;
  return BLSV_OK;
}

int blsv_sign(blsv_ctx* c, const uint8_t* sk32, int32_t index, const uint8_t* msgs, const uint32_t* msg_lens, size_t n,
              uint8_t* out) {
  if (!c) return BLSV_EINVAL;
  if (!sk32 || (n && (!msg_lens || !out)) || index > 65535) return fail(c, BLSV_EINVAL, "sign: bad arguments");
  if (n > kMaxChunk) return fail(c, BLSV_EINVAL, "sign: batch larger than %zu", kMaxChunk);
  (void)hipSetDevice(c->device);
  if (!n) return BLSV_OK;
  uint32_t sk[8];
  scalar_mod_r(sk32, sk);
  int rc = ensure_workspace(c, n);
  if (rc) return rc;
  rc = upload_messages(c, msgs, msg_lens, n);
  if (rc) return rc;
  const size_t stride = index >= 0 ? 98 : 96;
  HIPCHK(c, c->sk.ensure(32));
  HIPCHK(c, c->out.ensure(n * stride));
  HIPCHK(c, hipMemcpyAsync(c->sk.p, sk, 32, hipMemcpyHostToDevice, c->stream));
  (void)for_each_pass(c, n, [&](size_t base, size_t cnt) {
    hash_uploaded(c, base, cnt, c->stream);
    blsk::launch_sign(c->sk.as<uint32_t>(), index, c->H.as<uint32_t>(), c->h_inf.as<uint8_t>(), cnt,
                      c->out.as<uint8_t>() + base * stride, stride, c->stream);
    return BLSV_OK;
  });
  HIPCHK(c, hipGetLastError());
  HIPCHK(c, hipMemcpyAsync(out, c->out.p, n * stride, hipMemcpyDeviceToHost, c->stream));
  HIPCHK(c, hipStreamSynchronize(c->stream));
  return BLSV_OK;
}

}
```

drand_amd/csrc/verify.cpp:

```cpp
#include <sys/random.h>

#include <thread>

#include "host_internal.h"

static bool serial_stages() {
  static const bool on = [] {
    const char* e = getenv("BLSV_SERIAL_STAGES");
    return e && e[0] == '1';
  }();
  return on;
}

static void head_decompress(blsv_ctx* c, const SigSrc& sig, size_t base, size_t cnt, const Tail& tail, hipStream_t st) {
  const Staging w = staging(c);
  if (tail.fused_subgroup() && !blsk::g_generic_chains_all)
    blsk::launch_decompress_g2_only(sig.d, sig.stride, sig.offset, base, cnt, w.S, w.s_inf, w.cls, st);
  else
    blsk::launch_decompress_g2(sig.d, sig.stride, sig.offset, base, cnt, w.S, w.s_inf, w.cls, st);
}

int run_head(blsv_ctx* c, const SigSrc& sig, size_t base, size_t cnt, const Tail& tail, hipStream_t st,
             const HashFn& hash) {
  if (serial_stages()) {
    {
      StageTimer tm(c, ST_DECOMP, cnt, st);
      head_decompress(c, sig, base, cnt, tail, st);
    }
    StageTimer tm(c, ST_HASH, cnt, st);
    hash(base, cnt, st);
    return BLSV_OK;
  }
  HIPCHK(c, hipEventRecord(c->fork_ev, st));
  HIPCHK(c, hipStreamWaitEvent(c->side, c->fork_ev, 0));
  {
    StageTimer tm(c, ST_DECOMP, cnt, c->side);
    head_decompress(c, sig, base, cnt, tail, c->side);
  }
  HIPCHK(c, hipEventRecord(c->join_ev, c->side));
  {
    StageTimer tm(c, ST_HASH, cnt, st);
    hash(base, cnt, st);
  }
  HIPCHK(c, hipStreamWaitEvent(st, c->join_ev, 0));
  return BLSV_OK;
}

struct SplitDrain {
  blsv_ctx* c;
  bool armed = false;
  ~SplitDrain() {
    if (armed) (void)hipStreamSynchronize(c->side);
  }
};

static int pairing_check(blsv_ctx* c, const PkSel& pk, const uint32_t* H, const uint8_t* h_inf, const uint32_t* S,
                         const uint8_t* s_inf, uint8_t* cls, size_t cnt, bool check_subgroup, hipStream_t st) {
  const Staging w = staging(c);
  const size_t mn = serial_stages() || cnt > kLineSub ? cnt : tail_split_main(cnt, c->tail_q);
  if (mn == cnt) {
    {
      StageTimer tm(c, ST_MILLER, cnt, st);
      blsk::launch_miller(pk.tab, pk.inf, pk.idx, H, h_inf, S, s_inf, cls, cnt, w.F, w.LN, std::min(cnt, kLineSub),
                          w.FW, check_subgroup, st);
    }
    StageTimer tm(c, ST_FEXP, cnt, st);
    final_exp(c, cnt, cls, st);
    return BLSV_OK;
  }
  auto mark = [&](hipStream_t s) {
    hipEvent_t e = c->prof ? take_event(c) : nullptr;
    if (e) (void)hipEventRecord(e, s);
    return e;
  };
  auto keep = [&](ProfRec r) {
    if (!c->prof) return;
    if (!r.a2 || !r.b2) {
      for (hipEvent_t e : {r.a2, r.b2})
        if (e) c->event_pool.push_back(e);
      r.a2 = r.b2 = nullptr;
    }
    if (r.a && r.b) {
      c->recs.push_back(r);
    } else {
      for (hipEvent_t e : {r.a, r.b, r.a2, r.b2})
        if (e) c->event_pool.push_back(e);
    }
  };
  ProfRec rm{ST_MILLER, cnt, nullptr, nullptr}, rf{ST_FEXP, cnt, nullptr, nullptr};
  SplitDrain drain{c};
  const size_t rem = cnt - mn;
  rm.a = mark(st);
  blsk::launch_miller_lines(pk.tab, pk.inf, pk.idx, H, h_inf, S, s_inf, cls, cnt, 0, cnt, w.LN, cnt, check_subgroup, st);
  blsk::launch_miller_f(w.LN, cnt, cls, cnt, 0, mn, w.F, w.FW, false, st);
  rm.b = mark(st);
  int rc = BLSV_OK;
  auto chk = [&](hipError_t e, const char* what) {
    if (e != hipSuccess && rc == BLSV_OK) rc = fail(c, BLSV_EHIP, "%s: %s", what, hipGetErrorString(e));
    return e == hipSuccess;
  };
  if (chk(hipEventRecord(c->fork_ev, st), "split fork") && chk(hipStreamWaitEvent(c->side, c->fork_ev, 0), "split fork")) {
    drain.armed = true;
    rm.a2 = mark(c->side);
    blsk::launch_miller_f(w.LN, cnt, cls, cnt, mn, rem, w.F, nullptr, true, c->side);
    rm.b2 = mark(c->side);
    rf.a2 = mark(c->side);
    final_exp(c, cnt, mn, rem, cls, c->side);
    rf.b2 = mark(c->side);
    rf.a = mark(st);
    final_exp(c, cnt, 0, mn, cls, st);
    rf.b = mark(st);
    if (chk(hipEventRecord(c->join_ev, c->side), "split join") && chk(hipStreamWaitEvent(st, c->join_ev, 0), "split join"))
      drain.armed = false;
  }
  keep(rm);
  keep(rf);
  return rc;
}

static int finish_pass(blsv_ctx* c, size_t base, size_t cnt, const PassOut& out, hipStream_t st) {
  {
    StageTimer tm(c, ST_FINISH, cnt, st);
    blsk::launch_finish(c->cls.as<uint8_t>(), base, cnt, out.bitmap, out.first_bad, out.label0, st);
  }
  if (out.cls) HIPCHK(c, hipMemcpyAsync(out.cls + base, c->cls.p, cnt, hipMemcpyDeviceToDevice, st));
  HIPCHK(c, hipGetLastError());
  return BLSV_OK;
}

static int run_tail(blsv_ctx* c, size_t base, size_t cnt, const PkSel& pk, const PassOut& out, hipStream_t st) {
  const Staging w = staging(c);
  const int rc = pairing_check(c, pk, w.H, w.h_inf, w.S, w.s_inf, w.cls, cnt, true, st);
  return rc ? rc : finish_pass(c, base, cnt, out, st);
}


int rlc_draw_seed(blsv_ctx* c, uint32_t (&w)[8]) {
  uint8_t s[32];
  if (c->rlc.seed_pinned) {
    memcpy(s, c->rlc.seed, 32);
  } else {
    size_t got = 0;
    while (got < sizeof s) {
      const ssize_t r = getrandom(s + got, sizeof s - got, 0);
      if (r < 0 && errno == EINTR) continue;
      if (r <= 0) return fail(c, BLSV_EHIP, "rlc: getrandom failed: %s", strerror(errno));
      got += (size_t)r;
    }
  }
  for (int k = 0; k < 8; k++)
    w[k] = ((uint32_t)s[4 * k] << 24) | ((uint32_t)s[4 * k + 1] << 16) | ((uint32_t)s[4 * k + 2] << 8) | s[4 * k + 3];
  return BLSV_OK;
}

static size_t round64(size_t v) { return (std::max(v, size_t(1)) + 63) & ~size_t(63); }

int rlc_sums(blsv_ctx* c, size_t base, size_t cnt, const uint32_t (&seed)[8], hipStream_t st) {
  rlc_state& r = c->rlc;
  const Staging w = staging(c);
  const size_t ng = blsk::rlc_groups(cnt, r.group), cap = round64(ng);
  HIPCHK(c, r.part.ensure(2 * blsk::kRlcPartWords * blsk::rlc_lanes(cnt) * 4));
  HIPCHK(c, r.gH.ensure(cap * blsk::H_WORDS * 4));
  HIPCHK(c, r.gS.ensure(cap * blsk::S_WORDS * 4));
  HIPCHK(c, r.g_hinf.ensure(cap));
  HIPCHK(c, r.g_sinf.ensure(cap));
  HIPCHK(c, r.gcls.ensure(cap));
  StageTimer tm(c, ST_RLC, cnt, st);
  blsk::launch_rlc_sums(w.H, w.h_inf, w.S, w.s_inf, w.cls, cnt, base, seed, r.group, r.part.as<uint32_t>(),
                        r.gH.as<uint32_t>(), r.g_hinf.as<uint8_t>(), r.gS.as<uint32_t>(), r.g_sinf.as<uint8_t>(), st);
  return BLSV_OK;
}

static int run_tail_rlc(blsv_ctx* c, size_t base, size_t cnt, const uint32_t (&seed)[8], const PassOut& out,
                        hipStream_t st) {
  rlc_state& r = c->rlc;
  const Staging w = staging(c);
  const PkSel pk = group_pk(c);
  const size_t G = r.group, ng = blsk::rlc_groups(cnt, G);
  int rc = rlc_sums(c, base, cnt, seed, st);
  if (rc) return rc;
  HIPCHK(c, hipMemsetAsync(r.gcls.p, 0, ng, st));
  rc = pairing_check(c, pk, r.gH.as<uint32_t>(), r.g_hinf.as<uint8_t>(), r.gS.as<uint32_t>(), r.g_sinf.as<uint8_t>(),
                     r.gcls.as<uint8_t>(), ng, false, st);
  if (rc) return rc;
  HIPCHK(c, hipGetLastError());
  HIPCHK(c, r.host.ensure(kMaxChunk / kRlcGroupMin * 5 + 16));
  uint8_t* verdict = r.host.as<uint8_t>();
  HIPCHK(c, hipMemcpyAsync(verdict, r.gcls.p, ng, hipMemcpyDeviceToHost, st));
  HIPCHK(c, hipStreamSynchronize(st));
  uint32_t* fail_list = reinterpret_cast<uint32_t*>(verdict + ((ng + 7) & ~size_t(7)));
  size_t nf = 0;
  for (size_t g = 0; g < ng; g++)
    if (verdict[g] != BLSV_REJ_OK) fail_list[nf++] = (uint32_t)g;
  r.groups += ng;
  r.groups_failed += nf;
  if (nf) {
    const size_t m = rlc_failing_items(cnt, G, fail_list, nf), cap = round64(m);
    r.items_exact += m;
    HIPCHK(c, r.fail.ensure(nf * 4));
    HIPCHK(c, r.cH.ensure(cap * blsk::H_WORDS * 4));
    HIPCHK(c, r.cS.ensure(cap * blsk::S_WORDS * 4));
    HIPCHK(c, r.c_hinf.ensure(cap));
    HIPCHK(c, r.c_sinf.ensure(cap));
    HIPCHK(c, r.ccls.ensure(cap));
    HIPCHK(c, hipMemcpyAsync(r.fail.p, fail_list, nf * 4, hipMemcpyHostToDevice, st));
    {
      StageTimer tm(c, ST_RLC, m, st);
      blsk::launch_rlc_gather(r.fail.as<uint32_t>(), G, m, w.H, w.h_inf, w.S, w.s_inf, w.cls, cnt, r.cH.as<uint32_t>(),
                              r.c_hinf.as<uint8_t>(), r.cS.as<uint32_t>(), r.c_sinf.as<uint8_t>(), r.ccls.as<uint8_t>(),
                              st);
    }
    rc = pairing_check(c, pk, r.cH.as<uint32_t>(), r.c_hinf.as<uint8_t>(), r.cS.as<uint32_t>(), r.c_sinf.as<uint8_t>(),
                       r.ccls.as<uint8_t>(), m, false, st);
    if (rc) return rc;
    StageTimer tm(c, ST_RLC, m, st);
    blsk::launch_rlc_scatter(r.fail.as<uint32_t>(), G, m, r.ccls.as<uint8_t>(), w.cls, cnt, st);
  }
  return finish_pass(c, base, cnt, out, st);
}

int run_passes(blsv_ctx* c, size_t n, const SigSrc& sig, const PkSel& pk, const HashFn& hash, const Tail& tail,
               const PassOut& out, hipStream_t st) {
  return for_each_pass(c, n, [&](size_t base, size_t cnt) {
    const PkSel pass_pk{pk.tab, pk.inf, pk.idx ? pk.idx + base : nullptr};
    const int rc = run_head(c, sig, base, cnt, tail, st, hash);
    if (rc) return rc;
    return tail.randomized ? run_tail_rlc(c, base, cnt, tail.seed, out, st) : run_tail(c, base, cnt, pass_pk, out, st);
  });
}

int ctx_outputs(blsv_ctx* c, size_t n, bool with_cls, PassOut& out) {
  HIPCHK(c, c->bitmap.ensure((n + 63) / 64 * 8 + 8));
  HIPCHK(c, c->first_bad.ensure(8));
  HIPCHK(c, hipMemsetAsync(c->first_bad.p, 0xff, 8, c->stream));
  if (with_cls) HIPCHK(c, c->misc.ensure(n + 64));
  out = {c->bitmap.as<uint64_t>(), c->first_bad.as<unsigned long long>(), with_cls ? c->misc.as<uint8_t>() : nullptr, 0};
  return BLSV_OK;
}

using LatFn = std::function<void(uint8_t* cls)>;

static int verify_host(blsv_ctx* c, size_t n, const SigSrc& sig, const PkSel& pk, const HashFn& hash, const LatFn& lat,
                       bool randomized, uint64_t first_round, const uint64_t* rounds, uint8_t* ok_bitmap,
                       uint64_t* first_bad, uint8_t* reject_class) {
  auto put_first_bad = [&](uint64_t fb) {
    if (first_bad) *first_bad = fb == UINT64_MAX ? fb : rounds ? rounds[fb] : first_round + fb;
  };
  int rc = ensure_workspace(c, n);
  if (rc) return rc;
  if (use_lat(c, n)) {
    {
      StageTimer tm(c, ST_LAT, n, c->stream);
      lat(c->cls.as<uint8_t>());
    }
    HIPCHK(c, hipGetLastError());
    std::vector<uint8_t> own;
    uint8_t* cls = reject_class;
    if (!cls) {
      own.resize(n);
      cls = own.data();
    }
    HIPCHK(c, download_sync(c, {{cls, c->cls.p, n}}));
    put_first_bad(fold_classes(cls, n, ok_bitmap));
    return BLSV_OK;
  }
  Tail tail;
  tail.randomized = randomized;
  if (randomized && (rc = rlc_draw_seed(c, tail.seed))) return rc;
  PassOut out;
  rc = ctx_outputs(c, n, reject_class != nullptr, out);
  if (rc) return rc;
  rc = run_passes(c, n, sig, pk, hash, tail, out, c->stream);
  if (rc) return rc;
  const size_t words = (n + 63) / 64;
  std::vector<uint64_t> w(words + 1, 0);
  uint64_t fb = UINT64_MAX;
  HIPCHK(c, download_sync(c, {{w.data(), c->bitmap.p, words * 8},
                              {&fb, c->first_bad.p, 8},
                              {reject_class, c->misc.p, reject_class ? n : 0}}));
  if (ok_bitmap) bitmap_words_to_bytes(w.data(), n, ok_bitmap);
  put_first_bad(fb);
  return BLSV_OK;
}

int decode_g1(blsv_ctx* c, const uint8_t* pk48, size_t cnt, DBuf& tab, DBuf& inf, std::vector<uint8_t>& cls) {
  HIPCHK(c, tab.ensure(cnt * blsk::G1_WORDS * 4));
  HIPCHK(c, inf.ensure(cnt));
  HIPCHK(c, c->g1_cls.ensure(cnt));
  HIPCHK(c, c->misc.ensure(cnt * 48));
  HIPCHK(c, hipMemcpyAsync(c->misc.p, pk48, cnt * 48, hipMemcpyHostToDevice, c->stream));
  blsk::launch_decompress_g1(c->misc.as<uint8_t>(), cnt, tab.as<uint32_t>(), inf.as<uint8_t>(),
                             c->g1_cls.as<uint8_t>(), c->stream);
  HIPCHK(c, hipGetLastError());
  cls.assign(cnt, 0);
  HIPCHK(c, hipMemcpyAsync(cls.data(), c->g1_cls.p, cnt, hipMemcpyDeviceToHost, c->stream));
  HIPCHK(c, hipStreamSynchronize(c->stream));
  return BLSV_OK;
}

int upload_messages(blsv_ctx* c, const uint8_t* msgs, const uint32_t* msg_lens, size_t n) {
  std::vector<uint64_t> off(n + 1, 0);
  for (size_t i = 0; i < n; i++) off[i + 1] = off[i] + msg_lens[i];
  if (off[n] && !msgs) return fail(c, BLSV_EINVAL, "messages: %llu message bytes but no buffer",
                                   (unsigned long long)off[n]);
  HIPCHK(c, c->in_msgs.ensure(off[n] + 1));
  HIPCHK(c, c->in_off.ensure((n + 1) * 8));
  HIPCHK(c, c->in_len.ensure(n * 4 + 4));
  const size_t staged_max = kIoCap / 4;
  HIPCHK(c, h2d(c, c->in_msgs.p, msgs, off[n]));
  HIPCHK(c, h2d(c, c->in_off.p, off.data(), (n + 1) * 8));
  HIPCHK(c, h2d(c, c->in_len.p, msg_lens, n * 4));
  if ((n + 1) * 8 > staged_max) HIPCHK(c, hipStreamSynchronize(c->stream));
  return BLSV_OK;
}

int svc_verify_mixed(blsv_ctx* c, size_t n, const uint8_t* msgs, const uint64_t* off, const uint32_t* lens,
                     const uint8_t* sigs96, const uint32_t* idx, const uint32_t* d_tab, const uint8_t* d_tab_inf,
                     uint8_t* cls_out) {
  if (!n) return BLSV_OK;
  if (n > kMaxChunk) return fail(c, BLSV_EINVAL, "service batch larger than %zu", kMaxChunk);
  (void)hipSetDevice(c->device);
  int rc = ensure_workspace(c, std::min(n, c->chunk));
  if (rc) return rc;
  const size_t mbytes = off[n];
  const SvcLayout l = svc_layout(n, mbytes);
  HIPCHK(c, c->pin.ensure(std::max(l.total, n + 8)));
  uint8_t* h = c->pin.as<uint8_t>();
  memcpy(h, off, (n + 1) * 8);
  memcpy(h + l.o_len, lens, n * 4);
  memcpy(h + l.o_idx, idx, n * 4);
  memcpy(h + l.o_sig, sigs96, n * 96);
  if (mbytes) memcpy(h + l.o_msg, msgs, mbytes);
  HIPCHK(c, c->arena.ensure(l.total));
  HIPCHK(c, c->misc.ensure(n + 64));
  HIPCHK(c, hipMemcpyAsync(c->arena.p, h, l.total, hipMemcpyHostToDevice, c->stream));
  uint8_t* d = c->arena.as<uint8_t>();
  const uint64_t* d_off = reinterpret_cast<const uint64_t*>(d);
  const uint32_t* d_len = reinterpret_cast<const uint32_t*>(d + l.o_len);
  const uint8_t* d_msg = d + l.o_msg;
  const SigSrc sig{d + l.o_sig, 96, 0};
  const PkSel pk{d_tab, d_tab_inf, reinterpret_cast<const uint32_t*>(d + l.o_idx)};
  if (use_lat(c, n)) {
    blsk::launch_lat_messages(d_msg, d_off, d_len, sig.d, 96, 0, n, pk.tab, pk.inf, pk.idx, c->misc.as<uint8_t>(),
                              nullptr, nullptr, c->stream);
  } else {
    PassOut out;
    rc = ctx_outputs(c, n, true, out);
    if (rc) return rc;
    rc = run_passes(
        c, n, sig, pk,
        [&](size_t base, size_t cnt, hipStream_t st) { hash_messages(c, d_msg, d_off, d_len, base, cnt, st); }, Tail(),
        out, c->stream);
    if (rc) return rc;
  }
  HIPCHK(c, hipGetLastError());
  HIPCHK(c, hipMemcpyAsync(h, c->misc.p, n, hipMemcpyDeviceToHost, c->stream));
  HIPCHK(c, hipStreamSynchronize(c->stream));
  memcpy(cls_out, h, n);
  return BLSV_OK;
}

int stage_chain(blsv_ctx* c, uint64_t first_round, const uint8_t* prevs, size_t prev0_len, bool prev_rows,
                const uint8_t* sigs96, size_t n, blsk::ChainedSrc& src) {
  HIPCHK(c, c->in_sigs.ensure(n * 96 + 96));
  HIPCHK(c, c->seeds.ensure(prev_rows ? n * 96 + 96 : 96));
  if (n) {
    HIPCHK(c, h2d(c, c->in_sigs.p, sigs96, n * 96));
    HIPCHK(c, h2d(c, c->seeds.p, prevs, prev_rows ? n * 96 : prev0_len));
  }
  src = {c->in_sigs.as<uint8_t>(), c->seeds.as<uint8_t>(), first_round, prev_rows ? 1 : std::max<uint64_t>(n, 1),
         (uint32_t)prev0_len};
  return BLSV_OK;
}

static int chained_host(blsv_ctx* c, const char* name, bool prev_rows, bool randomized, uint64_t first_round,
                        const uint8_t* prevs, size_t prev0_len, const uint8_t* sigs96, size_t n, uint8_t* ok_bitmap,
                        uint64_t* first_bad, uint8_t* reject_class) {
  if (!c->has_group) return fail(c, BLSV_ENOGROUP, "%s: no group key set", name);
  if (n && (!sigs96 || !prevs || (prev0_len != 32 && prev0_len != 96)))
    return fail(c, BLSV_EINVAL, "%s: %s must be 32 or 96 bytes", name, prev_rows ? "row 0's prev" : "prev0");
  if (n > SIZE_MAX / 96 - 1) return fail(c, BLSV_EINVAL, "%s: %zu rounds overflow the byte count", name, n);
  (void)hipSetDevice(c->device);
  blsk::ChainedSrc src;
  const int rc = stage_chain(c, first_round, prevs, prev0_len, prev_rows, sigs96, n, src);
  if (rc) return rc;
  const PkSel pk = group_pk(c);
  return verify_host(
      c, n, {src.sigs, 96, 0}, pk, [&](size_t base, size_t cnt, hipStream_t st) { hash_chained(c, src, base, cnt, st); },
      [&](uint8_t* cls) { blsk::launch_lat_chained(src, 0, n, pk.tab, pk.inf, cls, c->stream); }, randomized,
      first_round, nullptr, ok_bitmap, first_bad, reject_class);
}

static int unchained_host(blsv_ctx* c, const char* name, bool randomized, const uint64_t* rounds, uint64_t first_round,
                          const uint8_t* sigs96, size_t n, uint8_t* ok_bitmap, uint64_t* first_bad,
                          uint8_t* reject_class) {
  if (!c->has_group) return fail(c, BLSV_ENOGROUP, "%s: no group key set", name);
  if (n && !sigs96) return fail(c, BLSV_EINVAL, "%s: null signatures", name);
  (void)hipSetDevice(c->device);
  HIPCHK(c, c->in_sigs.ensure(n * 96 + 96));
  if (n) HIPCHK(c, h2d(c, c->in_sigs.p, sigs96, n * 96));
  const uint64_t* d_rounds = nullptr;
  if (rounds && n) {
    HIPCHK(c, c->in_rounds.ensure(n * 8));
    HIPCHK(c, h2d(c, c->in_rounds.p, rounds, n * 8));
    d_rounds = c->in_rounds.as<uint64_t>();
  }
  const PkSel pk = group_pk(c);
  const SigSrc sig{c->in_sigs.as<uint8_t>(), 96, 0};
  return verify_host(
      c, n, sig, pk,
      [&](size_t base, size_t cnt, hipStream_t st) {
        const Staging w = staging(c);
        blsk::launch_hash_unchained(d_rounds, first_round, base, cnt, w.H, w.h_inf, w.HQ, st);
      },
      [&](uint8_t* cls) { blsk::launch_lat_unchained(d_rounds, first_round, sig.d, 0, n, pk.tab, pk.inf, cls, c->stream); },
      randomized, first_round, rounds, ok_bitmap, first_bad, reject_class);
}

static int run_lat(blsv_ctx* c, size_t n, const LatFn& lat, const PassOut& out, hipStream_t st) {
  {
    StageTimer tm(c, ST_LAT, n, st);
    lat(c->cls.as<uint8_t>());
  }
  blsk::launch_finish(c->cls.as<uint8_t>(), 0, n, out.bitmap, out.first_bad, out.label0, st);
  if (out.cls) HIPCHK(c, hipMemcpyAsync(out.cls, c->cls.p, n, hipMemcpyDeviceToDevice, st));
  HIPCHK(c, hipGetLastError());
  return BLSV_OK;
}

static int chained_dev(blsv_ctx* c, const char* name, bool randomized, uint64_t first_round, uint64_t seg_len,
                       uint64_t seg_phase, const uint8_t* d_seeds96, size_t seed0_len, const uint8_t* d_sigs96, size_t n,
                       uint64_t* d_bitmap, uint64_t* d_first_bad, uint8_t* d_reject_class, void* stream) {
  if (!c->has_group) return fail(c, BLSV_ENOGROUP, "%s: no group key set", name);
  if (n && (!d_seeds96 || !d_sigs96 || !d_bitmap || !d_first_bad || (seed0_len != 32 && seed0_len != 96)))
    return fail(c, BLSV_EINVAL, "%s: bad arguments", name);
  if (seg_phase && (!seg_len || seg_phase >= seg_len))
    return fail(c, BLSV_EINVAL, "%s: seg_phase must be < seg_len", name);
  (void)hipSetDevice(c->device);
  hipStream_t st = stream ? (hipStream_t)stream : c->stream;
  Tail tail;
  tail.randomized = randomized;
  int rc = randomized ? rlc_draw_seed(c, tail.seed) : BLSV_OK;
  if (rc) return rc;
  HIPCHK(c, hipMemsetAsync(d_first_bad, 0xff, 8, st));
  rc = ensure_workspace(c, n);
  if (rc) return rc;
  const blsk::ChainedSrc src{d_sigs96,           d_seeds96, first_round, seg_len ? seg_len : std::max<uint64_t>(n, 1),
                             (uint32_t)seed0_len, seg_phase};
  const PkSel pk = group_pk(c);
  const PassOut out{d_bitmap, (unsigned long long*)d_first_bad, d_reject_class, first_round};
  if (use_lat(c, n))
    return run_lat(c, n, [&](uint8_t* cls) { blsk::launch_lat_chained(src, 0, n, pk.tab, pk.inf, cls, st); }, out, st);
  return run_passes(
      c, n, {d_sigs96, 96, 0}, pk, [&](size_t base, size_t cnt, hipStream_t s) { hash_chained(c, src, base, cnt, s); },
      tail, out, st);
}

extern "C" {

int blsv_verify_chained(blsv_ctx* c, uint64_t first_round, const uint8_t* prev0, size_t prev0_len,
                        const uint8_t* sigs96, size_t n, uint8_t* ok_bitmap, uint64_t* first_bad,
                        uint8_t* reject_class) {
  if (!c) return BLSV_EINVAL;
  return chained_host(c, "verify_chained", false, false, first_round, prev0, prev0_len, sigs96, n, ok_bitmap, first_bad,
                      reject_class);
}

int blsv_verify_prevs(blsv_ctx* c, uint64_t first_round, const uint8_t* prevs96, size_t prev0_len,
                      const uint8_t* sigs96, size_t n, uint8_t* ok_bitmap, uint64_t* first_bad,
                      uint8_t* reject_class) {
  if (!c) return BLSV_EINVAL;
  return chained_host(c, "verify_prevs", true, false, first_round, prevs96, prev0_len, sigs96, n, ok_bitmap, first_bad,
                      reject_class);
}

int blsv_verify_chained_rlc(blsv_ctx* c, uint64_t first_round, const uint8_t* prev0, size_t prev0_len,
                            const uint8_t* sigs96, size_t n, uint8_t* ok_bitmap, uint64_t* first_bad,
                            uint8_t* reject_class) {
  if (!c) return BLSV_EINVAL;
  const bool rlc = use_rlc(c, n);
  return chained_host(c, rlc ? "verify_chained_rlc" : "verify_chained", false, rlc, first_round, prev0, prev0_len,
                      sigs96, n, ok_bitmap, first_bad, reject_class);
}

int blsv_verify_unchained(blsv_ctx* c, const uint64_t* rounds, uint64_t first_round, const uint8_t* sigs96, size_t n,
                          uint8_t* ok_bitmap, uint64_t* first_bad, uint8_t* reject_class) {
  if (!c) return BLSV_EINVAL;
  return unchained_host(c, "verify_unchained", false, rounds, first_round, sigs96, n, ok_bitmap, first_bad,
                        reject_class);
}

int blsv_verify_unchained_rlc(blsv_ctx* c, const uint64_t* rounds, uint64_t first_round, const uint8_t* sigs96,
                              size_t n, uint8_t* ok_bitmap, uint64_t* first_bad, uint8_t* reject_class) {
  if (!c) return BLSV_EINVAL;
  const bool rlc = use_rlc(c, n);
  return unchained_host(c, rlc ? "verify_unchained_rlc" : "verify_unchained", rlc, rounds, first_round, sigs96, n,
                        ok_bitmap, first_bad, reject_class);
}

int blsv_verify_chained_dev(blsv_ctx* c, uint64_t first_round, uint64_t seg_len, uint64_t seg_phase,
                            const uint8_t* d_seeds96, size_t seed0_len, const uint8_t* d_sigs96, size_t n,
                            uint64_t* d_bitmap, uint64_t* d_first_bad, uint8_t* d_reject_class, void* stream) {
  if (!c) return BLSV_EINVAL;
  return chained_dev(c, "verify_chained_dev", false, first_round, seg_len, seg_phase, d_seeds96, seed0_len, d_sigs96, n,
                     d_bitmap, d_first_bad, d_reject_class, stream);
}

int blsv_verify_chained_rlc_dev(blsv_ctx* c, uint64_t first_round, uint64_t seg_len, uint64_t seg_phase,
                                const uint8_t* d_seeds96, size_t seed0_len, const uint8_t* d_sigs96, size_t n,
                                uint64_t* d_bitmap, uint64_t* d_first_bad, uint8_t* d_reject_class, void* stream) {
  if (!c) return BLSV_EINVAL;
  const bool rlc = use_rlc(c, n);
  return chained_dev(c, rlc ? "verify_chained_rlc_dev" : "verify_chained_dev", rlc, first_round, seg_len, seg_phase,
                     d_seeds96, seed0_len, d_sigs96, n, d_bitmap, d_first_bad, d_reject_class, stream);
}

int blsv_verify_chained_multi(blsv_ctx* const* ctxs, size_t n_ctx, const size_t* shard_counts, uint64_t first_round,
                              const uint8_t* prev0, size_t prev0_len, const uint8_t* sigs96, size_t n,
                              uint8_t* ok_bitmap, uint64_t* first_bad, uint8_t* reject_class) {
  if (!ctxs || n_ctx == 0) return BLSV_EINVAL;
  for (size_t k = 0; k < n_ctx; k++) {
    if (!ctxs[k]) return BLSV_EINVAL;
    for (size_t j = 0; j < k; j++)
      if (ctxs[j] == ctxs[k]) return fail(ctxs[k], BLSV_EINVAL, "verify_chained_multi: context %zu repeated", k);
  }
  blsv_ctx* c0 = ctxs[0];
  for (size_t k = 0; k < n_ctx; k++) {
    if (!ctxs[k]->has_group) return fail(ctxs[k], BLSV_ENOGROUP, "verify_chained_multi: context %zu has no group", k);
    if (ctxs[k]->group_bytes != c0->group_bytes)
      return fail(ctxs[k], BLSV_EINVAL, "verify_chained_multi: context %zu holds another group", k);
  }
  if (n && (!sigs96 || !prev0 || (prev0_len != 32 && prev0_len != 96)))
    return fail(c0, BLSV_EINVAL, "verify_chained_multi: prev0 must be 32 or 96 bytes");
  std::vector<size_t> cnt(n_ctx), start(n_ctx);
  size_t sum = 0;
  for (size_t k = 0; k < n_ctx; k++) {
    cnt[k] = shard_counts ? shard_counts[k] : n / n_ctx + (k < n % n_ctx ? 1 : 0);
    start[k] = sum;
    sum += cnt[k];
  }
  if (sum != n) return fail(c0, BLSV_EINVAL, "verify_chained_multi: shard counts sum to %zu, not %zu", sum, n);
  std::vector<std::vector<uint8_t>> bms(n_ctx);
  std::vector<uint64_t> fbs(n_ctx, UINT64_MAX);
  std::vector<int> rcs(n_ctx, BLSV_OK);
  auto shard = [&](size_t k) {
    if (!cnt[k]) return;
    bms[k].assign((cnt[k] + 7) / 8, 0);
    const bool head = start[k] == 0;
    const uint8_t* halo = head ? prev0 : sigs96 + (start[k] - 1) * 96;
    rcs[k] = blsv_verify_chained(ctxs[k], first_round + start[k], halo, head ? prev0_len : 96, sigs96 + start[k] * 96,
                                 cnt[k], bms[k].data(), &fbs[k], reject_class ? reject_class + start[k] : nullptr);
  };
  std::vector<std::thread> th;
  for (size_t k = 1; k < n_ctx; k++)
    if (cnt[k]) th.emplace_back(shard, k);
  shard(0);
  for (auto& t : th) t.join();
  for (size_t k = 0; k < n_ctx; k++)
    if (rcs[k]) return rcs[k];
  uint64_t fb = UINT64_MAX;
  for (size_t k = 0; k < n_ctx; k++) fb = std::min(fb, fbs[k]);
  if (first_bad) *first_bad = fb;
  if (ok_bitmap && n) {
    memset(ok_bitmap, 0, (n + 7) / 8);
    for (size_t k = 0; k < n_ctx; k++)
      if (cnt[k]) or_bits_at(ok_bitmap, bms[k].data(), cnt[k], start[k]);
  }
  return BLSV_OK;
}

int blsv_verify_messages(blsv_ctx* c, const uint8_t* pk48, const uint8_t* msgs, const uint32_t* msg_lens, size_t n,
                         const uint8_t* sigs96, uint8_t* ok_bitmap, uint64_t* first_bad, uint8_t* reject_class) {
  if (!c) return BLSV_EINVAL;
  if (n && (!msg_lens || !sigs96)) return fail(c, BLSV_EINVAL, "verify_messages: null arguments");
  (void)hipSetDevice(c->device);
  PkSel pk;
  if (pk48) {
    if (!c->pk_cache_valid || memcmp(c->pk_cache, pk48, 48) != 0) {
      std::vector<uint8_t> cls;
      int rc = decode_g1(c, pk48, 1, c->pk_tab, c->pk_inf, cls);
      if (rc) return rc;
      if (cls[0]) return fail(c, BLSV_EINVAL, "verify_messages: public key rejected (class %d)", (int)cls[0]);
      memcpy(c->pk_cache, pk48, 48);
      c->pk_cache_valid = true;
    }
    pk = {c->pk_tab.as<uint32_t>(), c->pk_inf.as<uint8_t>(), nullptr};
  } else {
    if (!c->has_group) return fail(c, BLSV_ENOGROUP, "verify_messages: no group key set");
    pk = group_pk(c);
  }
  if (n > kMaxChunk) return fail(c, BLSV_EINVAL, "verify_messages: batch larger than %zu", kMaxChunk);
  int rc = upload_messages(c, msgs, msg_lens, n);
  if (rc) return rc;
  HIPCHK(c, c->in_sigs.ensure(n * 96 + 96));
  if (n) HIPCHK(c, h2d(c, c->in_sigs.p, sigs96, n * 96));
  const SigSrc sig{c->in_sigs.as<uint8_t>(), 96, 0};
  return verify_host(
      c, n, sig, pk, [&](size_t base, size_t cnt, hipStream_t st) { hash_uploaded(c, base, cnt, st); },
      [&](uint8_t* cls) { lat_uploaded(c, sig, n, pk, cls, nullptr, nullptr, c->stream); }, false, 0, nullptr, ok_bitmap,
      first_bad, reject_class);
}

int blsv_generate_chained_dev(blsv_ctx* c, const uint8_t* sk32, uint64_t first_round, uint64_t seg_len,
                              const uint8_t* d_seeds96, size_t seed0_len, uint8_t* d_sigs96, size_t n, void* stream) {
  if (!c) return BLSV_EINVAL;
  if (!sk32 || (n && (!d_seeds96 || !d_sigs96)) || (seed0_len != 32 && seed0_len != 96))
    return fail(c, BLSV_EINVAL, "generate_chained_dev: bad arguments");
  (void)hipSetDevice(c->device);
  hipStream_t st = stream ? (hipStream_t)stream : c->stream;
  uint32_t sk[8];
  scalar_mod_r(sk32, sk);
  HIPCHK(c, c->sk.ensure(32));
  HIPCHK(c, hipMemcpyAsync(c->sk.p, sk, 32, hipMemcpyHostToDevice, st));
  blsk::ChainedSrc src{d_sigs96, d_seeds96, first_round, seg_len ? seg_len : std::max<uint64_t>(n, 1),
                       (uint32_t)seed0_len};
  blsk::launch_gen_chained(c->sk.as<uint32_t>(), src, n, d_sigs96, st);
  HIPCHK(c, hipGetLastError());
  HIPCHK(c, hipStreamSynchronize(st));
  return BLSV_OK;
}

size_t blsv_set_rlc_group(blsv_ctx* c, size_t g) {
  if (!c) return 0;
  const size_t prev = c->rlc.group;
  size_t v = kRlcGroupMin;
  while (v * 2 <= g && v < kRlcGroupMax) v *= 2;
  c->rlc.group = v;
  return prev;
}

int blsv_rlc_stats(blsv_ctx* c, uint64_t* groups, uint64_t* groups_failed, uint64_t* items_exact) {
  if (!c) return BLSV_EINVAL;
  if (groups) *groups = c->rlc.groups;
  if (groups_failed) *groups_failed = c->rlc.groups_failed;
  if (items_exact) *items_exact = c->rlc.items_exact;
  return BLSV_OK;
}

}
```

Measured before the change: 2.523 million beacons/s.

## Use precomputed per-key scaling constants to cheapen Miller loop line steps

When the public key is fixed (single key or group key), a one-time kernel precomputes scaling constants (alpha, gamma, 12/yP^2, inverses, and so on) for the G1 point. A new scaled variant of the Miller doubling and addition steps uses these constants, so the line evaluations need fewer Fp2-by-Fp multiplications per step. The -g1 side uses compile-time constants and the subgroup check uses adjusted psi constants. This adds a sqrt and two inversions per key decode and more template variants, and correctness depends on the scaled coordinates being consistent with what the downstream F accumulation expects.

```diff
diff --git a/drand_amd/csrc/bls_constants.h b/drand_amd/csrc/bls_constants.h
--- a/drand_amd/csrc/bls_constants.h
+++ b/drand_amd/csrc/bls_constants.h
@@ -84,6 +84,20 @@
     {0x0u, 0x0u, 0x0u, 0x0u, 0x0u, 0x0u, 0x0u, 0x0u, 0x0u, 0x0u, 0x0u, 0x0u}};
 static constexpr uint32_t PSI2_KY[2][12] = {{0xfcb7adf3u, 0xa026ffffu, 0x4433fd4eu, 0xbcbf320u, 0x54a7e9b2u, 0x2fca331du, 0x19759edfu, 0x5ac6b042u, 0xb439151cu, 0xa35691dcu, 0x3c85e56du, 0x14896b90u},
     {0x0u, 0x0u, 0x0u, 0x0u, 0x0u, 0x0u, 0x0u, 0x0u, 0x0u, 0x0u, 0x0u, 0x0u}};
+static constexpr uint32_t G1N_LSC[8][12] = {
+    {0x66365f45u, 0x30dde520u, 0x27ce1134u, 0xde09b7a5u, 0x30044543u, 0x27e39507u, 0xc4db25b1u, 0xa0bbaf62u, 0xedd92ffcu, 0x1dbbaa05u, 0xd5a0d0dau, 0x73b138fu},
+    {0x18b6e47cu, 0x9af82af3u, 0x41127125u, 0xc38ce4efu, 0xc109b9d1u, 0x68c05d98u, 0x17fae9ddu, 0xd9b60eeeu, 0x7df09147u, 0xebfbbee9u, 0x55213dbu, 0xc3d21d2u},
+    {0x740de640u, 0x1975e929u, 0x7e0b7d87u, 0xe127b79eu, 0x4b45d9f6u, 0x4db1e4edu, 0xdc20b8e0u, 0x2b7f6f87u, 0x58d210au, 0x6a8236c6u, 0x46eaed3au, 0xf3d07f0u},
+    {0x9d81ab5fu, 0x8a5cb30bu, 0x998175d5u, 0x97ce09b4u, 0x742b16ddu, 0x8d73364fu, 0x2e468d9du, 0xaf18735du, 0x494342c0u, 0xf949d192u, 0xa979e2fbu, 0x13efb38eu},
+    {0x707017beu, 0x323d9deeu, 0x2fb1f21u, 0xa1593075u, 0x3779c552u, 0xf5461199u, 0xeca38c39u, 0xaddbdf12u, 0xbce81553u, 0x447d3eb4u, 0x4b2ea673u, 0xbe57359u},
+    {0x18b6e47cu, 0x9af82af3u, 0x41127125u, 0xc38ce4efu, 0xc109b9d1u, 0x68c05d98u, 0x17fae9ddu, 0xd9b60eeeu, 0x7df09147u, 0xebfbbee9u, 0x55213dbu, 0xc3d21d2u},
+    {0x8db6cb3du, 0xae653d80u, 0xcc371e6fu, 0xc07efbb3u, 0x3246689eu, 0x39045738u, 0x4bf86995u, 0x4afb3f5bu, 0x212fd5f1u, 0xb320d19eu, 0x4abc5e4du, 0x129f5890u},
+    {1u, 0u, 0u, 0u, 0u, 0u, 0u, 0u, 0u, 0u, 0u, 0u}};
+static constexpr bool G1N_LSC_SNEG = true;
+static constexpr uint32_t PSI_KX_G1N[2][12] = {{0x0u, 0x0u, 0x0u, 0x0u, 0x0u, 0x0u, 0x0u, 0x0u, 0x0u, 0x0u, 0x0u, 0x0u},
+    {0xddf5056fu, 0xd88c8030u, 0xc0c79274u, 0xa3f31ee0u, 0xb4300049u, 0x4a49abf2u, 0x5d9fccdau, 0x184f2398u, 0xfa55549u, 0x70045e27u, 0xfb555b9fu, 0xfbd1873u}};
+static constexpr uint32_t PSI_KY_G1N[2][12] = {{0x7860b0cfu, 0xb24fa32bu, 0x347d4cd8u, 0xeefbe820u, 0xe40a82f8u, 0x8cc80f22u, 0xa6629480u, 0x5262dfd0u, 0x329ab466u, 0x574fb413u, 0xb488f11au, 0x376d61cu},
+    {0x879ef9dcu, 0x7af5cd4u, 0x7cd6b327u, 0x2fb017deu, 0x12a6732bu, 0xda68c37eu, 0x4d227e3eu, 0x12146bb4u, 0x10b0f871u, 0xf3cbf3a3u, 0x84f6f57fu, 0x168a3bcdu}};
 static constexpr uint32_t FROB1_GAMMA[6][2][12] = {
     {{0x347fcb8u, 0x19d80000u, 0x6d2002b1u, 0x12e00cdeu, 0xa2090c72u, 0x37669f83u, 0xda0f73e0u, 0x9b09b42u, 0x8f1297bbu, 0xa7c515d9u, 0xfcfa012cu, 0x577a659u},
      {0x0u, 0x0u, 0x0u, 0x0u, 0x0u, 0x0u, 0x0u, 0x0u, 0x0u, 0x0u, 0x0u, 0x0u}},
diff --git a/drand_amd/csrc/engine_ctx.h b/drand_amd/csrc/engine_ctx.h
--- a/drand_amd/csrc/engine_ctx.h
+++ b/drand_amd/csrc/engine_ctx.h
@@ -302,11 +302,12 @@
   bool has_group = false;
   size_t t = 0, n = 0;
   DBuf commits, commit_inf;
+  DBuf commit_sc;
   std::vector<uint8_t> group_bytes;
   DBuf pk_all, pk_all_inf;
   size_t pk_all_n = 0;
   bool pk_all_built = false;
-  DBuf pk_tab, pk_inf;
+  DBuf pk_tab, pk_inf, pk_sc;
   uint8_t pk_cache[48];
   bool pk_cache_valid = false;
   size_t cap = 0;
diff --git a/drand_amd/csrc/gen_constants.py b/drand_amd/csrc/gen_constants.py
--- a/drand_amd/csrc/gen_constants.py
+++ b/drand_amd/csrc/gen_constants.py
@@ -206,6 +206,22 @@
     ky2 = m2((ky[0], (-ky[1]) % P), ky)
     w(c_fp2("PSI2_KX", kx2))
     w(c_fp2("PSI2_KY", ky2))
+    xP, yP = G1_X, (-G1_Y) % P
+    s = 1 if pow(3 * xP % P, (P - 1) // 2, P) == 1 else -1
+    a2 = s * 3 * xP % P
+    alpha = pow(a2, (P + 1) // 4, P)
+    assert alpha * alpha % P == a2
+    gamma = -s * yP % P
+    ginv = pow(gamma, P - 2, P)
+    lsc = [alpha, gamma, 12 * pow(yP * yP, P - 2, P) % P, ginv, alpha * xP % P, yP, alpha * a2 * ginv % P]
+    rows = ["{" + ", ".join(hex(x) + "u" for x in limbs(mont(v))) + "}" for v in lsc]
+    rows.append("{" + ", ".join(["1u" if s < 0 else "0u"] + ["0u"] * 11) + "}")
+    w("// -g1's constants for the scaled Miller steps: alpha, gamma, 12/yP^2, 1/gamma, alpha xP, yP, alpha^3/gamma, s == -1")
+    w("static constexpr uint32_t G1N_LSC[8][12] = {\n    " + ",\n    ".join(rows) + "};")
+    w(f"static constexpr bool G1N_LSC_SNEG = {'true' if s < 0 else 'false'};")
+    ag = alpha * ginv % P
+    w(c_fp2("PSI_KX_G1N", (kx[0] * ag % P, kx[1] * ag % P)))
+    w(c_fp2("PSI_KY_G1N", (ky[0] * ginv % P, ky[1] * ginv % P)))
     g1 = pow2(XI, (P - 1) // 6)
     g2 = pow2(XI, (P * P - 1) // 6)
     g1p = [(1, 0)]
diff --git a/drand_amd/csrc/host_internal.h b/drand_amd/csrc/host_internal.h
--- a/drand_amd/csrc/host_internal.h
+++ b/drand_amd/csrc/host_internal.h
@@ -53,8 +53,11 @@
   const uint32_t* tab;
   const uint8_t* inf;
   const uint32_t* idx;
+  const uint32_t* sc;
 };
-inline PkSel group_pk(const blsv_ctx* c) { return {c->commits.as<uint32_t>(), c->commit_inf.as<uint8_t>(), nullptr}; }
+inline PkSel group_pk(const blsv_ctx* c) {
+  return {c->commits.as<uint32_t>(), c->commit_inf.as<uint8_t>(), nullptr, c->commit_sc.as<uint32_t>()};
+}
 
 inline void hash_chained(blsv_ctx* c, const blsk::ChainedSrc& src, size_t base, size_t cnt, hipStream_t st) {
   const Staging w = staging(c);
@@ -117,7 +120,8 @@
 
 int stage_chain(blsv_ctx* c, uint64_t first_round, const uint8_t* prevs, size_t prev0_len, bool prev_rows,
                 const uint8_t* sigs96, size_t n, blsk::ChainedSrc& src);
-int decode_g1(blsv_ctx* c, const uint8_t* pk48, size_t cnt, DBuf& tab, DBuf& inf, std::vector<uint8_t>& cls);
+int decode_g1(blsv_ctx* c, const uint8_t* pk48, size_t cnt, DBuf& tab, DBuf& inf, std::vector<uint8_t>& cls,
+              DBuf* sc = nullptr);
 int upload_messages(blsv_ctx* c, const uint8_t* msgs, const uint32_t* msg_lens, size_t n);
 
 struct MaskTail {
diff --git a/drand_amd/csrc/k_group.hip b/drand_amd/csrc/k_group.hip
--- a/drand_amd/csrc/k_group.hip
+++ b/drand_amd/csrc/k_group.hip
@@ -106,6 +106,15 @@
   cls[i] = c;
 }
 
+static_assert(MILLER_SC_WORDS == LSC_WORDS, "kernels.h MILLER_SC_WORDS");
+__global__ void __launch_bounds__(TPB) k_g1_line_consts(const uint32_t* tab, uint32_t* sc) {
+  if (blockIdx.x | threadIdx.x) return;
+  fp k[LSC_SLOTS];
+  miller_scale_consts(ld_g1(tab, 0), k);
+  for (int s = 0; s < LSC_SLOTS; s++)
+    for (int w = 0; w < 12; w++) sc[12 * s + w] = k[s].l[w];
+}
+
 __global__ void __launch_bounds__(TPB) k_pubpoly_eval(const uint32_t* commits, const uint8_t* commit_inf, uint32_t t,
                                                       const uint32_t* idx, size_t cnt, uint32_t* out_tab,
                                                       uint8_t* out_inf) {
@@ -137,6 +146,10 @@
   hipLaunchKernelGGL(k_decompress_g1, dim3(grid_for(cnt)), dim3(TPB), 0, st, in, cnt, tab, inf, cls);
 }
 
+void launch_g1_line_consts(const uint32_t* tab, uint32_t* sc, hipStream_t st) {
+  hipLaunchKernelGGL(k_g1_line_consts, dim3(1), dim3(TPB), 0, st, tab, sc);
+}
+
 void launch_pubpoly_eval(const uint32_t* commits, const uint8_t* commit_inf, uint32_t t, const uint32_t* idx,
                          size_t cnt, uint32_t* out_tab, uint8_t* out_inf, hipStream_t st) {
   if (!cnt) return;
diff --git a/drand_amd/csrc/k_miller.hip b/drand_amd/csrc/k_miller.hip
--- a/drand_amd/csrc/k_miller.hip
+++ b/drand_amd/csrc/k_miller.hip
@@ -7,10 +7,10 @@
 namespace blsk {
 
 DI int line_slot(int step, int k) { return (step * 2 + k) * 6; }
-template <bool CHECK>
+template <bool CHECK, bool SCALED>
 BLS_KERNEL(BLS_WPE_LINES)
-k_miller_lines(const uint32_t* pk_tab, const uint8_t* pk_inf, const uint32_t* pk_idx, const uint32_t* H,
-               const uint8_t* h_inf, const uint32_t* S, const uint8_t* s_inf,
+k_miller_lines(const uint32_t* pk_tab, const uint8_t* pk_inf, const uint32_t* pk_idx, const uint32_t* pk_sc,
+               const uint32_t* H, const uint8_t* h_inf, const uint32_t* S, const uint8_t* s_inf,
                std::conditional_t<CHECK, uint8_t*, const uint8_t*> cls, size_t cnt, size_t base, size_t m, size_t sub,
                uint32_t* LN) {
   const int k = (int)(blockIdx.x & 1u);
@@ -51,24 +51,41 @@
     auto put = [&](int c, const fp2& v) { st_fp2<BLS_LN_AUX_ST>(LN, sub, i, line_slot(step, k) + 2 * c, v); };
     auto xp = [&]() { return pcoord(0); };
     auto yp = [&]() { return pcoord(1); };
+    auto pc = [&](int c) {
+      size_t o = (size_t)12 * c;
+      asm volatile("" : "+v"(o));
+      fp v;
+#pragma unroll
+      for (int w = 0; w < 12; w++) v.l[w] = pk_sc[o + w];
+      return k == 0 ? v : fp_load_const(G1N_LSC[c]);
+    };
+    bool sneg = false;
+    if constexpr (SCALED) sneg = k == 0 ? pk_sc[12 * LSC_SNEG] != 0 : G1N_LSC_SNEG;
     const g2proj_lds T{g_ml_T + threadIdx.x};
     {
       const g2a Q0 = load_q();
-      T.set(0, Q0.x);
       T.set(1, Q0.y);
-      T.set(2, fp2_one());
+      if constexpr (SCALED) {
+        T.set(0, fp2_mul_fp_inl(Q0.x, pc(LSC_ALPHA)));
+        T.set(2, fp2{pc(LSC_GAMMA), fp_zero()});
+      } else {
+        T.set(0, Q0.x);
+        T.set(2, fp2_one());
+      }
     }
 #pragma unroll 1
     for (int b = 62; b >= 0; b--) {
-      miller_dbl_step_ts(T, put, xp, yp);
+      if constexpr (SCALED) miller_dbl_step_scaled_ts(T, put, pc, sneg);
+      else miller_dbl_step_ts(T, put, xp, yp);
       step++;
       if ((BLS_X_ABS >> b) & 1ull) {
-        miller_add_step_ts(T, load_q, put, xp, yp);
+        if constexpr (SCALED) miller_add_step_scaled_ts(T, load_q, put, pc);
+        else miller_add_step_ts(T, load_q, put, xp, yp);
         step++;
       }
     }
     if constexpr (CHECK) {
-      if (k == 1 && !miller_t_in_subgroup(T, load_q)) {
+      if (k == 1 && !(SCALED ? miller_t_in_subgroup_scaled(T, load_q) : miller_t_in_subgroup(T, load_q))) {
         size_t j = g;
         asm volatile("" : "+v"(j));
         cls[j] = REJ_NOT_IN_SUBGROUP;
@@ -266,16 +283,24 @@
   return true;
 }
 
-void launch_miller_lines(const uint32_t* pk_tab, const uint8_t* pk_inf, const uint32_t* pk_idx, const uint32_t* H,
-                         const uint8_t* h_inf, const uint32_t* S, const uint8_t* s_inf, uint8_t* cls, size_t cnt,
-                         size_t base, size_t m, uint32_t* LN, size_t sub, bool check_subgroup, hipStream_t st) {
+template <bool CHECK, bool SCALED>
+static void launch_lines_as(const uint32_t* pk_tab, const uint8_t* pk_inf, const uint32_t* pk_idx,
+                            const uint32_t* pk_sc, const uint32_t* H, const uint8_t* h_inf, const uint32_t* S,
+                            const uint8_t* s_inf, uint8_t* cls, size_t cnt, size_t base, size_t m, uint32_t* LN,
+                            size_t sub, hipStream_t st) {
+  using cls_t = std::conditional_t<CHECK, uint8_t*, const uint8_t*>;
+  hipLaunchKernelGGL((k_miller_lines<CHECK, SCALED>), dim3(2 * grid_for(m)), dim3(TPB), 0, st, pk_tab, pk_inf, pk_idx,
+                     pk_sc, H, h_inf, S, s_inf, (cls_t)cls, cnt, base, m, sub, LN);
+}
+void launch_miller_lines(const uint32_t* pk_tab, const uint8_t* pk_inf, const uint32_t* pk_idx, const uint32_t* pk_sc,
+                         const uint32_t* H, const uint8_t* h_inf, const uint32_t* S, const uint8_t* s_inf, uint8_t* cls,
+                         size_t cnt, size_t base, size_t m, uint32_t* LN, size_t sub, bool check_subgroup,
+                         hipStream_t st) {
   if (!m) return;
-  if (check_subgroup)
-    hipLaunchKernelGGL(k_miller_lines<true>, dim3(2 * grid_for(m)), dim3(TPB), 0, st, pk_tab, pk_inf, pk_idx, H, h_inf,
-                       S, s_inf, cls, cnt, base, m, sub, LN);
-  else
-    hipLaunchKernelGGL(k_miller_lines<false>, dim3(2 * grid_for(m)), dim3(TPB), 0, st, pk_tab, pk_inf, pk_idx, H,
-                       h_inf, S, s_inf, (const uint8_t*)cls, cnt, base, m, sub, LN);
+  const bool scaled = !pk_idx && pk_sc;
+  auto go = check_subgroup ? (scaled ? launch_lines_as<true, true> : launch_lines_as<true, false>)
+                           : (scaled ? launch_lines_as<false, true> : launch_lines_as<false, false>);
+  go(pk_tab, pk_inf, pk_idx, pk_sc, H, h_inf, S, s_inf, cls, cnt, base, m, LN, sub, st);
 }
 
 void launch_miller_f(const uint32_t* LN, size_t sub, const uint8_t* cls, size_t cnt, size_t base, size_t m,
@@ -290,13 +315,15 @@
   }
 }
 
-void launch_miller(const uint32_t* pk_tab, const uint8_t* pk_inf, const uint32_t* pk_idx, const uint32_t* H,
-                   const uint8_t* h_inf, const uint32_t* S, const uint8_t* s_inf, uint8_t* cls, size_t cnt,
-                   uint32_t* F, uint32_t* LN, size_t sub, uint32_t* park, bool check_subgroup, hipStream_t st) {
+void launch_miller(const uint32_t* pk_tab, const uint8_t* pk_inf, const uint32_t* pk_idx, const uint32_t* pk_sc,
+                   const uint32_t* H, const uint8_t* h_inf, const uint32_t* S, const uint8_t* s_inf, uint8_t* cls,
+                   size_t cnt, uint32_t* F, uint32_t* LN, size_t sub, uint32_t* park, bool check_subgroup,
+                   hipStream_t st) {
   if (!cnt) return;
   for (size_t b = 0; b < cnt; b += sub) {
     const size_t m = cnt - b < sub ? cnt - b : sub;
-    launch_miller_lines(pk_tab, pk_inf, pk_idx, H, h_inf, S, s_inf, cls, cnt, b, m, LN, sub, check_subgroup, st);
+    launch_miller_lines(pk_tab, pk_inf, pk_idx, pk_sc, H, h_inf, S, s_inf, cls, cnt, b, m, LN, sub, check_subgroup,
+                        st);
     launch_miller_f(LN, sub, cls, cnt, b, m, F, park, false, st);
   }
 }
diff --git a/drand_amd/csrc/kernels.h b/drand_amd/csrc/kernels.h
--- a/drand_amd/csrc/kernels.h
+++ b/drand_amd/csrc/kernels.h
@@ -29,12 +29,14 @@
 void launch_decompress_g2(const uint8_t* sigs, size_t stride, size_t offset, size_t base, size_t cnt, uint32_t* S,
                           uint8_t* s_inf, uint8_t* cls, hipStream_t st);
 constexpr int MILLER_LINE_WORDS = 68 * 2 * 6 * 12;
-void launch_miller(const uint32_t* pk_tab, const uint8_t* pk_inf, const uint32_t* pk_idx, const uint32_t* H,
-                   const uint8_t* h_inf, const uint32_t* S, const uint8_t* s_inf, uint8_t* cls, size_t cnt,
-                   uint32_t* F, uint32_t* LN, size_t sub, uint32_t* park, bool check_subgroup, hipStream_t st);
-void launch_miller_lines(const uint32_t* pk_tab, const uint8_t* pk_inf, const uint32_t* pk_idx, const uint32_t* H,
-                         const uint8_t* h_inf, const uint32_t* S, const uint8_t* s_inf, uint8_t* cls, size_t cnt,
-                         size_t base, size_t m, uint32_t* LN, size_t sub, bool check_subgroup, hipStream_t st);
+void launch_miller(const uint32_t* pk_tab, const uint8_t* pk_inf, const uint32_t* pk_idx, const uint32_t* pk_sc,
+                   const uint32_t* H, const uint8_t* h_inf, const uint32_t* S, const uint8_t* s_inf, uint8_t* cls,
+                   size_t cnt, uint32_t* F, uint32_t* LN, size_t sub, uint32_t* park, bool check_subgroup,
+                   hipStream_t st);
+void launch_miller_lines(const uint32_t* pk_tab, const uint8_t* pk_inf, const uint32_t* pk_idx, const uint32_t* pk_sc,
+                         const uint32_t* H, const uint8_t* h_inf, const uint32_t* S, const uint8_t* s_inf, uint8_t* cls,
+                         size_t cnt, size_t base, size_t m, uint32_t* LN, size_t sub, bool check_subgroup,
+                         hipStream_t st);
 void launch_miller_f(const uint32_t* LN, size_t sub, const uint8_t* cls, size_t cnt, size_t base, size_t m,
                      uint32_t* F, uint32_t* park, bool single_lane, hipStream_t st);
 constexpr size_t TRI_PARK_WORDS(size_t items) { return 48 * 64 * ((items + 20) / 21); }
@@ -125,6 +127,8 @@
                       const uint8_t* scalars, size_t n, uint8_t* us, uint8_t* gts, uint8_t* ok, hipStream_t st);
 
 void launch_decompress_g1(const uint8_t* in, size_t cnt, uint32_t* tab, uint8_t* inf, uint8_t* cls, hipStream_t st);
+constexpr int MILLER_SC_WORDS = 8 * 12;
+void launch_g1_line_consts(const uint32_t* tab, uint32_t* sc, hipStream_t st);
 void launch_pubpoly_eval(const uint32_t* commits, const uint8_t* commit_inf, uint32_t t, const uint32_t* idx,
                          size_t cnt, uint32_t* out_tab, uint8_t* out_inf, hipStream_t st);
 void launch_lat_tauth_open(const uint8_t* sigs, const uint32_t* sig_of, const uint8_t* us, const uint8_t* vs,
diff --git a/drand_amd/csrc/pairing.h b/drand_amd/csrc/pairing.h
--- a/drand_amd/csrc/pairing.h
+++ b/drand_amd/csrc/pairing.h
@@ -108,21 +108,114 @@
   t.set(2, fp2_mul_inl(t.get(2), E));
 }
 
+enum { LSC_ALPHA = 0, LSC_GAMMA, LSC_KZ, LSC_GINV, LSC_AXP, LSC_YP, LSC_A3G, LSC_SNEG, LSC_SLOTS };
+constexpr int LSC_WORDS = LSC_SLOTS * 12;
+DI void miller_scale_consts(const g1a& P, fp (&k)[LSC_SLOTS]) {
+  k[LSC_ALPHA] = fp_sqrt_cand(fp_mul3(P.x));
+  const fp a2 = fp_sqr(k[LSC_ALPHA]);
+  const bool sneg = !fp_eq(a2, fp_mul3(P.x));
+  k[LSC_GAMMA] = sneg ? P.y : fp_neg(P.y);
+  k[LSC_KZ] = fp_mul(fp_mul4(fp_mul3(fp_one())), fp_inv(fp_sqr(P.y)));
+  k[LSC_GINV] = fp_inv(k[LSC_GAMMA]);
+  k[LSC_AXP] = fp_mul(k[LSC_ALPHA], P.x);
+  k[LSC_YP] = P.y;
+  k[LSC_A3G] = fp_mul(fp_mul(k[LSC_ALPHA], a2), k[LSC_GINV]);
+  k[LSC_SNEG] = fp_zero();
+  k[LSC_SNEG].l[0] = sneg;
+}
+template <typename TS, typename Put, typename PC>
+DI void miller_dbl_step_scaled_ts(const TS& t, Put put, PC pc, bool sneg) {
+  const fp2 B = fp2_sqr_inl(t.get(1));
+  BLS_SCHED_FENCE();
+  const fp2 C = fp2_sqr_inl(t.get(2));
+  BLS_SCHED_FENCE();
+  const fp2 H = fp2_sub(fp2_sqr_inl(fp2_add_lazy(t.get(1), t.get(2))), fp2_add(B, C));
+  BLS_SCHED_FENCE();
+  put(2, H);
+  const fp2 E = fp2_mul_xi(fp2_mul_fp_inl(C, pc(LSC_KZ)));
+  BLS_SCHED_FENCE();
+  t.set(2, fp2_mul_inl_k<0>(B, H));
+  BLS_SCHED_FENCE();
+  const fp2 F = fp2_mul3(E);
+  const fp2 G = fp2_half(fp2_add(B, F));
+  put(0, fp2_sub(fp2_select(sneg, B, E), fp2_select(sneg, E, B)));
+  const fp2 BF = fp2_sub(B, F);
+  const fp2 A = fp2_half(fp2_mul_inl_k<1>(t.get(0), t.get(1)));
+  BLS_SCHED_FENCE();
+  put(1, fp2_sqr_inl(t.get(0)));
+  BLS_SCHED_FENCE();
+  t.set(0, fp2_mul_inl(A, BF));
+  BLS_SCHED_FENCE();
+  const fp2 G2 = fp2_sqr_inl(G);
+  BLS_SCHED_FENCE();
+  t.set(1, fp2_sub(G2, fp2_mul3(fp2_sqr_inl(E))));
+}
+
+template <typename TS, typename Put, typename Q, typename PC>
+DI void miller_add_step_scaled_ts(const TS& t, Q qload, Put put, PC pc) {
+  fp2 theta, delta;
+  {
+    fp2 ax2;
+    {
+      const fp2 Z = fp2_mul_fp_inl(t.get(2), pc(LSC_GINV));
+      BLS_SCHED_FENCE();
+      theta = fp2_sub(t.get(1), fp2_mul_inl(qload().y, Z));
+      BLS_SCHED_FENCE();
+      ax2 = fp2_mul_fp_inl(qload().x, pc(LSC_ALPHA));
+      BLS_SCHED_FENCE();
+      delta = fp2_sub(t.get(0), fp2_mul_inl(ax2, Z));
+      BLS_SCHED_FENCE();
+    }
+    const fp2 u = fp2_mul_inl(theta, ax2);
+    BLS_SCHED_FENCE();
+    put(0, fp2_sub(u, fp2_mul_inl(delta, qload().y)));
+    BLS_SCHED_FENCE();
+  }
+  put(1, fp2_neg(fp2_mul_fp_inl(theta, pc(LSC_AXP))));
+  BLS_SCHED_FENCE();
+  put(2, fp2_mul_fp_inl(delta, pc(LSC_YP)));
+  BLS_SCHED_FENCE();
+  const fp2 C = fp2_sqr_inl(theta);
+  BLS_SCHED_FENCE();
+  const fp2 D = fp2_sqr_inl(delta);
+  BLS_SCHED_FENCE();
+  const fp2 E = fp2_mul_inl(D, delta);
+  BLS_SCHED_FENCE();
+  const fp2 F = fp2_mul_inl(fp2_mul_fp_inl(t.get(2), pc(LSC_A3G)), C);
+  BLS_SCHED_FENCE();
+  const fp2 G = fp2_mul_inl(t.get(0), D);
+  BLS_SCHED_FENCE();
+  const fp2 H = fp2_sub(fp2_add(E, F), fp2_dbl(G));
+  t.set(0, fp2_mul_inl(delta, H));
+  BLS_SCHED_FENCE();
+  t.set(1, fp2_sub(fp2_mul_inl(theta, fp2_sub(G, H)), fp2_mul_inl(t.get(1), E)));
+  BLS_SCHED_FENCE();
+  t.set(2, fp2_mul_inl(t.get(2), E));
+}
+
+template <typename TS, typename Q>
+DI bool miller_t_in_subgroup_k(const TS& t, Q qload, const uint32_t (&kx)[2][12], const uint32_t (&ky)[2][12]) {
+  bool ok = !fp2_is_zero(t.get(2));
+  {
+    const fp2 px = fp2_mul_inl(fp2_conj(qload().x), fp2_load_const(kx));
+    BLS_SCHED_FENCE();
+    ok &= fp2_eq(t.get(0), fp2_mul_inl(px, t.get(2)));
+  }
+  BLS_SCHED_FENCE();
+  {
+    const fp2 py = fp2_mul_inl(fp2_conj(qload().y), fp2_load_const(ky));
+    BLS_SCHED_FENCE();
+    ok &= fp2_eq(fp2_neg(t.get(1)), fp2_mul_inl(py, t.get(2)));
+  }
+  return ok;
+}
 template <typename TS, typename Q>
 DI bool miller_t_in_subgroup(const TS& t, Q qload) {
-  bool ok = !fp2_is_zero(t.get(2));
-  {
-    const fp2 px = fp2_mul_inl(fp2_conj(qload().x), fp2_load_const(PSI_KX));
-    BLS_SCHED_FENCE();
-    ok &= fp2_eq(t.get(0), fp2_mul_inl(px, t.get(2)));
-  }
-  BLS_SCHED_FENCE();
-  {
-    const fp2 py = fp2_mul_inl(fp2_conj(qload().y), fp2_load_const(PSI_KY));
-    BLS_SCHED_FENCE();
-    ok &= fp2_eq(fp2_neg(t.get(1)), fp2_mul_inl(py, t.get(2)));
-  }
-  return ok;
+  return miller_t_in_subgroup_k(t, qload, PSI_KX, PSI_KY);
+}
+template <typename TS, typename Q>
+DI bool miller_t_in_subgroup_scaled(const TS& t, Q qload) {
+  return miller_t_in_subgroup_k(t, qload, PSI_KX_G1N, PSI_KY_G1N);
 }
 
 template <typename Put, typename XP, typename YP>
diff --git a/drand_amd/csrc/threshold.cpp b/drand_amd/csrc/threshold.cpp
--- a/drand_amd/csrc/threshold.cpp
+++ b/drand_amd/csrc/threshold.cpp
@@ -11,7 +11,7 @@
   c->has_group = false;
   c->group_bytes.clear();
   std::vector<uint8_t> cls;
-  int rc = decode_g1(c, commits48, t, c->commits, c->commit_inf, cls);
+  int rc = decode_g1(c, commits48, t, c->commits, c->commit_inf, cls, &c->commit_sc);
   if (rc) return rc;
   for (size_t i = 0; i < t; i++)
     if (cls[i]) return fail(c, BLSV_EINVAL, "set_group: commitment %zu rejected (class %d)", i, (int)cls[i]);
@@ -85,7 +85,7 @@
   bool in_table = true;
   for (size_t i = 0; i < k; i++) in_table = in_table && index[i] < c->pk_all_n;
   std::vector<uint32_t> ident;
-  PkSel pk{c->pk_all.as<uint32_t>(), c->pk_all_inf.as<uint8_t>(), c->idx.as<uint32_t>()};
+  PkSel pk{c->pk_all.as<uint32_t>(), c->pk_all_inf.as<uint8_t>(), c->idx.as<uint32_t>(), nullptr};
   if (!in_table) {
     HIPCHK(c, c->pp_tab.ensure(k * blsk::G1_WORDS * 4));
     HIPCHK(c, c->pp_inf.ensure(k));
diff --git a/drand_amd/csrc/verify.cpp b/drand_amd/csrc/verify.cpp
--- a/drand_amd/csrc/verify.cpp
+++ b/drand_amd/csrc/verify.cpp
@@ -61,8 +61,8 @@
   if (mn == cnt) {
     {
       StageTimer tm(c, ST_MILLER, cnt, st);
-      blsk::launch_miller(pk.tab, pk.inf, pk.idx, H, h_inf, S, s_inf, cls, cnt, w.F, w.LN, std::min(cnt, kLineSub),
-                          w.FW, check_subgroup, st);
+      blsk::launch_miller(pk.tab, pk.inf, pk.idx, pk.sc, H, h_inf, S, s_inf, cls, cnt, w.F, w.LN,
+                          std::min(cnt, kLineSub), w.FW, check_subgroup, st);
     }
     StageTimer tm(c, ST_FEXP, cnt, st);
     final_exp(c, cnt, cls, st);
@@ -91,7 +91,8 @@
   SplitDrain drain{c};
   const size_t rem = cnt - mn;
   rm.a = mark(st);
-  blsk::launch_miller_lines(pk.tab, pk.inf, pk.idx, H, h_inf, S, s_inf, cls, cnt, 0, cnt, w.LN, cnt, check_subgroup, st);
+  blsk::launch_miller_lines(pk.tab, pk.inf, pk.idx, pk.sc, H, h_inf, S, s_inf, cls, cnt, 0, cnt, w.LN, cnt,
+                            check_subgroup, st);
   blsk::launch_miller_f(w.LN, cnt, cls, cnt, 0, mn, w.F, w.FW, false, st);
   rm.b = mark(st);
   int rc = BLSV_OK;
@@ -222,7 +223,7 @@
 int run_passes(blsv_ctx* c, size_t n, const SigSrc& sig, const PkSel& pk, const HashFn& hash, const Tail& tail,
                const PassOut& out, hipStream_t st) {
   return for_each_pass(c, n, [&](size_t base, size_t cnt) {
-    const PkSel pass_pk{pk.tab, pk.inf, pk.idx ? pk.idx + base : nullptr};
+    const PkSel pass_pk{pk.tab, pk.inf, pk.idx ? pk.idx + base : nullptr, pk.sc};
     const int rc = run_head(c, sig, base, cnt, tail, st, hash);
     if (rc) return rc;
     return tail.randomized ? run_tail_rlc(c, base, cnt, tail.seed, out, st) : run_tail(c, base, cnt, pass_pk, out, st);
@@ -283,14 +284,17 @@
   return BLSV_OK;
 }
 
-int decode_g1(blsv_ctx* c, const uint8_t* pk48, size_t cnt, DBuf& tab, DBuf& inf, std::vector<uint8_t>& cls) {
+int decode_g1(blsv_ctx* c, const uint8_t* pk48, size_t cnt, DBuf& tab, DBuf& inf, std::vector<uint8_t>& cls,
+              DBuf* sc) {
   HIPCHK(c, tab.ensure(cnt * blsk::G1_WORDS * 4));
+  if (sc) HIPCHK(c, sc->ensure(blsk::MILLER_SC_WORDS * 4));
   HIPCHK(c, inf.ensure(cnt));
   HIPCHK(c, c->g1_cls.ensure(cnt));
   HIPCHK(c, c->misc.ensure(cnt * 48));
   HIPCHK(c, hipMemcpyAsync(c->misc.p, pk48, cnt * 48, hipMemcpyHostToDevice, c->stream));
   blsk::launch_decompress_g1(c->misc.as<uint8_t>(), cnt, tab.as<uint32_t>(), inf.as<uint8_t>(),
                              c->g1_cls.as<uint8_t>(), c->stream);
+  if (sc && cnt) blsk::launch_g1_line_consts(tab.as<uint32_t>(), sc->as<uint32_t>(), c->stream);
   HIPCHK(c, hipGetLastError());
   cls.assign(cnt, 0);
   HIPCHK(c, hipMemcpyAsync(cls.data(), c->g1_cls.p, cnt, hipMemcpyDeviceToHost, c->stream));
@@ -339,7 +343,7 @@
   const uint32_t* d_len = reinterpret_cast<const uint32_t*>(d + l.o_len);
   const uint8_t* d_msg = d + l.o_msg;
   const SigSrc sig{d + l.o_sig, 96, 0};
-  const PkSel pk{d_tab, d_tab_inf, reinterpret_cast<const uint32_t*>(d + l.o_idx)};
+  const PkSel pk{d_tab, d_tab_inf, reinterpret_cast<const uint32_t*>(d + l.o_idx), nullptr};
   if (use_lat(c, n)) {
     blsk::launch_lat_messages(d_msg, d_off, d_len, sig.d, 96, 0, n, pk.tab, pk.inf, pk.idx, c->misc.as<uint8_t>(),
                               nullptr, nullptr, c->stream);
@@ -578,13 +582,13 @@
   if (pk48) {
     if (!c->pk_cache_valid || memcmp(c->pk_cache, pk48, 48) != 0) {
       std::vector<uint8_t> cls;
-      int rc = decode_g1(c, pk48, 1, c->pk_tab, c->pk_inf, cls);
+      int rc = decode_g1(c, pk48, 1, c->pk_tab, c->pk_inf, cls, &c->pk_sc);
       if (rc) return rc;
       if (cls[0]) return fail(c, BLSV_EINVAL, "verify_messages: public key rejected (class %d)", (int)cls[0]);
       memcpy(c->pk_cache, pk48, 48);
       c->pk_cache_valid = true;
     }
-    pk = {c->pk_tab.as<uint32_t>(), c->pk_inf.as<uint8_t>(), nullptr};
+    pk = {c->pk_tab.as<uint32_t>(), c->pk_inf.as<uint8_t>(), nullptr, c->pk_sc.as<uint32_t>()};
   } else {
     if (!c->has_group) return fail(c, BLSV_ENOGROUP, "verify_messages: no group key set");
     pk = group_pk(c);
```

Measured after the change: 2.547 million beacons/s (median of 6 runs). No clear change (+0.9%).
